# martinruenz/co-fusion

Hardware: AMD Instinct MI355X
Metric: frames/sec at 640x480 (N active models) + ICP-reduce achieved HBM GB/s vs peak (higher is better)
Workload: dtype f32

## Files before the change

co_fusion_amd/csrc/cabi_model.hip:

```cpp
#include <math.h>
#include <string.h>

#include <string>
#include <vector>

#include "cf_host.h"

using namespace cf;

#define HIPCHK(ctx, call)                                                                      \
    do {                                                                                       \
        hipError_t e_ = (call);                                                                \
        if (e_ != hipSuccess) {                                                                \
            (ctx)->set_error(std::string(#call) + ": " + hipGetErrorString(e_));               \
            return CF_EHIP;                                                                    \
        }                                                                                      \
    } while (0)
#define LAUNCHCHK(ctx) HIPCHK(ctx, hipGetLastError())

struct cf_model {
    cf_ctx* ctx = nullptr;
    uint32_t max_surfels = 0;
    uint32_t count_host = 0;
    bool count_pending = false;
    hipEvent_t count_event = nullptr;
    hipEvent_t count_wait = nullptr;
    bool ratio_valid = false;
    hipEvent_t ratio_event = nullptr;
    float* buf[2] = {nullptr, nullptr};
    int target = 0;
    float* staged = nullptr;
    unsigned* flags = nullptr;
    unsigned* block_sums = nullptr;
    unsigned* d_count = nullptr;
    unsigned* d_nfresh = nullptr;
    unsigned* d_tmp2 = nullptr;
    unsigned* h_counts = nullptr;
    float* records = nullptr;
    float* fresh = nullptr;
    unsigned* new_flags = nullptr;
    bool new_flags_clean = true;
    unsigned* owner = nullptr;
    float* fb_rec = nullptr;
    float* fb_raw = nullptr;
    float* fb_filt = nullptr;
    unsigned long long* keys = nullptr;
    unsigned* index = nullptr;
    float *vertConf = nullptr, *colorTime = nullptr, *normRad = nullptr;
    float* clean_rec = nullptr;
    uint8_t* splat_image = nullptr;
    float *splat_vertex = nullptr, *splat_normal = nullptr;
    uint16_t* splat_time = nullptr;
    float *fill_vertex = nullptr, *fill_normal = nullptr;
    uint8_t* fill_image = nullptr;
    float *tcx = nullptr, *tcy = nullptr;
    float* t_inv_dev = nullptr;
    const cf_odom* preindex_od = nullptr;
    int preindex_time = -1;
    float preindex_cutoff = 0.f; int preindex_delta = 0; uint32_t preindex_nb = 0;
    void drop_preindex() { preindex_od = nullptr; preindex_time = -1; }
    float* rays = nullptr;
    float inv_fx = 0, inv_fy = 0;
};

template <typename T>
static int dmalloc(cf_ctx* ctx, T** p, size_t count)
{
    HIPCHK(ctx, hipMalloc(reinterpret_cast<void**>(p), count * sizeof(T)));
    HIPCHK(ctx, hipMemsetAsync(*p, 0, count * sizeof(T), ctx->cur()));
    return CF_OK;
}

using cf::inv44f;

static inline cf_cam ctx_cam(const cf_ctx* ctx) { return cf_cam{ctx->cfg.fx, ctx->cfg.fy, ctx->cfg.cx, ctx->cfg.cy}; }

extern "C" {

int cf_bilateral(cf_ctx* ctx, const float* depth, int cols, int rows, float maxD, float* out)
{
    if (!ctx || !depth || !out) return CF_EINVAL;
    launch_bilateral(ctx->cur(), depth, cols, rows, maxD, out);
    LAUNCHCHK(ctx);
    return CF_OK;
}

int cf_model_create(cf_ctx* ctx, int max_surfels, cf_model** out)
{
    if (!ctx || !out || max_surfels <= 0) return CF_EINVAL;
    cf_model* m = new cf_model();
    m->ctx = ctx; m->max_surfels = (uint32_t)max_surfels;
    *out = m;
    const int W = ctx->cfg.width, H = ctx->cfg.height;
    const size_t N = (size_t)W * H, M = (size_t)max_surfels, Q = N / 4 + 64;
    if (int r = dmalloc(ctx, &m->buf[0], M * 12)) return r;
    if (int r = dmalloc(ctx, &m->buf[1], M * 12)) return r;
    if (int r = dmalloc(ctx, &m->staged, (M + Q) * 12)) return r;
    if (int r = dmalloc(ctx, &m->flags, M + Q)) return r;
    if (int r = dmalloc(ctx, &m->block_sums, (M + Q) / 2048 + N / 2048 + 16)) return r;
    if (int r = dmalloc(ctx, &m->d_count, 1)) return r;
    if (int r = dmalloc(ctx, &m->d_nfresh, 1)) return r;
    if (int r = dmalloc(ctx, &m->d_tmp2, 4)) return r;
    if (int r = dmalloc(ctx, &m->records, N * 12)) return r;
    if (int r = dmalloc(ctx, &m->fresh, Q * 12)) return r;
    if (int r = dmalloc(ctx, &m->new_flags, N)) return r;
    if (int r = dmalloc(ctx, &m->owner, M)) return r;
    HIPCHK(ctx, hipMemsetAsync(m->owner, 0xFF, M * sizeof(unsigned), ctx->cur()));
    if (int r = dmalloc(ctx, &m->fb_rec, N * 12)) return r;
    if (int r = dmalloc(ctx, &m->fb_raw, N * 12)) return r;
    if (int r = dmalloc(ctx, &m->fb_filt, N * 12)) return r;
    if (int r = dmalloc(ctx, &m->keys, N)) return r;
    HIPCHK(ctx, hipMemsetAsync(m->keys, 0xFF, N * sizeof(unsigned long long), ctx->cur()));
    if (int r = dmalloc(ctx, &m->index, N)) return r;
    if (int r = dmalloc(ctx, &m->vertConf, N * 4)) return r;
    if (int r = dmalloc(ctx, &m->colorTime, N * 4)) return r;
    if (int r = dmalloc(ctx, &m->normRad, N * 4)) return r;
    if (int r = dmalloc(ctx, &m->clean_rec, N * 8)) return r;
    if (int r = dmalloc(ctx, &m->splat_image, N * 4)) return r;
    if (int r = dmalloc(ctx, &m->splat_vertex, N * 4)) return r;
    if (int r = dmalloc(ctx, &m->splat_normal, N * 4)) return r;
    if (int r = dmalloc(ctx, &m->splat_time, N)) return r;
    if (int r = dmalloc(ctx, &m->fill_vertex, N * 4)) return r;
    if (int r = dmalloc(ctx, &m->fill_normal, N * 4)) return r;
    if (int r = dmalloc(ctx, &m->fill_image, N * 4)) return r;
    if (int r = dmalloc(ctx, &m->tcx, (size_t)W)) return r;
    if (int r = dmalloc(ctx, &m->tcy, (size_t)H)) return r;
    if (int r = dmalloc(ctx, &m->rays, N * 4)) return r;
    if (int r = dmalloc(ctx, &m->t_inv_dev, 16)) return r;
    launch_splat_rays(ctx->cur(), ctx_cam(ctx), W, H, m->rays);
    HIPCHK(ctx, hipHostMalloc(reinterpret_cast<void**>(&m->h_counts), sizeof(unsigned) * 4, hipHostMallocCoherent));
    HIPCHK(ctx, hipEventCreateWithFlags(&m->count_event, hipEventDisableTiming));
    HIPCHK(ctx, hipEventCreateWithFlags(&m->ratio_event, hipEventDisableTiming));
    std::vector<float> tx(W), ty(H);
    for (int i = 0; i < W; i++) tx[i] = (float)((double)((float)i / (float)W) + 1.0 / (2.0 * (double)(float)W));
    for (int j = 0; j < H; j++) ty[j] = (float)((double)((float)j / (float)H) + 1.0 / (2.0 * (double)(float)H));
    HIPCHK(ctx, hipMemcpyAsync(m->tcx, tx.data(), sizeof(float) * W, hipMemcpyHostToDevice, ctx->cur()));
    HIPCHK(ctx, hipMemcpyAsync(m->tcy, ty.data(), sizeof(float) * H, hipMemcpyHostToDevice, ctx->cur()));
    m->inv_fx = (float)(1.0 / (double)ctx->cfg.fx); m->inv_fy = (float)(1.0 / (double)ctx->cfg.fy);
    HIPCHK(ctx, hipStreamSynchronize(ctx->cur()));
    return CF_OK;
}

void cf_model_destroy(cf_model* m)
{
    if (!m) return;
    (void)hipStreamSynchronize(m->ctx->cur());
    void* ptrs[] = {m->buf[0], m->buf[1], m->staged, m->flags, m->block_sums, m->d_count, m->d_nfresh, m->d_tmp2, m->records,
                    m->fresh, m->new_flags, m->owner, m->fb_rec, m->fb_raw, m->fb_filt, m->keys, m->index, m->vertConf,
                    m->colorTime, m->normRad, m->splat_image, m->splat_vertex, m->splat_normal, m->splat_time, m->fill_vertex,
                    m->fill_normal, m->fill_image, m->tcx, m->tcy, m->rays, m->t_inv_dev, m->clean_rec};
    for (void* p : ptrs) (void)hipFree(p);
    (void)hipHostFree(m->h_counts);
    if (m->count_event) (void)hipEventDestroy(m->count_event);
    if (m->ratio_event) (void)hipEventDestroy(m->ratio_event);
    delete m;
}

static int adopt_count(cf_model* m)
{
    m->count_host = m->h_counts[0];
    m->count_pending = false;
    if (m->count_host > m->max_surfels) { m->ctx->set_error("surfel buffer overflow"); return CF_ENOMEM; }
    return CF_OK;
}
static int sync_count(cf_model* m)
{
    cf_ctx* ctx = m->ctx;
    HIPCHK(ctx, hipMemcpyAsync(m->h_counts, m->d_count, sizeof(unsigned), hipMemcpyDeviceToHost, ctx->cur()));
    HIPCHK(ctx, hipStreamSynchronize(ctx->cur()));
    return adopt_count(m);
}
static int post_count(cf_model* m, uint32_t upper_bound)
{
    cf_ctx* ctx = m->ctx;
    HIPCHK(ctx, hipEventRecord(m->count_event, ctx->cur()));
    m->count_wait = m->count_event;
    m->count_host = upper_bound;
    m->count_pending = true;
    return CF_OK;
}
static int count_bound(cf_model* m, uint32_t* out)
{
    if (m->count_pending) {
        if (!m->count_wait) { if (int r = sync_count(m)) return r; *out = m->count_host; return CF_OK; }
        if (hipEventQuery(m->count_wait) == hipSuccess) { if (int r = adopt_count(m)) return r; }
        else (void)hipGetLastError();
    }
    *out = m->count_host;
    return CF_OK;
}
static int exact_count(cf_model* m, uint32_t* out)
{
    if (m->count_pending) {
        if (!m->count_wait) { if (int r = sync_count(m)) return r; *out = m->count_host; return CF_OK; }
        HIPCHK(m->ctx, hipEventSynchronize(m->count_wait));
        if (int r = adopt_count(m)) return r;
    }
    *out = m->count_host;
    return CF_OK;
}

int cf_model_initialise(cf_model* m, const uint8_t* rgba, const float* depth_raw, const float* depth_filt, int time, float maxDepth)
{
    if (!m || !rgba || !depth_raw || !depth_filt) return CF_EINVAL;
    m->drop_preindex();
    cf_ctx* ctx = m->ctx; hipStream_t s = ctx->cur();
    const int W = ctx->cfg.width, H = ctx->cfg.height; const long long N = (long long)W * H;
    if ((uint32_t)N > m->max_surfels) return CF_ENOMEM;
    const cf_cam cam = ctx_cam(ctx);
    launch_feedback(s, rgba, depth_raw, W, H, cam, m->inv_fx, m->inv_fy, m->tcx, m->tcy, time, maxDepth, m->fb_rec, m->new_flags);
    HIPCHK(ctx, hipMemsetAsync(m->fb_raw, 0, sizeof(float) * 12 * N, s));
    launch_scan_scatter(s, m->fb_rec, m->new_flags, N, m->block_sums, m->d_count, 0, m->fb_raw);
    launch_feedback(s, rgba, depth_filt, W, H, cam, m->inv_fx, m->inv_fy, m->tcx, m->tcy, time, maxDepth, m->fb_rec, m->new_flags);
    HIPCHK(ctx, hipMemsetAsync(m->fb_filt, 0, sizeof(float) * 12 * N, s));
    launch_scan_scatter(s, m->fb_rec, m->new_flags, N, m->block_sums, m->d_tmp2, 0, m->fb_filt);
    m->new_flags_clean = false;
    launch_init(s, m->fb_raw, m->fb_filt, m->d_count, N, m->buf[m->target]);
    LAUNCHCHK(ctx);
    return sync_count(m);
}

int cf_model_count(cf_model* m, uint32_t* count) { if (!m || !count) return CF_EINVAL; return exact_count(m, count); }

int cf_model_predict_indices(cf_model* m, const float pose[16], int time, float maxDepth, int timeDelta)
{
    if (!m || !pose) return CF_EINVAL;
    m->drop_preindex();
    cf_ctx* ctx = m->ctx;
    float t_inv[16];
    inv44f(pose, t_inv);
    uint32_t nb = 0;
    if (int r = count_bound(m, &nb)) return r;
    launch_predict_indices(ctx->cur(), m->buf[m->target], m->d_count, nb, t_inv, ctx_cam(ctx), ctx->cfg.width, ctx->cfg.height,
                           maxDepth, time, timeDelta, m->keys, m->index, m->vertConf, m->colorTime, m->normRad);
    LAUNCHCHK(ctx);
    return CF_OK;
}

int cf_model_index_keys(cf_model* m, const float pose[16], int time, float maxDepth, int timeDelta, uint32_t surfel_begin, uint32_t surfel_end,
                        uint64_t* keys_dev)
{
    if (!m || !pose || !keys_dev || surfel_begin > surfel_end) return CF_EINVAL;
    m->drop_preindex();
    cf_ctx* ctx = m->ctx;
    const int W = ctx->cfg.width, H = ctx->cfg.height;
    float t_inv[16];
    inv44f(pose, t_inv);
    uint32_t nb = 0;
    if (int r = count_bound(m, &nb)) return r;
    HIPCHK(ctx, hipMemsetAsync(keys_dev, 0xFF, sizeof(uint64_t) * (size_t)W * H, ctx->cur()));
    launch_index_keys(ctx->cur(), m->buf[m->target], m->d_count, surfel_begin, surfel_end < nb ? surfel_end : nb, t_inv, ctx_cam(ctx), W, H, maxDepth,
                      time, timeDelta, reinterpret_cast<unsigned long long*>(keys_dev));
    LAUNCHCHK(ctx);
    return CF_OK;
}
int cf_model_index_resolve(cf_model* m, const float pose[16], uint64_t* keys_dev)
{
    if (!m || !pose || !keys_dev) return CF_EINVAL;
    m->drop_preindex();
    cf_ctx* ctx = m->ctx;
    float t_inv[16];
    inv44f(pose, t_inv);
    launch_index_resolve(ctx->cur(), m->buf[m->target], t_inv, ctx->cfg.width, ctx->cfg.height, reinterpret_cast<unsigned long long*>(keys_dev),
                         m->index, m->vertConf, m->colorTime, m->normRad);
    LAUNCHCHK(ctx);
    return CF_OK;
}

int cf_model_predict_indices_sharded(cf_model* m, const float pose[16], int time, float maxDepth, int timeDelta, int shard, int nshards)
{
    if (!m || !pose || nshards < 1 || shard < 0 || shard >= nshards) return CF_EINVAL;
    m->drop_preindex();
    cf_ctx* ctx = m->ctx;
    if (!ctx->collective) { ctx->set_error("cf_model_predict_indices_sharded: no collective registered (cf_set_collective)"); return CF_ESTATE; }
    uint32_t n = 0;
    if (int r = exact_count(m, &n)) return r;
    const uint32_t b = (uint32_t)(((uint64_t)n * (uint64_t)shard) / (uint64_t)nshards), e = (uint32_t)(((uint64_t)n * (uint64_t)(shard + 1)) / (uint64_t)nshards);
    if (int r = cf_model_index_keys(m, pose, time, maxDepth, timeDelta, b, e, reinterpret_cast<uint64_t*>(m->keys))) return r;
    if (ctx->collective(ctx->collective_user, 1, m->keys, (uint64_t)ctx->cfg.width * ctx->cfg.height, (void*)ctx->cur()) != 0) {
        ctx->set_error("cf_model_predict_indices_sharded: the collective failed");
        return CF_ESTATE;
    }
    return cf_model_index_resolve(m, pose, reinterpret_cast<uint64_t*>(m->keys));
}

int cf_model_combined_predict(cf_model* m, const float pose[16], float maxDepth, float confThreshold, int time, int maxTime, int timeDelta)
{
    if (!m || !pose) return CF_EINVAL;
    cf_ctx* ctx = m->ctx;
    float t_inv[16];
    inv44f(pose, t_inv);
    uint32_t nb = 0;
    if (int r = count_bound(m, &nb)) return r;
    launch_combined_predict(ctx->cur(), m->buf[m->target], m->d_count, nb, t_inv, ctx_cam(ctx), ctx->cfg.width, ctx->cfg.height,
                            maxDepth, confThreshold, time, maxTime, timeDelta, m->rays, m->keys, m->splat_image, m->splat_vertex, m->splat_normal,
                            m->splat_time);
    LAUNCHCHK(ctx);
    m->ratio_valid = false;
    return CF_OK;
}

int cf_model_prefetch_fill_ratio(cf_model* m)
{
    if (!m) return CF_EINVAL;
    cf_ctx* ctx = m->ctx;
    launch_fill_ratio(ctx->cur(), m->splat_image, ctx->cfg.width, ctx->cfg.height, m->d_tmp2 + 2, m->h_counts + 2);
    LAUNCHCHK(ctx);
    HIPCHK(ctx, hipEventRecord(m->ratio_event, ctx->cur()));
    m->ratio_valid = true;
    return CF_OK;
}

int cf_model_perform_fill_in(cf_model* m, const uint8_t* rgba, const float* depth_filt, int passthrough_geom, int passthrough_rgb)
{
    if (!m || !rgba || !depth_filt) return CF_EINVAL;
    cf_ctx* ctx = m->ctx;
    launch_fill_in(ctx->cur(), m->splat_vertex, m->splat_normal, m->splat_image, depth_filt, rgba, ctx->cfg.width, ctx->cfg.height, ctx_cam(ctx),
                   m->inv_fx, m->inv_fy, passthrough_geom, passthrough_rgb, m->fill_vertex, m->fill_normal, m->fill_image);
    LAUNCHCHK(ctx);
    return CF_OK;
}

int cf_model_requires_fill_in(cf_model* m, float ratio, int* out)
{
    if (!m || !out) return CF_EINVAL;
    cf_ctx* ctx = m->ctx;
    if (m->ratio_valid) {
        HIPCHK(ctx, hipEventSynchronize(m->ratio_event));
    } else {
        launch_fill_ratio(ctx->cur(), m->splat_image, ctx->cfg.width, ctx->cfg.height, m->d_tmp2 + 2, m->h_counts + 2);
        LAUNCHCHK(ctx);
        HIPCHK(ctx, hipStreamSynchronize(ctx->cur()));
    }
    *out = ((float)m->h_counts[2] / (float)m->h_counts[3] < ratio) ? 1 : 0;
    return CF_OK;
}

int cf_model_fill_ratio_device(cf_model* m, const uint32_t** counts_dev)
{
    if (!m || !counts_dev) return CF_EINVAL;
    *counts_dev = m->ratio_valid ? m->d_tmp2 + 2 : nullptr;
    return CF_OK;
}

int cf_model_fuse(cf_model* m, const float pose[16], int time, const uint8_t* rgba, const uint8_t* mask, const float* depth_raw,
                  const float* depth_filt, float maxDepth, float weighting, int maskID)
{
    if (!m || !pose || !rgba || !mask || !depth_raw || !depth_filt) return CF_EINVAL;
    m->drop_preindex();
    cf_ctx* ctx = m->ctx; hipStream_t s = ctx->cur();
    const int W = ctx->cfg.width, H = ctx->cfg.height; const long long N = (long long)W * H;
    SurfelFuseArgs a;
    a.index = m->index; a.vertConf = m->vertConf; a.normRad = m->normRad; a.rgba = rgba; a.depth_raw = depth_raw; a.depth_filt = depth_filt;
    a.mask = mask; a.tcx = m->tcx; a.tcy = m->tcy; memcpy(a.pose, pose, sizeof(a.pose)); a.cam = ctx_cam(ctx); a.inv_fx = m->inv_fx;
    a.inv_fy = m->inv_fy; a.cols = W; a.rows = H; a.time = time; a.weighting = weighting; a.maskID = maskID; a.maxDepth = maxDepth;
    a.records = m->records; a.new_flags = m->new_flags; a.owner = m->owner; a.flags_clean = m->new_flags_clean ? 1 : 0;
    launch_associate(s, a);
    {
        ScanPassArgs sp{m->records, m->new_flags, N, m->block_sums, m->d_nfresh, 0, m->fresh, nullptr};
        sp.zero_flags = 1;
        launch_scan_scatter_batch(s, &sp, 1);
        m->new_flags_clean = true;
    }
    uint32_t nb = 0;
    if (int r = count_bound(m, &nb)) return r;
    launch_update(s, m->buf[m->target], m->d_count, nb, m->owner, m->records, time, m->buf[1 - m->target]);
    m->target = 1 - m->target;
    LAUNCHCHK(ctx);
    return CF_OK;
}

int cf_model_clean(cf_model* m, const float pose[16], int time, float confThreshold, float outlierCoeff, int timeDelta, const float* depth_filt,
                   const uint8_t* mask, int maskID, uint32_t* count_out)
{
    if (!m || !pose || !depth_filt || !mask) return CF_EINVAL;
    m->drop_preindex();
    cf_ctx* ctx = m->ctx; hipStream_t s = ctx->cur();
    const int W = ctx->cfg.width, H = ctx->cfg.height;
    uint32_t nb = 0;
    if (int r = count_bound(m, &nb)) return r;
    const unsigned bound = nb + (unsigned)((W / 2) * (H / 2));
    if (bound > m->max_surfels + (unsigned)(W * H / 4 + 64)) return CF_ENOMEM;
    SurfelCleanArgs a;
    a.index = m->index; a.vertConf = m->vertConf; a.colorTime = m->colorTime; a.depth_filt = depth_filt; a.mask = mask; a.rec = nullptr;
    inv44f(pose, a.t_inv); a.cam = ctx_cam(ctx); a.cols = W; a.rows = H; a.time = time; a.confThreshold = confThreshold;
    a.outlierCoeff = outlierCoeff; a.timeDelta = timeDelta; a.maskID = maskID;
    launch_clean(s, m->buf[m->target], m->d_count, m->fresh, m->d_nfresh, bound, a, m->staged, m->flags);
    launch_scan_scatter(s, m->staged, m->flags, bound, m->block_sums, m->d_count, 0, m->buf[1 - m->target], m->h_counts);
    m->target = 1 - m->target;
    LAUNCHCHK(ctx);
    const uint32_t upper = bound < m->max_surfels ? bound : m->max_surfels;
    if (int r = post_count(m, upper)) return r;
    if (count_out) return exact_count(m, count_out);
    return CF_OK;
}

int cf_models_preindex(cf_ctx* ctx, const cf_model_preindex* items, int n, float depth_cutoff, int time_delta)
{
    if (!ctx || !items || n <= 0) return CF_EINVAL;
    hipStream_t s = ctx->cur();
    const int W = ctx->cfg.width, H = ctx->cfg.height;
    std::vector<IndexPassArgs> a((size_t)n);
    for (int k = 0; k < n; k++) {
        cf_model* m = items[k].model; const cf_odom* od = items[k].odom;
        if (!m || !od || m->ctx != ctx || od->ctx != ctx) return CF_EINVAL;
        uint32_t nb = 0;
        if (int r = count_bound(m, &nb)) return r;
        const float* pinv = reinterpret_cast<const float*>(reinterpret_cast<const char*>(od->d_state) + offsetof(cf::OdomDev, pose_inv));
        IndexPassArgs& p = a[k];
        p.surfels = m->buf[m->target]; p.count = m->d_count; p.id_begin = 0; p.id_end = nb; p.maxDepth = depth_cutoff; p.time = items[k].time;
        p.timeDelta = time_delta; p.keys = m->keys; p.index = m->index; p.vertConf = m->vertConf; p.colorTime = m->colorTime; p.normRad = m->normRad;
        p.t_inv_dev = pinv;
    }
    launch_index_keys_batch(s, a.data(), n, ctx_cam(ctx), W, H);
    launch_index_resolve_batch(s, a.data(), n, ctx_cam(ctx), W, H);
    LAUNCHCHK(ctx);
    for (int k = 0; k < n; k++) {
        cf_model* m = items[k].model;
        m->preindex_od = items[k].odom; m->preindex_time = items[k].time; m->preindex_cutoff = depth_cutoff; m->preindex_delta = time_delta; m->preindex_nb = a[k].id_end;
    }
    return CF_OK;
}
static bool preindexed_with(const cf_model* m, const float pose[16], int time, float depth_cutoff, int time_delta, uint32_t nb)
{
    if (!m->preindex_od || m->preindex_time != time) return false;
    if (m->preindex_cutoff != depth_cutoff || m->preindex_delta != time_delta || m->preindex_nb != nb) return false;
    const cf::OdomDev* h = m->preindex_od->h_state;
    for (int r = 0; r < 3; r++) {
        if (memcmp(&pose[r * 4], &h->Rcurr[r * 3], 12) != 0 || memcmp(&pose[r * 4 + 3], &h->tcurr[r], 4) != 0) return false;
    }
    return pose[12] == 0 && pose[13] == 0 && pose[14] == 0 && pose[15] == 1;
}

int cf_models_frame_passes(cf_ctx* ctx, const cf_model_pass* items, int n, float depth_cutoff, float outlier_coeff, int time_delta)
{
    if (!ctx || !items || n <= 0) return CF_EINVAL;
    hipStream_t s = ctx->cur();
    const int W = ctx->cfg.width, H = ctx->cfg.height; const long long N = (long long)W * H;
    const cf_cam cam = ctx_cam(ctx);
    std::vector<int> fusing;
    for (int k = 0; k < n; k++) {
        const cf_model_pass& it = items[k];
        if (!it.model || it.model->ctx != ctx || !it.pose || !it.rgba || !it.depth_filtered) return CF_EINVAL;
        if (it.do_fuse) { if (!it.mask || !it.depth_raw) return CF_EINVAL; fusing.push_back(k); }
    }
    for (int k : fusing) {
        cf_model* m = items[k].model;
        uint32_t nb = 0;
        if (int r = count_bound(m, &nb)) return r;
        if (nb + (unsigned)((W / 2) * (H / 2)) > m->max_surfels + (unsigned)(W * H / 4 + 64)) {
            ctx->set_error("cf_models_frame_passes: a model's surfel buffer cannot hold the clean stage's staging area (max_surfels too small)");
            return CF_ENOMEM;
        }
    }
    for (int k = 0; k < n; k++) { uint32_t nb = 0; if (int r = count_bound(items[k].model, &nb)) return r; }
    int surf_ev = -1;
    if (ctx->prof.enabled > 0 && (ctx->surf_calls_seen++ % (unsigned)ctx->prof.enabled) == 0 && ctx->surf_used + 2 <= cf_ctx::kSurfEvents) {
        for (int e = ctx->surf_used; e < ctx->surf_used + 2; e++)
            if (!ctx->surf_events[e]) HIPCHK(ctx, hipEventCreate(&ctx->surf_events[e]));
        surf_ev = ctx->surf_used; ctx->surf_used += 2;
        HIPCHK(ctx, hipEventRecord(ctx->surf_events[surf_ev], s));
        for (int k = 0; k < n; k++) ctx->surf_bytes += (uint64_t)items[k].model->count_host * 48u * (items[k].do_fuse ? 8u : 2u);
        ctx->surf_calls++;
    }
    static const bool clean_rec_on = getenv("CF_NO_CLEAN_REC") == nullptr;
    auto index_args_of = [&](const std::vector<int>& which, bool feeds_clean, std::vector<IndexPassArgs>& a) -> int {
        a.assign(which.size(), IndexPassArgs{});
        for (size_t q = 0; q < which.size(); q++) {
            const cf_model_pass& it = items[which[q]]; cf_model* m = it.model;
            uint32_t nb = 0;
            if (int r = count_bound(m, &nb)) return r;
            IndexPassArgs& p = a[q];
            p.surfels = m->buf[m->target]; p.count = m->d_count; p.id_begin = 0; p.id_end = nb; inv44f(it.pose, p.t_inv); p.maxDepth = depth_cutoff;
            p.time = it.time; p.timeDelta = time_delta; p.keys = m->keys; p.index = m->index; p.vertConf = m->vertConf; p.colorTime = m->colorTime;
            p.normRad = m->normRad;
            if (feeds_clean && clean_rec_on) { p.clean_rec = m->clean_rec; p.clean_depth = it.depth_filtered; }
        }
        return CF_OK;
    };
    auto index_pass = [&](const std::vector<int>& which) -> int {
        std::vector<IndexPassArgs> a;
        if (int r = index_args_of(which, false, a)) return r;
        launch_index_keys_batch(s, a.data(), (int)a.size(), cam, W, H);
        launch_index_resolve_batch(s, a.data(), (int)a.size(), cam, W, H);
        return CF_OK;
    };
    if (!fusing.empty()) {
        const int nf = (int)fusing.size();
        {
            std::vector<int> todo;
            for (int k : fusing) {
                uint32_t nb = 0;
                if (int r = count_bound(items[k].model, &nb)) return r;
                if (!preindexed_with(items[k].model, items[k].pose, items[k].time, depth_cutoff, time_delta, nb)) todo.push_back(k);
            }
            if (!todo.empty()) { if (int r = index_pass(todo)) return r; }
        }
        std::vector<SurfelFuseArgs> fa(nf);
        std::vector<ScanPassArgs> sa(nf);
        std::vector<UpdatePassArgs> ua(nf);
        for (int q = 0; q < nf; q++) {
            const cf_model_pass& it = items[fusing[q]]; cf_model* m = it.model;
            SurfelFuseArgs& a = fa[q];
            a.index = m->index; a.vertConf = m->vertConf; a.normRad = m->normRad; a.rgba = it.rgba; a.depth_raw = it.depth_raw; a.depth_filt = it.depth_filtered;
            a.mask = it.mask; a.tcx = m->tcx; a.tcy = m->tcy; memcpy(a.pose, it.pose, sizeof(a.pose)); a.cam = cam; a.inv_fx = m->inv_fx;
            a.inv_fy = m->inv_fy; a.cols = W; a.rows = H; a.time = it.time; a.weighting = it.weighting; a.maskID = it.mask_id; a.maxDepth = it.fuse_max_depth;
            a.records = m->records; a.new_flags = m->new_flags; a.owner = m->owner; a.flags_clean = m->new_flags_clean ? 1 : 0;
            sa[q] = ScanPassArgs{m->records, m->new_flags, N, m->block_sums, m->d_nfresh, 0, m->fresh, nullptr};
            sa[q].zero_flags = 1;
            m->new_flags_clean = true;
            uint32_t nb = 0;
            if (int r = count_bound(m, &nb)) return r;
            ua[q] = UpdatePassArgs{m->buf[m->target], m->d_count, nb, m->owner, m->records, it.time, m->buf[1 - m->target]};
        }
        launch_associate_batch(s, fa.data(), nf);
        for (int q = 0; q < nf; q++) items[fusing[q]].model->target = 1 - items[fusing[q]].model->target;
        {
            std::vector<IndexPassArgs> ia;
            if (int r = index_args_of(fusing, true, ia)) return r;
            static const bool side_by_side = getenv("CF_NO_SIDE_BY_SIDE") == nullptr;
            if (!(side_by_side && launch_update_compaction_index_keys(s, ua.data(), sa.data(), ia.data(), nf, cam, W, H))) {
                launch_scan_scatter_batch(s, sa.data(), nf);
                launch_update_batch(s, ua.data(), nf);
                launch_index_keys_batch(s, ia.data(), nf, cam, W, H);
            }
            launch_index_resolve_batch(s, ia.data(), nf, cam, W, H);
        }
        std::vector<CleanPassArgs> ca(nf);
        std::vector<uint32_t> upper(nf);
        for (int q = 0; q < nf; q++) {
            const cf_model_pass& it = items[fusing[q]]; cf_model* m = it.model;
            uint32_t nb = 0;
            if (int r = count_bound(m, &nb)) return r;
            const unsigned bound = nb + (unsigned)((W / 2) * (H / 2));
            if (bound > m->max_surfels + (unsigned)(W * H / 4 + 64)) return CF_ENOMEM;
            CleanPassArgs& c = ca[q];
            c.h.index = m->index; c.h.vertConf = m->vertConf; c.h.colorTime = m->colorTime; c.h.depth_filt = it.depth_filtered; c.h.mask = it.mask;
            c.h.rec = clean_rec_on ? m->clean_rec : nullptr;
            inv44f(it.pose, c.h.t_inv); c.h.cam = cam; c.h.cols = W; c.h.rows = H; c.h.time = it.time; c.h.confThreshold = it.conf_threshold;
            c.h.outlierCoeff = outlier_coeff; c.h.timeDelta = time_delta; c.h.maskID = it.mask_id;
            c.surfels = m->buf[m->target]; c.count = m->d_count; c.fresh = m->fresh; c.n_fresh = m->d_nfresh; c.total_bound = bound; c.staged = m->staged;
            c.flags = m->flags;
            sa[q] = ScanPassArgs{m->staged, m->flags, (long long)bound, m->block_sums, m->d_count, 0, m->buf[1 - m->target], m->h_counts};
            upper[q] = bound < m->max_surfels ? bound : m->max_surfels;
        }
        launch_clean_batch(s, ca.data(), nf);
        launch_scan_scatter_batch(s, sa.data(), nf);
        if (!ctx->batch_event) HIPCHK(ctx, hipEventCreateWithFlags(&ctx->batch_event, hipEventDisableTiming));
        for (int q = 0; q < nf; q++) {
            cf_model* m = items[fusing[q]].model;
            m->target = 1 - m->target;
            m->count_host = upper[q]; m->count_pending = true; m->count_wait = nullptr;
        }
    }
    std::vector<SplatPassArgs> pa(n);
    for (int k = 0; k < n; k++) {
        const cf_model_pass& it = items[k]; cf_model* m = it.model;
        uint32_t nb = m->count_host;
        if (!(m->count_pending && !m->count_wait)) { if (int r = count_bound(m, &nb)) return r; }
        SplatPassArgs& p = pa[k];
        p.surfels = m->buf[m->target]; p.count = m->d_count; p.count_bound = nb; inv44f(it.pose, p.t_inv); p.maxDepth = depth_cutoff;
        p.confThreshold = it.conf_threshold; p.time = it.time; p.maxTime = it.time; p.timeDelta = time_delta; p.rays = m->rays; p.keys = m->keys;
        p.image = m->splat_image; p.vertexConf = m->splat_vertex; p.normalRad = m->splat_normal; p.time16 = m->splat_time;
        m->ratio_valid = false;
    }
    launch_combined_predict_batch(s, pa.data(), n, cam, W, H);
    LAUNCHCHK(ctx);
    if (surf_ev >= 0) HIPCHK(ctx, hipEventRecord(ctx->surf_events[surf_ev + 1], s));
    if (!fusing.empty()) {
        HIPCHK(ctx, hipEventRecord(ctx->batch_event, s));
        for (int k : fusing) items[k].model->count_wait = ctx->batch_event;
    }
    for (int k = 0; k < n; k++) items[k].model->drop_preindex();
    return CF_OK;
}

int cf_model_download_map(cf_model* m, float* host_surfels, uint32_t capacity, uint32_t* count)
{
    if (!m || !count) return CF_EINVAL;
    cf_ctx* ctx = m->ctx;
    if (int r = exact_count(m, count)) return r;
    if (host_surfels) {
        const uint32_t n = m->count_host < capacity ? m->count_host : capacity;
        HIPCHK(ctx, hipMemcpyAsync(host_surfels, m->buf[m->target], (size_t)n * 48, hipMemcpyDeviceToHost, ctx->cur()));
        HIPCHK(ctx, hipStreamSynchronize(ctx->cur()));
    }
    return CF_OK;
}

int cf_model_upload_map(cf_model* m, const float* host_surfels, uint32_t count)
{
    if (!m || (!host_surfels && count) || count > m->max_surfels) return CF_EINVAL;
    m->drop_preindex();
    cf_ctx* ctx = m->ctx;
    if (count) HIPCHK(ctx, hipMemcpyAsync(m->buf[m->target], host_surfels, (size_t)count * 48, hipMemcpyHostToDevice, ctx->cur()));
    launch_set_count(ctx->cur(), m->d_count, count);
    HIPCHK(ctx, hipStreamSynchronize(ctx->cur()));
    m->count_host = count; m->count_pending = false;
    return CF_OK;
}

int cf_model_buffer(cf_model* m, int which, void** dptr, uint64_t* bytes)
{
    if (!m || !dptr) return CF_EINVAL;
    const size_t N = (size_t)m->ctx->cfg.width * m->ctx->cfg.height;
    void* p = nullptr; size_t b = 0;
    switch (which) {
        case 0: p = m->index; b = N * 4; break;
        case 1: p = m->vertConf; b = N * 16; break;
        case 2: p = m->colorTime; b = N * 16; break;
        case 3: p = m->normRad; b = N * 16; break;
        case 4: p = m->splat_image; b = N * 4; break;
        case 5: p = m->splat_vertex; b = N * 16; break;
        case 6: p = m->splat_normal; b = N * 16; break;
        case 7: p = m->splat_time; b = N * 2; break;
        case 8: p = m->fill_vertex; b = N * 16; break;
        case 9: p = m->fill_normal; b = N * 16; break;
        case 10: p = m->fill_image; b = N * 4; break;
        case 11: { uint32_t c = 0; if (int r = exact_count(m, &c)) return r; p = m->buf[m->target]; b = (size_t)c * 48; break; }
        default: return CF_EINVAL;
    }
    *dptr = p; if (bytes) *bytes = b;
    return CF_OK;
}

float cf_fusion_weight(const float pose[16], const float lastPose[16], float weightMultiplier)
{
    float pinv[16], diff[16];
    inv44f(pose, pinv);
    for (int i = 0; i < 4; i++)
        for (int j = 0; j < 4; j++) {
            float s = 0;
            for (int k = 0; k < 4; k++) s += pinv[i * 4 + k] * lastPose[k * 4 + j];
            diff[i * 4 + j] = s;
        }
    const float tn = sqrtf(diff[3] * diff[3] + diff[7] * diff[7] + diff[11] * diff[11]);
    const float* R = diff;
    double rx = R[2 * 4 + 1] - R[1 * 4 + 2], ry = R[0 * 4 + 2] - R[2 * 4 + 0], rz = R[1 * 4 + 0] - R[0 * 4 + 1];
    const double s = sqrt((rx * rx + ry * ry + rz * rz) * 0.25);
    double c = (double)((R[0] + R[5] + R[10]) - 1.0f) * 0.5;
    c = c > 1. ? 1. : c < -1. ? -1. : c;
    double theta = acos(c);
    if (s < 1e-5) {
        double t;
        if (c > 0) rx = ry = rz = 0;
        else {
            t = (R[0] + 1) * 0.5; rx = sqrt(t > 0.0 ? t : 0.0);
            t = (R[5] + 1) * 0.5; ry = sqrt(t > 0.0 ? t : 0.0) * (R[0 * 4 + 1] < 0 ? -1.0 : 1.0);
            t = (R[10] + 1) * 0.5; rz = sqrt(t > 0.0 ? t : 0.0) * (R[0 * 4 + 2] < 0 ? -1.0 : 1.0);
            if (fabs(rx) < fabs(ry) && fabs(rx) < fabs(rz) && (R[1 * 4 + 2] > 0) != (ry * rz > 0)) rz = -rz;
            theta /= sqrt(rx * rx + ry * ry + rz * rz);
            rx *= theta; ry *= theta; rz *= theta;
        }
    } else {
        double vth = 1 / (2 * s);
        vth *= theta;
        rx *= vth; ry *= vth; rz *= vth;
    }
    const float rv[3] = {(float)rx, (float)ry, (float)rz};
    const float rn = sqrtf(rv[0] * rv[0] + rv[1] * rv[1] + rv[2] * rv[2]);
    float weighting = tn > rn ? tn : rn;
    const float largest = 0.01f, minWeight = 0.5f;
    if (weighting > largest) weighting = largest;
    const float w = 1.0f - (weighting / largest);
    weighting = (w > minWeight ? w : minWeight) * weightMultiplier;
    return weighting;
}

}
```

co_fusion_amd/csrc/cf_kernels.h:

```cpp
#pragma once

#include <hip/hip_runtime.h>
#include <hip/hip_ext.h>
#include <stdint.h>

#include "../../include/cofusion_hip.h"

namespace cf {

constexpr int kGroups = 64;

struct alignas(64) GnHot {
    int icp, level_done; float cull_z[2];
    float Rcurr[9], tcurr[3];
    float Rprev_inv[9], tprev[3];
    int cull_box[4];
    int rgb, rgbOnly, level_done2, pad;
    float krkInv[9], kt[3];
};
static_assert(sizeof(GnHot) == 192, "three 64-byte lines");

struct OdomDev;
struct OdomDev {
    const float* vmap_curr[3];
    const float* nmap_curr[3];
    const float* vmap_g_prev[3];
    const float* nmap_g_prev[3];
    const float* lastDepth[3];
    const float* nextDepth[3];
    const uint8_t* lastImage[3];
    const uint8_t* nextImage[3];
    const uint8_t* lastNextImage[3];
    const int16_t* dIdx[3];
    const int16_t* dIdy[3];
    const float* cloud[3];
    cf_dataterm* corres[3];
    const uint8_t* cand[3];
    unsigned long long* icp_acc;
    unsigned long long* rgb_acc;
    float* err_surface;
    cf_cam intr;
    int width, height;
    float distThres, angleThres, sobelScale, maxDepthDeltaRGB;
    float minGrad[3];
    float icpWeight;
    int icp, rgb, rgbOnly;
    unsigned* aabb_acc;
    int cull;
    float box_R[9], box_t[3];
    unsigned* res_range;
    OdomDev* host_twin;
    float Rprev[9], tprev[3], Rprev_inv[9], Rcurr[9], tcurr[3];
    double resultRt[16];
    float krkInv[9], kt[3];
    float lastRGBError;
    int level_done;
    int solves;
    float residual[2];
    float box_lo[3], box_hi[3];
    int res_seen[3];
    float cull_z[2];
    float pose_inv[16];
    cf_track_stats stats;
    GnHot hot;
};
__host__ __device__ inline void refresh_hot(OdomDev* od)
{
    GnHot& h = od->hot;
    h.icp = od->icp; h.level_done = od->level_done; h.cull_z[0] = od->cull_z[0]; h.cull_z[1] = od->cull_z[1];
    for (int k = 0; k < 9; k++) { h.Rcurr[k] = od->Rcurr[k]; h.Rprev_inv[k] = od->Rprev_inv[k]; h.krkInv[k] = od->krkInv[k]; }
    for (int k = 0; k < 3; k++) { h.tcurr[k] = od->tcurr[k]; h.tprev[k] = od->tprev[k]; h.kt[k] = od->kt[k]; }
    for (int k = 0; k < 4; k++) h.cull_box[k] = od->stats.cull_box[k];
    h.rgb = od->rgb; h.rgbOnly = od->rgbOnly; h.level_done2 = od->level_done; h.pad = 0;
}

void launch_vmap(hipStream_t s, const float* depth, int cols, int rows, cf_cam intr, float cutoff, float* vmap);
void launch_nmap(hipStream_t s, const float* vmap, int cols, int rows, float* nmap);
void launch_copy_maps(hipStream_t s, const float* v4, const float* n4, int cols, int rows, float* vmap, float* nmap);
void launch_resize_map(hipStream_t s, const float* in, int in_cols, int in_rows, float* out, bool normalize);
void launch_transform_maps(hipStream_t s, float* vmap, float* nmap, int cols, int rows, const float R[9], const float t[3]);
void launch_vertices_to_depth(hipStream_t s, const float* v4, int cols, int rows, float cutoff, float* depth);
void launch_pyrdown_f32(hipStream_t s, const float* src, int scols, int srows, float* dst);
void launch_pyrdown_u8(hipStream_t s, const uint8_t* src, int scols, int srows, uint8_t* dst);
void launch_intensity(hipStream_t s, const uint8_t* rgba, int cols, int rows, uint8_t* dst);
void launch_rgb_expand(hipStream_t s, const uint8_t* rgb, int n, uint8_t* rgba);
void launch_sobel(hipStream_t s, const uint8_t* src, int cols, int rows, int16_t* dx, int16_t* dy);
void launch_cloud(hipStream_t s, const float* depth, int cols, int rows, cf_cam il, float* cloud3);

struct Level3 { int cols[3], rows[3], blk_end[3]; };
struct FrameMapsArgs {
    Level3 L;
    const float* depth[3]; float* vmap[3]; float* nmap[3];
    float fx_inv[3], fy_inv[3], cx[3], cy[3];
    float cutoff;
    float2* zrange[3];
};
struct RgbPrepArgs {
    Level3 L;
    const uint8_t* nextImage[3]; const float* nextDepth[3]; const float* lastDepth[3];
    int16_t* dIdx[3]; int16_t* dIdy[3]; uint8_t* cand[3]; float* cloud[3];
    float minScale[3], fx_inv[3], fy_inv[3], cx[3], cy[3];
    unsigned* res_range;
};
struct ModelMapsArgs {
    const float* pred_v4; const float* pred_n4;
    const float* alt_v4; const float* alt_n4;
    const unsigned* sel; float sel_ratio;
    float* snapshot;
    float* vmap[3]; float* nmap[3];
    int cols, rows;
    float R[9], t[3];
    unsigned char* occ;
    unsigned* aabb;
};
constexpr int kPrepBatch = 8;
struct ModelMapsBatch { ModelMapsArgs m[kPrepBatch]; };
struct RgbPrepBatch { RgbPrepArgs m[kPrepBatch]; };
struct RgbdChain {
    const float* v4; const uint8_t* rgba; float* depth[3]; uint8_t* image[3];
    const float* alt_v4; const uint8_t* alt_rgba; const unsigned* sel; float sel_ratio;
};
struct RgbdBatch {
    RgbdChain c[2 * kPrepBatch];
    uint8_t* fan_image[3][kPrepBatch];
    signed char fan_owner[kPrepBatch];
};
void launch_model_maps(hipStream_t s, const ModelMapsBatch& b, int n);
void launch_frame_maps(hipStream_t s, FrameMapsArgs a, int W, int H);
void launch_rgbd_pyramids(hipStream_t s, const RgbdBatch& b, int n_chains, int W, int H, float cutoff);
void launch_model_maps_and_pyramids(hipStream_t s, const ModelMapsBatch& mb, int n, const RgbdBatch& rb, int n_chains, int W, int H, float cutoff);
void launch_rgb_prep(hipStream_t s, RgbPrepBatch b, int n, int W, int H);

struct IDiv { unsigned M, s; };
inline IDiv make_idiv(int d)
{
    if (d < 2) return IDiv{0x80000000u, 0u};
    unsigned l = 0;
    while ((1u << l) < (unsigned)d) l++;
    return IDiv{(unsigned)((((unsigned long long)1 << (31 + l)) + (unsigned)d - 1) / (unsigned)d), l - 1};
}
constexpr int kGramBits[8] = {20, 20, 20, 17, 17, 17, 22, 0};
struct LaunchShape { int icp[3]; int res[3]; int icp_err; };
struct IcpLaunch { int threads; int ppt; int gram;
                   LaunchShape* const* shape = nullptr; };

constexpr int kMaxBatch = 16;
struct IcpModelArgs {
    const float* vc; const float* nc;
    const float* vp; const float* np;
    const OdomDev* st;
    unsigned long long* acc;
    float* err;
    const unsigned char* occ;
    int row_begin, row_end;
    int cull;
    const float2* zr;
    int box_blocks;
};
constexpr int kNoBoxHint = 0x7fffffff;
struct CullRuns { int x0, y0, nrx, total; };
__host__ __device__ inline CullRuns cull_runs(const int box[4], int L, int cols, int rows)
{
    int bx0 = (box[0] >> L) - 1, by0 = (box[1] >> L) - 1, bx1 = (box[2] >> L) + 1, by1 = (box[3] >> L) + 1;
    bx0 = bx0 < 0 ? 0 : bx0; by0 = by0 < 0 ? 0 : by0; bx1 = bx1 > cols - 1 ? cols - 1 : bx1; by1 = by1 > rows - 1 ? rows - 1 : by1;
    if (bx0 > bx1 || by0 > by1) return CullRuns{0, 0, 0, 0};
    if ((cols & 63) == 0) { const int nrx = (bx1 >> 6) - (bx0 >> 6) + 1; return CullRuns{bx0 >> 6, by0, nrx, nrx * (by1 - by0 + 1)}; }
    const int q0 = (by0 * cols) >> 6, q1 = ((by1 + 1) * cols - 1) >> 6;
    return CullRuns{0, q0, 0, q1 - q0 + 1};
}
inline int box_blocks_for(const int box_hint[4], int L, int cols, int rows, int threads)
{
    if (box_hint[0] == kNoBoxHint) return 0;
    const CullRuns cr = cull_runs(box_hint, L, cols, rows);
    const int wpb = threads / 64;
    const int runs = cr.total + cr.total / 4 + 2 * (cr.nrx > 0 ? cr.nrx : (cols + 63) / 64);
    int want = (((runs + 2 * wpb - 1) / (2 * wpb) + 7) / 8) * 8;
    return want < 8 ? 8 : want;
}
inline int residual_blocks_for(int seen) { return seen < 0 ? 0 : seen + seen / 4 + 2; }
struct GnArgs {
    OdomDev* od[kMaxBatch];
    unsigned long long* icp_acc[kMaxBatch];
    unsigned long long* rgb_acc[kMaxBatch];
    OdomDev* od_host[kMaxBatch];
    int slot_px;
    int icp_gram;
};
struct RgbModelArgs {
    OdomDev* st;
    const uint8_t* cand; const float* nextDepth; const float* lastDepth;
    const uint8_t* lastImage; const uint8_t* nextImage;
    cf_dataterm* corres; const float* cloud; const int16_t* dIdx; const int16_t* dIdy;
    unsigned long long* icp_acc; unsigned long long* rgb_acc;
    int no_counts;
    uint2* recs;
    unsigned* slot_counts;
    const unsigned* res_range;
    int res_blocks;
};
struct RgbArgs {
    RgbModelArgs m[kMaxBatch];
    int cols, rows;
    cf_cam il;
    float sobelScale, maxDepthDelta;
    int compact;
    int slot_px;
    IDiv cdiv;
};
inline RgbModelArgs rgb_model_args(const OdomDev* h , OdomDev* d_state, int level)
{
    return RgbModelArgs{d_state, h->cand[level], h->nextDepth[level], h->lastDepth[level], h->lastImage[level], h->nextImage[level],
                        h->corres[level], h->cloud[level], h->dIdx[level], h->dIdy[level], h->icp_acc, h->rgb_acc, 0,
                        reinterpret_cast<uint2*>(h->corres[level]),
                        reinterpret_cast<unsigned*>(reinterpret_cast<uint2*>(h->corres[level]) + (size_t)(h->width >> level) * (h->height >> level)),
                        h->res_range ? h->res_range + 2 * level : nullptr, 0};
}
constexpr int kMaxSlots = 2 * kMaxBatch;
struct IcpArgs {
    IcpModelArgs m[kMaxBatch];
    int cols, rows;
    cf_cam intr;
    float distThres, angleThres;
    float angleSqLt, distSqLe;
    int occ_w, occ_shift;
    int flags;
    int row_begin, row_end;
    IDiv cdiv;
    int slot_end[kMaxSlots];
    unsigned char slot_desc[kMaxSlots];
    int slots_used;
};
constexpr unsigned char kResidualSlot = 0x80;
void launch_icp_level(hipStream_t s, IcpLaunch cfg, const IcpArgs& args, int n, int level, hipEvent_t ev0 = nullptr, hipEvent_t ev1 = nullptr);
void launch_rgb_residual(hipStream_t s, const RgbArgs& ra, int n);
void launch_rgb_step(hipStream_t s, const RgbArgs& ra, int n);
constexpr uint64_t kRgbResidualBytes = 27;
constexpr uint64_t kRgbResidualBytesCompact = 11;
void launch_acc_total(hipStream_t s, const unsigned long long* acc, unsigned long long* out);
void launch_rgb_cand(hipStream_t s, const int16_t* dIdx, const int16_t* dIdy, const float* next_depth,
                     const uint8_t* next_image, float min_scale, int cols, int rows, uint8_t* cand);
void launch_so3_step(hipStream_t s, const uint8_t* last_image, const uint8_t* next_image, const float basis[9],
                     const float kinv[9], const float krlr[9], int cols, int rows, unsigned long long* out16);

struct ProfSink {
    hipEvent_t* events; int capacity; int used; uint64_t bytes; uint64_t launches; int enabled;
};

constexpr int kSo3Blocks = 16;
constexpr int kStepSubs = 16;
struct So3Sync { unsigned long long acc[10][16]; unsigned arrive, depart;
                 unsigned step_top, pad;
                 unsigned step_sub[kStepSubs][32]; };
struct GnHook { int (*fn)(void* user, int op, void* dev_buf, uint64_t words, void* stream); void* user; int split[kMaxBatch]; };
struct TrackerStates { OdomDev* dev[kMaxBatch]; const OdomDev* host[kMaxBatch]; };
bool launch_gn_track(hipStream_t s, IcpLaunch cfg, const TrackerStates& states, So3Sync* so3_syncs ,
                     const GnHook* hook, const IcpArgs icp_args[3], const RgbArgs rgb_args[3], int n, int width, int height, bool so3,
                     bool pyramid, bool fast_odom, bool rgb, bool icp, int mode, ProfSink* prof,
                     OdomDev* const* h_states = nullptr ,
                     const RgbPrepBatch* prep = nullptr );
void rgb_prep_levels(RgbPrepBatch& b, int n, int W, int H);
float replay_icp_level0(hipStream_t s, IcpLaunch cfg, const IcpArgs& a0, const RgbArgs& r0, int n, int slots, int ablate, int reps, hipEvent_t e0, hipEvent_t e1);
#ifdef CF_ABLATE
void trace_so3_dump(hipStream_t s);
void trace_solve_begin();
void trace_solve_end(hipStream_t s, const char* path);
void trace_step_solve(hipStream_t s, IcpLaunch cfg, const IcpArgs& a0, const RgbArgs& r0, So3Sync* syncs, int n, const char* path);
void trace_icp_level0(hipStream_t s, IcpLaunch cfg, const IcpArgs& a0, const RgbArgs& r0, int n, int slots, const char* path);
#endif
bool probe_xcd_round_robin(hipStream_t s);
float sqrt_gate_lt(float T);
float sqrt_gate_le(float T);

constexpr int kSurfBatch = 16;
struct IndexPassArgs {
    const float* surfels; const unsigned* count; unsigned id_begin, id_end; float t_inv[16]; float maxDepth; int time, timeDelta;
    unsigned long long* keys; unsigned* index; float* vertConf; float* colorTime; float* normRad;
    const float* t_inv_dev;
    float* clean_rec;
    const float* clean_depth;
};
__host__ __device__ inline void inv44f(const float a[16], float o[16])
{
    const float c00 = a[5] * a[10] - a[6] * a[9];
    const float c01 = a[6] * a[8] - a[4] * a[10];
    const float c02 = a[4] * a[9] - a[5] * a[8];
    const float det = a[0] * c00 + a[1] * c01 + a[2] * c02;
    const float id = 1.0f / det;
    float Li[9];
    Li[0] = c00 * id; Li[1] = (a[2] * a[9] - a[1] * a[10]) * id; Li[2] = (a[1] * a[6] - a[2] * a[5]) * id;
    Li[3] = c01 * id; Li[4] = (a[0] * a[10] - a[2] * a[8]) * id; Li[5] = (a[2] * a[4] - a[0] * a[6]) * id;
    Li[6] = c02 * id; Li[7] = (a[1] * a[8] - a[0] * a[9]) * id; Li[8] = (a[0] * a[5] - a[1] * a[4]) * id;
    for (int i = 0; i < 3; i++) {
        o[i * 4 + 0] = Li[i * 3 + 0]; o[i * 4 + 1] = Li[i * 3 + 1]; o[i * 4 + 2] = Li[i * 3 + 2];
        o[i * 4 + 3] = -(Li[i * 3 + 0] * a[3] + Li[i * 3 + 1] * a[7] + Li[i * 3 + 2] * a[11]);
    }
    o[12] = 0; o[13] = 0; o[14] = 0; o[15] = 1;
}
struct SplatPassArgs {
    const float* surfels; const unsigned* count; unsigned count_bound; float t_inv[16]; float maxDepth, confThreshold; int time, maxTime, timeDelta;
    const float* rays; unsigned long long* keys; uint8_t* image; float* vertexConf; float* normalRad; uint16_t* time16;
};
struct UpdatePassArgs { const float* in; const unsigned* count; unsigned count_bound; unsigned* owner; const float* records; int time; float* out; };
struct SurfelFuseArgs {
    const unsigned* index; const float* vertConf; const float* normRad;
    const uint8_t* rgba; const float* depth_raw; const float* depth_filt; const uint8_t* mask;
    const float* tcx; const float* tcy;
    float pose[16]; cf_cam cam; float inv_fx, inv_fy;
    int cols, rows, time; float weighting; int maskID; float maxDepth;
    float* records; unsigned* new_flags; unsigned* owner;
    int flags_clean = 0;
};
struct SurfelCleanArgs {
    const unsigned* index; const float* vertConf; const float* colorTime;
    const float* depth_filt; const uint8_t* mask;
    const float* rec;
    float t_inv[16]; cf_cam cam; int cols, rows, time; float confThreshold, outlierCoeff; int timeDelta, maskID;
};
struct CleanPassArgs {
    SurfelCleanArgs h; const float* surfels; const unsigned* count; const float* fresh; const unsigned* n_fresh; unsigned total_bound;
    float* staged; unsigned* flags;
};
struct ScanPassArgs {
    const float* rec; const unsigned* flags; long long n; unsigned* block_sums; unsigned* total; unsigned add_to_total; float* out; unsigned* total_host;
    int zero_flags = 0;
};
void launch_index_keys_batch(hipStream_t s, const IndexPassArgs* items, int n, cf_cam cam, int cols, int rows);
bool launch_update_compaction_index_keys(hipStream_t s, const UpdatePassArgs* up, const ScanPassArgs* sc, const IndexPassArgs* ix, int n, cf_cam cam, int cols,
                                         int rows);
void launch_index_resolve_batch(hipStream_t s, const IndexPassArgs* items, int n, cf_cam cam, int cols, int rows);
void launch_combined_predict_batch(hipStream_t s, const SplatPassArgs* items, int n, cf_cam cam, int cols, int rows);
void launch_associate_batch(hipStream_t s, const SurfelFuseArgs* items, int n);
void launch_update_batch(hipStream_t s, const UpdatePassArgs* items, int n);
void launch_clean_batch(hipStream_t s, const CleanPassArgs* items, int n);
void launch_scan_scatter_batch(hipStream_t s, const ScanPassArgs* items, int n);
void launch_bilateral(hipStream_t s, const float* depth, int cols, int rows, float maxD, float* out);
void launch_scan_scatter(hipStream_t s, const float* rec, const unsigned* flags, long long n, unsigned* block_sums, unsigned* total,
                         unsigned add_to_total, float* out, unsigned* total_host = nullptr );
void launch_feedback(hipStream_t s, const uint8_t* rgba, const float* depth, int cols, int rows, cf_cam cam, float inv_fx, float inv_fy,
                     const float* tcx, const float* tcy, int time, float maxDepth, float* rec, unsigned* flags);
void launch_init(hipStream_t s, const float* raw, const float* filt, const unsigned* raw_count, long long max_n, float* out);
void launch_index_keys(hipStream_t s, const float* surfels, const unsigned* count, unsigned id_begin, unsigned id_end, const float t_inv[16],
                       cf_cam cam, int cols, int rows, float maxDepth, int time, int timeDelta, unsigned long long* keys);
void launch_index_resolve(hipStream_t s, const float* surfels, const float t_inv[16], int cols, int rows, unsigned long long* keys,
                          unsigned* index, float* vertConf, float* colorTime, float* normRad);
void launch_predict_indices(hipStream_t s, const float* surfels, const unsigned* count, unsigned count_bound, const float t_inv[16], cf_cam cam,
                            int cols, int rows, float maxDepth, int time, int timeDelta, unsigned long long* keys, unsigned* index,
                            float* vertConf, float* colorTime, float* normRad);
void launch_splat_rays(hipStream_t s, cf_cam cam, int cols, int rows, float* rays );
void launch_combined_predict(hipStream_t s, const float* surfels, const unsigned* count, unsigned count_bound, const float t_inv[16], cf_cam cam,
                             int cols, int rows, float maxDepth, float confThreshold, int time, int maxTime, int timeDelta,
                             const float* rays, unsigned long long* keys, uint8_t* image, float* vertexConf, float* normalRad, uint16_t* time16);
void launch_fill_in(hipStream_t s, const float* pv, const float* pn, const uint8_t* pimg, const float* depth, const uint8_t* rgba, int cols,
                    int rows, cf_cam cam, float inv_fx, float inv_fy, int pass_geom, int pass_rgb, float* ov, float* on, uint8_t* oi);
void launch_fill_ratio(hipStream_t s, const uint8_t* pimg, int cols, int rows, unsigned* out2, unsigned* out2_host = nullptr );
void launch_associate(hipStream_t s, const SurfelFuseArgs& h);
void launch_update(hipStream_t s, const float* in, const unsigned* count, unsigned count_bound, unsigned* owner, const float* records, int time,
                   float* out);
void launch_clean(hipStream_t s, const float* surfels, const unsigned* count, const float* fresh, const unsigned* n_fresh, unsigned total_bound,
                  const SurfelCleanArgs& h, float* staged, unsigned* flags);
void launch_set_count(hipStream_t s, unsigned* out, unsigned v);

}
```

co_fusion_amd/csrc/cf_surfel_device.h:

```cpp
#pragma once

#include "cf_device.h"

namespace cf {

struct Surfel { float4 pos_conf, col_time, norm_rad; };

__device__ __forceinline__ int iclamp(int v, int lo, int hi) { return v < lo ? lo : (v > hi ? hi : v); }
__device__ __forceinline__ int nearest_texel(float u, int size) { return iclamp((int)floorf(u * (float)size), 0, size - 1); }

__device__ __forceinline__ float det_expf(float x)
{
    if (!(x > -87.0f)) return (x != x) ? x : 0.0f;
    if (x > 88.0f) return __int_as_float(0x7f800000);
    const float n = rintf(x * 1.44269504088896341f);
    float r = x - n * 0.693145751953125f;
    r = r - n * 1.42860682030941723212e-6f;
    float p = 1.0f / 720.0f;
    p = p * r + 1.0f / 120.0f;
    p = p * r + 1.0f / 24.0f;
    p = p * r + 1.0f / 6.0f;
    p = p * r + 0.5f;
    p = p * r + 1.0f;
    p = p * r + 1.0f;
    return ldexpf(p, (int)n);
}
__device__ __forceinline__ float det_acos_r(float z)
{
    const float pS0 = 1.6666586697e-01f, pS1 = -4.2743422091e-02f, pS2 = -8.6563630030e-03f, qS1 = -7.0662963390e-01f;
    const float p = z * (pS0 + z * (pS1 + z * pS2));
    const float q = 1.0f + z * qS1;
    return p / q;
}
__device__ __forceinline__ float det_acosf(float x)
{
    const float pio2 = 1.57079637050628662109375f, pi = 3.1415927410125732421875f;
    if (x != x || x > 1.0f || x < -1.0f) return qnan();
    if (fabsf(x) < 0.5f) return pio2 - (x + x * det_acos_r(x * x));
    if (x < 0.0f) {
        const float z = (1.0f + x) * 0.5f, s = sqrtf(z);
        return pi - 2.0f * (s + s * det_acos_r(z));
    }
    const float z = (1.0f - x) * 0.5f, s = sqrtf(z);
    return 2.0f * (s + s * det_acos_r(z));
}

__device__ __forceinline__ float get_radius(float depth, float norm_z, float inv_fx, float inv_fy)
{
    const float meanFocal = ((1.0f / fabsf(inv_fx)) + (1.0f / fabsf(inv_fy))) / 2.0f;
    const float sqrt2 = 1.41421356237f;
    const float radius = (depth / meanFocal) * sqrt2;
    float radius_n = radius;
    radius_n = radius_n / fabsf(norm_z);
    radius_n = fminf(2.0f * radius, radius_n);
    return radius_n;
}
__device__ __forceinline__ float confidence(float x, float y, float cx, float cy, float weighting)
{
    const float dx = x - cx, dy = y - cy;
    const float radialDist = sqrtf(dx * dx + dy * dy) / 400.0f;
    return det_expf((-(radialDist * radialDist) / 0.72f)) * weighting;
}
__device__ __forceinline__ float glsl_round(float v) { return (v < 0) ? -floorf(-v + 0.5f) : floorf(v + 0.5f); }
__device__ __forceinline__ float encode_color(float r, float g, float b)
{
    int rgb = (int)glsl_round(r * 255.0f);
    rgb = (rgb << 8) + (int)glsl_round(g * 255.0f);
    rgb = (rgb << 8) + (int)glsl_round(b * 255.0f);
    return (float)rgb;
}
__device__ __forceinline__ f3 decode_color(float c)
{
    const int ci = (int)c;
    return f3{(float)((ci >> 16) & 0xFF) / 255.0f, (float)((ci >> 8) & 0xFF) / 255.0f, (float)(ci & 0xFF) / 255.0f};
}

struct Mat4 { float m[16]; };
__device__ __forceinline__ f3 xform_point(const Mat4& T, f3 p)
{
    return f3{T.m[0] * p.x + T.m[1] * p.y + T.m[2] * p.z + T.m[3], T.m[4] * p.x + T.m[5] * p.y + T.m[6] * p.z + T.m[7],
              T.m[8] * p.x + T.m[9] * p.y + T.m[10] * p.z + T.m[11]};
}
__device__ __forceinline__ f3 xform_dir(const Mat4& T, f3 p)
{
    return f3{T.m[0] * p.x + T.m[1] * p.y + T.m[2] * p.z, T.m[4] * p.x + T.m[5] * p.y + T.m[6] * p.z,
              T.m[8] * p.x + T.m[9] * p.y + T.m[10] * p.z};
}

__device__ __forceinline__ float4 tex4_linear(const float4* __restrict__ img, int cols, int rows, float u, float v)
{
    const float fu = u * (float)cols - 0.5f, fv = v * (float)rows - 0.5f;
    const float x0f = floorf(fu), y0f = floorf(fv);
    const float wx = fu - x0f, wy = fv - y0f;
    const int x0 = iclamp((int)x0f, 0, cols - 1), x1 = iclamp((int)x0f + 1, 0, cols - 1);
    const int y0 = iclamp((int)y0f, 0, rows - 1), y1 = iclamp((int)y0f + 1, 0, rows - 1);
    const float4 a = img[y0 * cols + x0], b = img[y0 * cols + x1], c = img[y1 * cols + x0], d = img[y1 * cols + x1];
    float4 r;
    {
        const float top = a.x * (1.0f - wx) + b.x * wx, bot = c.x * (1.0f - wx) + d.x * wx;
        r.x = top * (1.0f - wy) + bot * wy;
    }
    {
        const float top = a.y * (1.0f - wx) + b.y * wx, bot = c.y * (1.0f - wx) + d.y * wx;
        r.y = top * (1.0f - wy) + bot * wy;
    }
    {
        const float top = a.z * (1.0f - wx) + b.z * wx, bot = c.z * (1.0f - wx) + d.z * wx;
        r.z = top * (1.0f - wy) + bot * wy;
    }
    {
        const float top = a.w * (1.0f - wx) + b.w * wx, bot = c.w * (1.0f - wx) + d.w * wx;
        r.w = top * (1.0f - wy) + bot * wy;
    }
    return r;
}

__device__ __forceinline__ f3 get_vertex(const float* __restrict__ depth, int cols, int rows, int px, int py, float x, float y,
                                         float cx, float cy, float inv_fx, float inv_fy)
{
    const float z = depth[iclamp(py, 0, rows - 1) * cols + iclamp(px, 0, cols - 1)];
    return f3{(x - cx) * z * inv_fx, (y - cy) * z * inv_fy, z};
}
__device__ __forceinline__ f3 half_sum(f3 a, f3 b) { return f3{(a.x + b.x) / 2, (a.y + b.y) / 2, (a.z + b.z) / 2}; }
__device__ __forceinline__ f3 get_normal_central(f3 p, const float* __restrict__ depth, int cols, int rows, int px, int py, float x,
                                                 float y, float cx, float cy, float inv_fx, float inv_fy)
{
    const f3 xf = get_vertex(depth, cols, rows, px + 1, py, x + 1, y, cx, cy, inv_fx, inv_fy);
    const f3 xb = get_vertex(depth, cols, rows, px - 1, py, x - 1, y, cx, cy, inv_fx, inv_fy);
    const f3 yf = get_vertex(depth, cols, rows, px, py + 1, x, y + 1, cx, cy, inv_fx, inv_fy);
    const f3 yb = get_vertex(depth, cols, rows, px, py - 1, x, y - 1, cx, cy, inv_fx, inv_fy);
    const f3 del_x = half_sum(xb, p) - half_sum(xf, p);
    const f3 del_y = half_sum(yb, p) - half_sum(yf, p);
    return normalized(cross(del_x, del_y));
}

}
```

co_fusion_amd/csrc/surfel.hip:

```cpp
#include "cf_surfel_device.h"
#include "cf_kernels.h"

namespace cf {

static constexpr int kB = 256;
static inline int gridFor(long long n) { return (int)((n + kB - 1) / kB); }
static inline int gridXcd(long long n, int chunk = 1) { const int q = 8 * (chunk > 1 ? chunk : 1); return (gridFor(n) + q - 1) / q * q; }
#ifdef CF_ABLATE
static int xcd_env(const char* name, int dflt) { const char* e = getenv(name); return e ? atoi(e) : dflt; }
#else
static constexpr int xcd_env(const char*, int dflt) { return dflt; }
#endif
struct BatchHdr { int n; int blk_end[kSurfBatch]; };
template <class A> struct Batch { BatchHdr h; A m[kSurfBatch]; };
struct VBlock { int model, bid, nblk; };
__device__ __forceinline__ VBlock batch_decode_at(const BatchHdr& h, int b)
{
    int slot = 0;
#pragma unroll
    for (int k = 0; k < kSurfBatch - 1; k++) slot += (b >= h.blk_end[k]) ? 1 : 0;
    const int start = slot ? h.blk_end[slot - 1] : 0;
    return VBlock{slot, b - start, h.blk_end[slot] - start};
}
__device__ __forceinline__ VBlock batch_decode(const BatchHdr& h) { return batch_decode_at(h, (int)blockIdx.x); }
template <class A>
static int batch_layout(Batch<A>& B, const int* blocks, int n)
{
    int total = 0;
    B.h.n = n;
    for (int k = 0; k < kSurfBatch; k++) {
        if (k < n) total += (blocks[k] + 7) / 8 * 8;
        B.h.blk_end[k] = k < n ? total : 0x7fffffff;
    }
    return total;
}

__device__ __forceinline__ int xcd_block(int chunk, int b, int nblk)
{
    if (chunk == 0) return b;
    const int per = nblk >> 3, x = b & 7, r = b >> 3;
    if (chunk < 0) return x * per + r;
    const int lb = ((r / chunk) * 8 + x) * chunk + (r % chunk);
    return lb;
}

__device__ __forceinline__ unsigned sortable_bits(float z)
{
    const unsigned b = __float_as_uint(z);
    return (b & 0x80000000u) ? ~b : (b | 0x80000000u);
}
__device__ __forceinline__ unsigned long long zkey(float z, unsigned id) { return ((unsigned long long)sortable_bits(z) << 32) | id; }
constexpr unsigned long long kEmptyKey = ~0ull;

__global__ void __launch_bounds__(kB) bilateral_kernel(const float* __restrict__ depth, int cols, int rows, float maxD,
                                                       float* __restrict__ out)
{
    const int i = blockIdx.x * kB + threadIdx.x;
    if (i >= cols * rows) return;
    const int y = i / cols, x = i - y * cols;
    const float value = depth[i];
    if (value > maxD || value < 0.3f) { out[i] = 0; return; }
    float sum1 = 0, sum2 = 0;
#pragma unroll
    for (int dy = -6; dy <= 6; ++dy) {
        const int cy = y + dy;
        if (cy < 0 || cy >= rows) continue;
        const float* __restrict__ rowp = depth + cy * cols + x;
#pragma unroll
        for (int dx = -6; dx <= 6; ++dx) {
            const int cx = x + dx;
            if (cx < 0 || cx >= cols) continue;
            const float tmp = rowp[dx];
            const float space2 = (float)(dx * dx + dy * dy);
            const float color2 = (value - tmp) * (value - tmp);
            const float weight = det_expf(-(space2 * 0.024691358f + color2 * 555.556f));
            sum1 += tmp * weight;
            sum2 += weight;
        }
    }
    out[i] = sum1 / sum2;
}

static constexpr int kScanItems = 2048;
struct ScanArgs {
    const float4* rec; const unsigned* flags; long long n; unsigned* block_sums; unsigned* total; unsigned add_to_total; float4* out;
    unsigned* total_host; int zero_flags;
};
__device__ __forceinline__ void scan_load_flags(const unsigned* __restrict__ flags, long long i0, long long n, unsigned (&f)[8])
{
    if (i0 + 8 <= n) {
        const uint4 a = *reinterpret_cast<const uint4*>(flags + i0), c = *reinterpret_cast<const uint4*>(flags + i0 + 4);
        f[0] = a.x; f[1] = a.y; f[2] = a.z; f[3] = a.w; f[4] = c.x; f[5] = c.y; f[6] = c.z; f[7] = c.w;
    } else {
        unsigned t[8];
#pragma unroll
        for (int e = 0; e < 8; e++) t[e] = flags[i0 + e < n ? i0 + e : n - 1];
#pragma unroll
        for (int e = 0; e < 8; e++) f[e] = (i0 + e < n) ? t[e] : 0u;
    }
}
__device__ __forceinline__ void scan_block_sums_body(const Batch<ScanArgs>& B, int blk)
{
    const VBlock vb = batch_decode_at(B.h, blk);
    const ScanArgs& a = B.m[vb.model];
    const unsigned* __restrict__ flags = a.flags; const long long n = a.n; unsigned* __restrict__ block_sums = a.block_sums;
    if ((long long)vb.bid * kScanItems >= n) return;
    unsigned f[8];
    scan_load_flags(flags, (long long)vb.bid * kScanItems + (long long)threadIdx.x * 8, n, f);
    unsigned s = 0;
#pragma unroll
    for (int e = 0; e < 8; e++) s += f[e];
    for (int o = 32; o > 0; o >>= 1) s += __shfl_xor((int)s, o, 64);
    __shared__ unsigned w[4];
    if ((threadIdx.x & 63) == 0) w[threadIdx.x >> 6] = s;
    __syncthreads();
    if (threadIdx.x == 0) block_sums[vb.bid] = w[0] + w[1] + w[2] + w[3];
}
__global__ void __launch_bounds__(256) scan_block_sums_kernel(const Batch<ScanArgs> B) { scan_block_sums_body(B, (int)blockIdx.x); }
__global__ void set_count_kernel(unsigned* out, unsigned v);
__global__ void set_count2_kernel(unsigned* out, unsigned* out_host, unsigned v);
__device__ __forceinline__ void scan_scatter_body(const Batch<ScanArgs>& B, int blk)
{
    const VBlock vb = batch_decode_at(B.h, blk);
    const ScanArgs& a = B.m[vb.model];
    const float4* __restrict__ rec = a.rec; const unsigned* __restrict__ flags = a.flags; const long long n = a.n;
    const unsigned* __restrict__ block_sums = a.block_sums; unsigned* __restrict__ total = a.total; const unsigned add_to_total = a.add_to_total;
    float4* __restrict__ out = a.out; unsigned* __restrict__ total_host = a.total_host;
    const int nb = (int)((n + kScanItems - 1) / kScanItems);
    if (vb.bid >= nb) return;
    __shared__ unsigned wsum[4], s_base;
    __shared__ unsigned short s_src[kScanItems];
    const int tid = threadIdx.x, lane = tid & 63, wave = tid >> 6;
    const long long i0 = (long long)vb.bid * kScanItems + (long long)tid * 8;
    unsigned f[8];
    scan_load_flags(flags, i0, n, f);
    if (a.zero_flags) {
        unsigned* fz = const_cast<unsigned*>(flags);
        if (i0 + 8 <= n) { *reinterpret_cast<uint4*>(fz + i0) = make_uint4(0, 0, 0, 0); *reinterpret_cast<uint4*>(fz + i0 + 4) = make_uint4(0, 0, 0, 0); }
        else
            for (int e = 0; e < 8; e++) if (i0 + e < n) fz[i0 + e] = 0;
    }
    unsigned b = 0;
    for (int k = tid; k < vb.bid; k += 256) b += block_sums[k];
    for (int o = 32; o > 0; o >>= 1) b += __shfl_xor((int)b, o, 64);
    if (lane == 0) wsum[wave] = b;
    __syncthreads();
    if (tid == 0) s_base = wsum[0] + wsum[1] + wsum[2] + wsum[3];
    unsigned mine = 0;
#pragma unroll
    for (int e = 0; e < 8; e++) mine += f[e];
    unsigned incl = mine;
    for (int o = 1; o < 64; o <<= 1) { const unsigned t = __shfl_up((int)incl, o, 64); if (lane >= o) incl += t; }
    __syncthreads();
    if (lane == 63) wsum[wave] = incl;
    __syncthreads();
    unsigned rel = incl - mine;
    for (int w = 0; w < wave; w++) rel += wsum[w];
#pragma unroll
    for (int e = 0; e < 8; e++)
        if (f[e]) s_src[rel++] = (unsigned short)(tid * 8 + e);
    const unsigned count = wsum[0] + wsum[1] + wsum[2] + wsum[3];
    const unsigned base = s_base;
    __syncthreads();
    const float4* __restrict__ in0 = rec + (size_t)vb.bid * kScanItems * 3;
    float4* __restrict__ out0 = out + (size_t)base * 3;
    const unsigned words = count * 3;
#ifndef CF_SCAN_FLY
#define CF_SCAN_FLY 4
#endif
    constexpr int kFly = CF_SCAN_FLY;
    for (unsigned m0 = tid; m0 < words; m0 += kFly * 256) {
        float4 v[kFly];
#pragma unroll
        for (int u = 0; u < kFly; u++) {
            const unsigned m = m0 + u * 256;
            const unsigned mc = m < words ? m : words - 1;
            const unsigned j = mc / 3u;
            v[u] = in0[(size_t)s_src[j] * 3 + (mc - 3u * j)];
        }
#pragma unroll
        for (int u = 0; u < kFly; u++) { const unsigned m = m0 + u * 256; if (m < words) out0[m] = v[u]; }
    }
    if (vb.bid == nb - 1 && tid == 255) {
        *total = base + count + add_to_total;
        if (total_host) *total_host = base + count + add_to_total;
    }
}
__global__ void __launch_bounds__(256) scan_scatter_kernel(const Batch<ScanArgs> B) { scan_scatter_body(B, (int)blockIdx.x); }

void launch_scan_scatter_batch(hipStream_t s, const ScanPassArgs* items, int n_items)
{
    for (int base = 0; base < n_items; base += kSurfBatch) {
        const int nb = n_items - base < kSurfBatch ? n_items - base : kSurfBatch;
        Batch<ScanArgs> B;
        int blocks[kSurfBatch], any = 0;
        for (int k = 0; k < nb; k++) {
            const ScanPassArgs& h = items[base + k];
            B.m[k] = ScanArgs{reinterpret_cast<const float4*>(h.rec), h.flags, h.n, h.block_sums, h.total, h.add_to_total, reinterpret_cast<float4*>(h.out), h.total_host, h.zero_flags};
            blocks[k] = (int)((B.m[k].n + kScanItems - 1) / kScanItems);
            any += blocks[k];
            if (blocks[k] == 0) set_count2_kernel<<<1, 1, 0, s>>>(B.m[k].total, B.m[k].total_host, B.m[k].add_to_total);
        }
        if (!any) continue;
        const int grid = batch_layout(B, blocks, nb);
        scan_block_sums_kernel<<<grid, 256, 0, s>>>(B);
        scan_scatter_kernel<<<grid, 256, 0, s>>>(B);
    }
}
void launch_scan_scatter(hipStream_t s, const float* rec, const unsigned* flags, long long n, unsigned* block_sums, unsigned* total,
                         unsigned add_to_total, float* out, unsigned* total_host)
{
    const ScanPassArgs a{rec, flags, n, block_sums, total, add_to_total, out, total_host};
    launch_scan_scatter_batch(s, &a, 1);
}

__global__ void __launch_bounds__(kB) feedback_kernel(const uchar4* __restrict__ rgba, const float* __restrict__ depth, int cols, int rows,
                                                      float cx, float cy, float inv_fx, float inv_fy, const float* __restrict__ tcx,
                                                      const float* __restrict__ tcy, int time, float maxDepth,
                                                      float4* __restrict__ rec , unsigned* __restrict__ flags)
{
    const int q = blockIdx.x * kB + threadIdx.x;
    if (q >= cols * rows) return;
    const int j = q / cols, i = q - j * cols;
    const int rank = i * rows + j;
    const float x = tcx[i] * (float)cols, y = tcy[j] * (float)rows;
    const f3 p = get_vertex(depth, cols, rows, i, j, x, y, cx, cy, inv_fx, inv_fy);
    if (p.z <= 0 || p.z > maxDepth) { flags[rank] = 0; return; }
    const f3 n = get_normal_central(p, depth, cols, rows, i, j, x, y, cx, cy, inv_fx, inv_fy);
    const uchar4 c = rgba[q];
    flags[rank] = 1;
    rec[rank * 3 + 0] = make_float4(p.x, p.y, p.z, confidence(x, y, cx, cy, 1.0f));
    rec[rank * 3 + 1] = make_float4(encode_color((float)c.x / 255.0f, (float)c.y / 255.0f, (float)c.z / 255.0f), 0.f, (float)c.z / 255.0f, (float)time);
    rec[rank * 3 + 2] = make_float4(n.x, n.y, n.z, get_radius(p.z, n.z, inv_fx, inv_fy));
}


__global__ void __launch_bounds__(kB) init_kernel(const float4* __restrict__ raw, const float4* __restrict__ filt,
                                                  const unsigned* __restrict__ raw_count, float4* __restrict__ out)
{
    const unsigned k = blockIdx.x * kB + threadIdx.x;
    if (k >= *raw_count) return;
    const float4 c = raw[k * 3 + 1];
    out[k * 3] = raw[k * 3];
    out[k * 3 + 1] = make_float4(c.x, 0.f, 1.f, c.w);
    out[k * 3 + 2] = filt[k * 3 + 2];
}

__device__ __forceinline__ bool index_project(const float4 pc, const float4 ct, const Mat4& t_inv, cf_cam cam, int cols, int rows,
                                              float maxDepth, int time, int timeDelta, f3& ph, int& q)
{
    ph = xform_point(t_inv, f3{pc.x, pc.y, pc.z});
    if (ph.z > maxDepth || ph.z < 0 || (float)time - ct.w > (float)timeDelta) return false;
    const float u = ((cam.fx * ph.x) / ph.z) + cam.cx, v = ((cam.fy * ph.y) / ph.z) + cam.cy;
    if (!(u >= 0.0f && v >= 0.0f && u < (float)cols && v < (float)rows)) return false;
    if (!(ph.z < maxDepth)) return false;
    q = (int)floorf(v) * cols + (int)floorf(u);
    return true;
}

struct IndexArgs {
    const float4* surfels; const unsigned* count; Mat4 t_inv; float maxDepth; int time, timeDelta; unsigned id_begin, id_end;
    unsigned long long* keys; unsigned* index; float4* vertConf; float4* colorTime; float4* normRad;
    const float* t_inv_dev;
    float4* clean_rec; const float* clean_depth;
};
__device__ __forceinline__ Mat4 index_matrix(const IndexArgs& a)
{
    if (!a.t_inv_dev) return a.t_inv;
    Mat4 m;
#pragma unroll
    for (int k = 0; k < 16; k++) m.m[k] = a.t_inv_dev[k];
    return m;
}
struct FrameGeom { cf_cam cam; int cols, rows; };

__device__ __forceinline__ void index_splat_body(const Batch<IndexArgs>& B, const FrameGeom& g, int blk)
{
    const VBlock vb = batch_decode_at(B.h, blk);
    const IndexArgs& a = B.m[vb.model];
    const float4* __restrict__ surfels = a.surfels;
    const unsigned id = a.id_begin + vb.bid * kB + threadIdx.x;
    if (id >= *a.count || id >= a.id_end) return;
    f3 ph; int q;
    const Mat4 T = index_matrix(a);
    if (!index_project(surfels[id * 3], surfels[id * 3 + 1], T, g.cam, g.cols, g.rows, a.maxDepth, a.time, a.timeDelta, ph, q)) return;
    atomicMin(&a.keys[q], zkey(ph.z, id));
}
__global__ void __launch_bounds__(kB) index_splat_kernel(const Batch<IndexArgs> B, const FrameGeom g) { index_splat_body(B, g, (int)blockIdx.x); }

__global__ void __launch_bounds__(kB) index_resolve_kernel(const Batch<IndexArgs> B, const FrameGeom g)
{
    const VBlock vb = batch_decode(B.h);
    const IndexArgs& a = B.m[vb.model];
    const float4* __restrict__ surfels = a.surfels; unsigned long long* __restrict__ keys = a.keys; unsigned* __restrict__ index = a.index;
    float4* __restrict__ vertConf = a.vertConf; float4* __restrict__ colorTime = a.colorTime; float4* __restrict__ normRad = a.normRad;
    const int q = vb.bid * kB + threadIdx.x;
    if (q >= g.cols * g.rows) return;
    const unsigned long long k = keys[q];
    keys[q] = kEmptyKey;
    float4* __restrict__ const rec = a.clean_rec;
    const float dflt = rec ? a.clean_depth[q] : 0.f;
    if (k == kEmptyKey) {
        index[q] = 0;
        vertConf[q] = colorTime[q] = normRad[q] = make_float4(0, 0, 0, 0);
        if (rec) { rec[2 * q] = make_float4(0, 0, 0, 0); rec[2 * q + 1] = make_float4(0, 0, __uint_as_float(0u), dflt); }
        return;
    }
    const unsigned id = (unsigned)k;
    const float4 pc = surfels[id * 3], ct = surfels[id * 3 + 1], nr = surfels[id * 3 + 2];
    const Mat4 T = index_matrix(a);
    const f3 ph = xform_point(T, f3{pc.x, pc.y, pc.z});
    const f3 n = normalized(xform_dir(T, f3{nr.x, nr.y, nr.z}));
    index[q] = id;
    vertConf[q] = make_float4(ph.x, ph.y, ph.z, pc.w);
    colorTime[q] = ct;
    normRad[q] = make_float4(n.x, n.y, n.z, nr.w);
    if (rec) { rec[2 * q] = make_float4(ph.x, ph.y, ph.z, pc.w); rec[2 * q + 1] = make_float4(ct.z, ct.w, __uint_as_float(id), dflt); }
}

struct SplatSetup { f3 ph, n; float rad, pn; int x_lo, x_hi, y_lo, y_hi; };

__device__ __forceinline__ bool splat_setup(const float4 pc, const float4 ct, const float4 nr, const Mat4& t_inv, cf_cam cam, int cols,
                                            int rows, float maxDepth, float confThreshold, int time, int maxTime, int timeDelta,
                                            SplatSetup& s)
{
    s.ph = xform_point(t_inv, f3{pc.x, pc.y, pc.z});
    if (s.ph.z > maxDepth || s.ph.z < 0 || pc.w < confThreshold || (float)time - ct.w > (float)timeDelta || ct.w > (float)maxTime) return false;
    s.n = normalized(xform_dir(t_inv, f3{nr.x, nr.y, nr.z}));
    s.rad = nr.w;
    const f3 x1n = normalized(f3{s.n.y - s.n.z, -s.n.x, s.n.x});
    const f3 x1 = {x1n.x * s.rad * 1.41421356f, x1n.y * s.rad * 1.41421356f, x1n.z * s.rad * 1.41421356f};
    const f3 y1 = cross(s.n, x1);
    const f3 c[4] = {s.ph + x1, s.ph + y1, s.ph - y1, s.ph - x1};
    float px_[4], py_[4];
#pragma unroll
    for (int k = 0; k < 4; k++) { px_[k] = ((cam.fx * c[k].x) / c[k].z) + cam.cx; py_[k] = ((cam.fy * c[k].y) / c[k].z) + cam.cy; }
    const float xmin = fminf(px_[0], fminf(px_[1], fminf(px_[2], px_[3]))), xmax = fmaxf(px_[0], fmaxf(px_[1], fmaxf(px_[2], px_[3])));
    const float ymin = fminf(py_[0], fminf(py_[1], fminf(py_[2], py_[3]))), ymax = fmaxf(py_[0], fmaxf(py_[1], fmaxf(py_[2], py_[3])));
    const float size = fmaxf(0.0f, fmaxf(fabsf(xmax - xmin), fabsf(ymax - ymin)));
    if (!(size > 0.0f) || !(size <= 4096.0f)) return false;
    const float u = ((cam.fx * s.ph.x) / s.ph.z) + cam.cx, v = ((cam.fy * s.ph.y) / s.ph.z) + cam.cy;
    if (!(u >= 0.0f && v >= 0.0f && u <= (float)cols && v <= (float)rows)) return false;
    const float half = size * 0.5f;
    s.x_lo = max((int)ceilf(u - half - 0.5f), 0); s.x_hi = min((int)ceilf(u + half - 0.5f) - 1, cols - 1);
    s.y_lo = max((int)ceilf(v - half - 0.5f), 0); s.y_hi = min((int)ceilf(v + half - 0.5f) - 1, rows - 1);
    s.pn = dot(s.ph, s.n);
    return true;
}

__device__ __forceinline__ bool splat_fragment(const SplatSetup& s, const float4* __restrict__ rays, int cols, int px, int py, float maxDepth,
                                               float& z)
{
    const float4 lr = rays[py * cols + px];
    const f3 l = {lr.x, lr.y, lr.z};
    const float k = s.pn / dot(l, s.n);
    const f3 cp = {k * l.x, k * l.y, k * l.z};
    const f3 diff = cp - s.ph;
    if (!(dot(diff, diff) <= s.rad * s.rad)) return false;
    if (!(cp.z < maxDepth)) return false;
    z = cp.z;
    return true;
}

__global__ void __launch_bounds__(kB) splat_rays_kernel(cf_cam cam, int cols, int rows, float4* __restrict__ rays)
{
    const int q = blockIdx.x * kB + threadIdx.x;
    if (q >= cols * rows) return;
    const int py = q / cols, px = q - py * cols;
    const float fx_ = (float)px + 0.5f, fy_ = (float)py + 0.5f;
    const f3 l = normalized(f3{(fx_ - cam.cx) / cam.fx, (fy_ - cam.cy) / cam.fy, 1.0f});
    rays[q] = make_float4(l.x, l.y, l.z, 0.f);
}

struct SplatArgs {
    const float4* surfels; const unsigned* count; Mat4 t_inv; float maxDepth, confThreshold; int time, maxTime, timeDelta;
    const float4* rays; unsigned long long* keys; uchar4* image; float4* vertexConf; float4* normalRad; unsigned short* time16;
};

__global__ void __launch_bounds__(kB) splat_raster_kernel(const Batch<SplatArgs> B, const FrameGeom g)
{
    const VBlock vb = batch_decode(B.h);
    const SplatArgs& a = B.m[vb.model];
    const float4* __restrict__ surfels = a.surfels; const float4* __restrict__ rays = a.rays; unsigned long long* __restrict__ keys = a.keys;
    const int cols = g.cols, rows = g.rows;
    const unsigned gt = vb.bid * kB + threadIdx.x;
    const unsigned id = gt >> 2;
    const int sub = (int)(gt & 3u);
    if (id >= *a.count) return;
    SplatSetup s;
    if (!splat_setup(surfels[id * 3], surfels[id * 3 + 1], surfels[id * 3 + 2], a.t_inv, g.cam, cols, rows, a.maxDepth, a.confThreshold, a.time,
                     a.maxTime, a.timeDelta, s))
        return;
    const int w = s.x_hi - s.x_lo + 1, h = s.y_hi - s.y_lo + 1;
    if (w <= 0 || h <= 0) return;
    int fx = sub, fy = 0;
    while (fx >= w) { fx -= w; fy++; }
    while (fy < h) {
        const int px = s.x_lo + fx, py = s.y_lo + fy;
        float z;
        if (splat_fragment(s, rays, cols, px, py, a.maxDepth, z)) {
            atomicMin(&keys[py * cols + px], zkey(z, id));
        }
        fx += 4;
        while (fx >= w) { fx -= w; fy++; }
    }
}

__global__ void __launch_bounds__(kB) splat_resolve_kernel(const Batch<SplatArgs> B, const FrameGeom g)
{
    const VBlock vb = batch_decode(B.h);
    const SplatArgs& a = B.m[vb.model];
    const float4* __restrict__ surfels = a.surfels; const float4* __restrict__ rays = a.rays; unsigned long long* __restrict__ keys = a.keys;
    uchar4* __restrict__ image = a.image; float4* __restrict__ vertexConf = a.vertexConf; float4* __restrict__ normalRad = a.normalRad;
    unsigned short* __restrict__ time16 = a.time16;
    const int cols = g.cols, rows = g.rows;
    const cf_cam cam = g.cam;
    const int q = vb.bid * kB + threadIdx.x;
    if (q >= cols * rows) return;
    const unsigned long long k = keys[q];
    keys[q] = kEmptyKey;
    if (k == kEmptyKey) {
        image[q] = make_uchar4(0, 0, 0, 0);
        vertexConf[q] = normalRad[q] = make_float4(0, 0, 0, 0);
        time16[q] = 0;
        return;
    }
    const unsigned id = (unsigned)k;
    const int py = q / cols, px = q - py * cols;
    const float4 pc = surfels[id * 3], ct = surfels[id * 3 + 1], nr = surfels[id * 3 + 2];
    SplatSetup s;
    splat_setup(pc, ct, nr, a.t_inv, cam, cols, rows, a.maxDepth, a.confThreshold, a.time, a.maxTime, a.timeDelta, s);
    float z;
    splat_fragment(s, rays, cols, px, py, a.maxDepth, z);
    const f3 col = decode_color(ct.x);
    image[q] = make_uchar4((unsigned char)glsl_round(col.x * 255.0f), (unsigned char)glsl_round(col.y * 255.0f),
                           (unsigned char)glsl_round(col.z * 255.0f), 255);
    const float fx_ = (float)px + 0.5f, fy_ = (float)py + 0.5f;
    vertexConf[q] = make_float4((fx_ - cam.cx) * z * (1.f / cam.fx), (fy_ - cam.cy) * z * (1.f / cam.fy), z, pc.w);
    normalRad[q] = make_float4(s.n.x, s.n.y, s.n.z, s.rad);
    time16[q] = (unsigned short)(unsigned)ct.z;
}

__global__ void __launch_bounds__(kB) fill_in_kernel(const float4* __restrict__ pv, const float4* __restrict__ pn, const uchar4* __restrict__ pimg,
                                                     const float* __restrict__ depth, const uchar4* __restrict__ rgba, int cols, int rows,
                                                     float cx, float cy, float inv_fx, float inv_fy, int pass_geom, int pass_rgb,
                                                     float4* __restrict__ ov, float4* __restrict__ on, uchar4* __restrict__ oi)
{
    const int q = blockIdx.x * kB + threadIdx.x;
    if (q >= cols * rows) return;
    const int y = q / cols, x = q - y * cols;
    const float z = depth[q];
    const f3 p = {((float)x - cx) * z * inv_fx, ((float)y - cy) * z * inv_fy, z};
    const float4 v = pv[q];
    ov[q] = (v.z == 0 || pass_geom) ? make_float4(p.x, p.y, p.z, 1.f) : v;
    const float4 n = pn[q];
    if (n.z == 0 || pass_geom) {
        const float zx = depth[y * cols + min(x + 1, cols - 1)], zy = depth[min(y + 1, rows - 1) * cols + x];
        const f3 vx = {((float)(x + 1) - cx) * zx * inv_fx, ((float)y - cy) * zx * inv_fy, zx};
        const f3 vy = {((float)x - cx) * zy * inv_fx, ((float)(y + 1) - cy) * zy * inv_fy, zy};
        const f3 nn = normalized(cross(vx - p, vy - p));
        on[q] = make_float4(nn.x, nn.y, nn.z, 1.f);
    } else
        on[q] = n;
    const uchar4 e = pimg[q];
    oi[q] = (((int)e.x + (int)e.y + (int)e.z) == 0 || pass_rgb) ? rgba[q] : e;
}

__global__ void __launch_bounds__(1024) fill_ratio_kernel(const uchar4* __restrict__ pimg, int cols, int rows, unsigned* __restrict__ out2,
                                                          unsigned* __restrict__ out2_host)
{
    const int dw = cols / 20, dh = rows / 20;
    unsigned s = 0;
    for (int k = threadIdx.x; k < dw * dh; k += 1024) {
        const int j = k / dw, i = k - j * dw;
        const int sx = nearest_texel(((float)i + 0.5f) / (float)dw, cols), sy = nearest_texel(((float)j + 0.5f) / (float)dh, rows);
        const uchar4 p = pimg[sy * cols + sx];
        s += (p.x > 0 && p.y > 0 && p.z > 0) ? 1u : 0u;
    }
    for (int o = 32; o > 0; o >>= 1) s += __shfl_xor((int)s, o, 64);
    __shared__ unsigned w[16];
    if ((threadIdx.x & 63) == 0) w[threadIdx.x >> 6] = s;
    __syncthreads();
    if (threadIdx.x == 0) {
        unsigned t = 0;
        for (int k = 0; k < 16; k++) t += w[k];
        out2[0] = t; out2[1] = (unsigned)(dw * dh);
        if (out2_host) { out2_host[0] = t; out2_host[1] = (unsigned)(dw * dh); }
    }
}

__device__ __forceinline__ float angle_between(f3 a, f3 b) { return det_acosf(dot(a, b) / (norm(a) * norm(b))); }

struct FuseArgs {
    const unsigned* index; const float4* vertConf; const float4* normRad;
    const uchar4* rgba; const float* depth_raw; const float* depth_filt; const unsigned char* mask;
    const float* tcx; const float* tcy;
    Mat4 pose; cf_cam cam; float inv_fx, inv_fy;
    int cols, rows, time; float weighting; int maskID; float maxDepth;
    float4* records;
    unsigned* new_flags;
    unsigned* owner;
};

__device__ __forceinline__ float bilerp(float a, float b, float c, float d, float wx, float wy)
{
    const float top = a * (1.0f - wx) + b * wx, bot = c * (1.0f - wx) + d * wx;
    return top * (1.0f - wy) + bot * wy;
}

static constexpr int kAssocItems = kB / 4;
static constexpr int kPatchStride = 7 * 16 + 1;

__global__ void __launch_bounds__(kB) associate_kernel(const Batch<FuseArgs> B, int xcd)
{
    __shared__ float s_patch[kAssocItems * kPatchStride];
    const VBlock vb = batch_decode(B.h);
    const FuseArgs& a = B.m[vb.model];
    const int cols = a.cols, rows = a.rows;
    const int par = a.time % 2;
    const int n_i = (cols - par + 1) / 2, n_j = (rows - par + 1) / 2;
    const int gt = xcd_block(xcd, vb.bid, vb.nblk) * kB + threadIdx.x;
    const int t = gt >> 2, sub = gt & 3;
    float* const P = s_patch + (threadIdx.x >> 2) * kPatchStride;
    bool alive = t < n_i * n_j;
    int i = 0, j = 0, q = 0, rank = 0;
    float tcx = 0, tcy = 0, x = 0, y = 0;
    f3 vPosLocal{0, 0, 0};
    if (alive) {
        j = 2 * (t / n_i) + par; i = 2 * (t % n_i) + par;
        q = j * cols + i; rank = i * rows + j;
        tcx = a.tcx[i]; tcy = a.tcy[j];
        x = tcx * (float)cols; y = tcy * (float)rows;
        alive = (((int)x % 2 == a.time % 2) && ((int)y % 2 == a.time % 2)) && ((int)a.mask[q] == a.maskID);
    }
    const float* dr = a.depth_raw;
    if (alive)
        alive = !(dr[j * cols + iclamp(i - 1, 0, cols - 1)] == 0 || dr[iclamp(j - 1, 0, rows - 1) * cols + i] == 0 ||
                  dr[j * cols + iclamp(i + 1, 0, cols - 1)] == 0 || dr[iclamp(j + 1, 0, rows - 1) * cols + i] == 0);
    const float cx = a.cam.cx, cy = a.cam.cy;
    if (alive) {
        vPosLocal = get_vertex(dr, cols, rows, i, j, x, y, cx, cy, a.inv_fx, a.inv_fy);
        alive = (vPosLocal.z > 0 && vPosLocal.z <= a.maxDepth);
    }
    const float scale = 1.0f;
    const float indexXStep = (1.0f / ((float)cols * scale)) * 0.5f, indexYStep = (1.0f / ((float)rows * scale)) * 0.5f;
    const float windowMultiplier = 2;
    const float iBeg = tcx - (scale * indexXStep * windowMultiplier), jBeg = tcy - (scale * indexYStep * windowMultiplier);
    const int X0 = (int)floorf(iBeg * (float)cols - 0.5f), Y0 = (int)floorf(jBeg * (float)rows - 0.5f);
    if (alive) {
#pragma unroll
        for (int c = 0; c < 4; c++) {
            const int k = sub * 4 + c;
            const int g = iclamp(Y0 + sub, 0, rows - 1) * cols + iclamp(X0 + c, 0, cols - 1);
            const float4 vcf = a.vertConf[g];
            const float4 nrd = a.normRad[g];
            const unsigned idx = a.index[g];
            P[0 * 16 + k] = vcf.x; P[1 * 16 + k] = vcf.y; P[2 * 16 + k] = vcf.z;
            P[3 * 16 + k] = nrd.x; P[4 * 16 + k] = nrd.y; P[5 * 16 + k] = nrd.z;
            P[6 * 16 + k] = __uint_as_float(idx);
        }
    }
    __syncthreads();
    if (!alive) return;

    const f3 vPos = xform_point(a.pose, vPosLocal);
    const f3 vPos_f = get_vertex(a.depth_filt, cols, rows, i, j, x, y, cx, cy, a.inv_fx, a.inv_fy);
    const f3 vNormLocal = get_normal_central(vPos_f, a.depth_filt, cols, rows, i, j, x, y, cx, cy, a.inv_fx, a.inv_fy);
    const float xl = (x - cx) * a.inv_fx, yl = (y - cy) * a.inv_fy;
    const float lambda = sqrtf(xl * xl + yl * yl + 1);
    const f3 ray = {xl, yl, 1};
    float bestDist = 1000;
    unsigned best = 0; int operation = 0, bestSeq = 0;
    float ii = iBeg;
    for (int s4 = 0; s4 < sub; s4++) ii += indexXStep;
    for (int outer = sub; ii < tcx + (scale * indexXStep * windowMultiplier);
         outer += 4, ii += indexXStep, ii += indexXStep, ii += indexXStep, ii += indexXStep) {
        int inner = 0;
        for (float jj = jBeg; jj < tcy + (scale * indexYStep * windowMultiplier); jj += indexYStep, inner++) {
            const int nlx = (int)floorf(ii * (float)cols) - X0, nly = (int)floorf(jj * (float)rows) - Y0;
            const unsigned current = ((unsigned)nlx < 4u && (unsigned)nly < 4u)
                                         ? __float_as_uint(P[6 * 16 + nly * 4 + nlx])
                                         : a.index[nearest_texel(jj, rows) * cols + nearest_texel(ii, cols)];
            if (current > 0U) {
                const float fu = ii * (float)cols - 0.5f, fv = jj * (float)rows - 0.5f;
                const float x0f = floorf(fu), y0f = floorf(fv);
                const int lx = (int)x0f - X0, ly = (int)y0f - Y0;
                const bool staged = (unsigned)lx < 3u && (unsigned)ly < 3u;
                const float wx = fu - x0f, wy = fv - y0f;
                const float* qd = P + (ly * 4 + lx);
                float4 vertConf;
                if (staged) {
                    vertConf.x = bilerp(qd[0 * 16], qd[0 * 16 + 1], qd[0 * 16 + 4], qd[0 * 16 + 5], wx, wy);
                    vertConf.y = bilerp(qd[1 * 16], qd[1 * 16 + 1], qd[1 * 16 + 4], qd[1 * 16 + 5], wx, wy);
                    vertConf.z = bilerp(qd[2 * 16], qd[2 * 16 + 1], qd[2 * 16 + 4], qd[2 * 16 + 5], wx, wy);
                } else
                    vertConf = tex4_linear(a.vertConf, cols, rows, ii, jj);
                const float zdiff = (vertConf.z - vPosLocal.z);
                if (fabsf(zdiff * lambda) < 0.05f) {
                    const float dist = norm(cross(ray, f3{vertConf.x, vertConf.y, vertConf.z}));
                    float4 normRad;
                    if (staged) {
                        normRad.x = bilerp(qd[3 * 16], qd[3 * 16 + 1], qd[3 * 16 + 4], qd[3 * 16 + 5], wx, wy);
                        normRad.y = bilerp(qd[4 * 16], qd[4 * 16 + 1], qd[4 * 16 + 4], qd[4 * 16 + 5], wx, wy);
                        normRad.z = bilerp(qd[5 * 16], qd[5 * 16 + 1], qd[5 * 16 + 4], qd[5 * 16 + 5], wx, wy);
                    } else
                        normRad = tex4_linear(a.normRad, cols, rows, ii, jj);
                    if (dist < bestDist && (fabsf(normRad.z) < 0.75f || fabsf(angle_between(f3{normRad.x, normRad.y, normRad.z}, vNormLocal)) < 0.5f)) {
                        operation = 1; bestDist = dist; best = current; bestSeq = outer * 64 + inner;
                    }
                }
            }
        }
    }
#pragma unroll
    for (int o = 1; o <= 2; o <<= 1) {
        const int oOp = __shfl_xor(operation, o, 4), oSeq = __shfl_xor(bestSeq, o, 4);
        const float oDist = __shfl_xor(bestDist, o, 4);
        const unsigned oBest = (unsigned)__shfl_xor((int)best, o, 4);
        const bool take = oOp && (!operation || oDist < bestDist || (oDist == bestDist && oSeq < bestSeq));
        if (take) { operation = 1; bestDist = oDist; best = oBest; bestSeq = oSeq; }
    }
    if (sub != 0) return;
    const uchar4 c = a.rgba[q];
    const f3 nG = xform_dir(a.pose, vNormLocal);
    const float radius = get_radius(vPos_f.z, vNormLocal.z, a.inv_fx, a.inv_fy);
    const float conf = confidence(x, y, cx, cy, a.weighting);
    const float col = (float)(((int)c.x << 16) + ((int)c.y << 8) + (int)c.z);
    a.records[rank * 3 + 0] = make_float4(vPos.x, vPos.y, vPos.z, conf);
    a.records[rank * 3 + 1] = make_float4(col, 0.f, (float)a.time, operation == 1 ? -1.f : -2.f);
    a.records[rank * 3 + 2] = make_float4(nG.x, nG.y, nG.z, radius);
    if (operation == 1) atomicMin(&a.owner[best], (unsigned)rank);
    else a.new_flags[rank] = 1;
}

struct UpdateArgs { const float4* in; const unsigned* count; unsigned* owner; const float4* records; int time; float4* out; };
__device__ __forceinline__ void update_body(const Batch<UpdateArgs>& B, int blk)
{
    const VBlock vb = batch_decode_at(B.h, blk);
    const UpdateArgs& ua = B.m[vb.model];
    const float4* __restrict__ in = ua.in; unsigned* __restrict__ owner = ua.owner; const float4* __restrict__ records = ua.records;
    float4* __restrict__ out = ua.out; const int time = ua.time;
    const unsigned id = vb.bid * kB + threadIdx.x;
    if (id >= *ua.count) return;
    const float4 pc = in[id * 3], ct = in[id * 3 + 1], nr = in[id * 3 + 2];
    const unsigned ow = owner[id];
    if (ow == 0xFFFFFFFFu) { out[id * 3] = pc; out[id * 3 + 1] = ct; out[id * 3 + 2] = nr; return; }
    owner[id] = 0xFFFFFFFFu;
    const float4 rp = records[ow * 3], rc = records[ow * 3 + 1], rn = records[ow * 3 + 2];
    const float c_k = pc.w, a = rp.w;
    if (rn.w < (1.0f + 0.5f) * nr.w) {
        float4 op, oc, on;
        op.x = ((c_k * pc.x) + (a * rp.x)) / (c_k + a);
        op.y = ((c_k * pc.y) + (a * rp.y)) / (c_k + a);
        op.z = ((c_k * pc.z) + (a * rp.z)) / (c_k + a);
        op.w = c_k + a;
        const f3 oldc = decode_color(ct.x), newc = decode_color(rc.x);
        oc.x = encode_color(((c_k * oldc.x) + (a * newc.x)) / (c_k + a), ((c_k * oldc.y) + (a * newc.y)) / (c_k + a),
                            ((c_k * oldc.z) + (a * newc.z)) / (c_k + a));
        oc.y = ct.y; oc.z = ct.z; oc.w = (float)time;
        const float n0 = ((c_k * nr.x) + (a * rn.x)) / (c_k + a), n1 = ((c_k * nr.y) + (a * rn.y)) / (c_k + a);
        const float n2 = ((c_k * nr.z) + (a * rn.z)) / (c_k + a), n3 = ((c_k * nr.w) + (a * rn.w)) / (c_k + a);
        const f3 nn = normalized(f3{n0, n1, n2});
        on = make_float4(nn.x, nn.y, nn.z, n3);
        out[id * 3] = op; out[id * 3 + 1] = oc; out[id * 3 + 2] = on;
    } else {
        out[id * 3] = make_float4(pc.x, pc.y, pc.z, c_k + a);
        out[id * 3 + 1] = make_float4(ct.x, ct.y, ct.z, (float)time);
        out[id * 3 + 2] = nr;
    }
}
__global__ void __launch_bounds__(kB) update_kernel(const Batch<UpdateArgs> B) { update_body(B, (int)blockIdx.x); }

static_assert(sizeof(Batch<IndexArgs>) + sizeof(FrameGeom) + sizeof(Batch<ScanArgs>) + 16 <= 4096 && sizeof(Batch<UpdateArgs>) + sizeof(Batch<ScanArgs>) + 16 <= 4096,
              "the side-by-side launches carry two batches' arguments in one 4 KB kernel-argument segment");
__global__ void __launch_bounds__(kB) update_blocksums_kernel(const Batch<UpdateArgs> U, const Batch<ScanArgs> S, int u_blocks)
{
    const int b = (int)blockIdx.x;
    if (b < u_blocks) update_body(U, b);
    else scan_block_sums_body(S, b - u_blocks);
}
__global__ void __launch_bounds__(kB) indexsplat_scatter_kernel(const Batch<IndexArgs> I, const FrameGeom g, const Batch<ScanArgs> S, int i_blocks)
{
    const int b = (int)blockIdx.x;
    if (b < i_blocks) index_splat_body(I, g, b);
    else scan_scatter_body(S, b - i_blocks);
}

struct CleanArgs {
    const unsigned* index; const float4* vertConf; const float4* colorTime;
    const float* depth_filt; const unsigned char* mask;
    Mat4 t_inv; cf_cam cam; int cols, rows, time; float confThreshold, outlierCoeff; int timeDelta, maskID;
    const float4* rec;
    const float4* surfels; const unsigned* count; const float4* fresh; const unsigned* n_fresh; unsigned total_bound; float4* staged; unsigned* flags;
    int xcd;
#ifdef CF_ABLATE
    int abl;
#endif
};

#ifndef CF_CLEAN_B
#define CF_CLEAN_B 64
#endif
static constexpr int kCleanB = CF_CLEAN_B;
static constexpr int kCleanItems = kCleanB / 4;
static constexpr int kCleanStride = 8 * 16 + 1;

__global__ void __launch_bounds__(kCleanB) clean_kernel(const Batch<CleanArgs> B)
{
    __shared__ float s_patch[kCleanItems * kCleanStride];
    const VBlock vb = batch_decode(B.h);
    const CleanArgs& a = B.m[vb.model];
    const float4* __restrict__ surfels = a.surfels; const unsigned* __restrict__ count = a.count; const float4* __restrict__ fresh = a.fresh;
    const unsigned* __restrict__ n_fresh = a.n_fresh; const unsigned total_bound = a.total_bound; float4* __restrict__ staged = a.staged;
    unsigned* __restrict__ flags = a.flags;
    float* const P = s_patch + (threadIdx.x >> 2) * kCleanStride;
    const float4* __restrict__ const rec = a.rec;
    const unsigned gt = (unsigned)xcd_block(a.xcd, vb.bid, vb.nblk) * kCleanB + threadIdx.x;
    const unsigned k = gt >> 2;
    const int sub = (int)(gt & 3u);
    const unsigned n_old = *count, n_all = n_old + *n_fresh;
    const bool exists = k < n_all;
    if (!exists && sub == 0 && k < total_bound) flags[k] = 0;
    const int cols = a.cols, rows = a.rows;
    const float scale = 1.0f;
    float4 pc = make_float4(0, 0, 0, 0), ct = pc, nr = pc;
    f3 localPos{0, 0, 0}, localNorm{0, 0, 0};
    float x = 0, y = 0, x_n = 0, y_n = 0;
    const float stepX = 1.0f / (float)cols, stepY = 1.0f / (float)rows;
    const float indexXStep = stepX * 0.5f / scale, indexYStep = stepY * 0.5f / scale;
    const float windowMultiplier = 2;
    bool window = false;
    if (exists) {
        const float4* src = (k < n_old) ? surfels + (size_t)k * 3 : fresh + (size_t)(k - n_old) * 3;
        pc = src[0]; ct = src[1]; nr = src[2];
        localPos = xform_point(a.t_inv, f3{pc.x, pc.y, pc.z});
        x = ((a.cam.fx * localPos.x) / localPos.z) + a.cam.cx; y = ((a.cam.fy * localPos.y) / localPos.z) + a.cam.cy;
        localNorm = normalized(xform_dir(a.t_inv, f3{nr.x, nr.y, nr.z}));
        x_n = x / (float)cols; y_n = y / (float)rows;
        window = (float)a.time - ct.w < (float)a.timeDelta && localPos.z > 0 && x > 0 && y > 0 && x < (float)cols && y < (float)rows;
    }
    const float iBeg = x_n - (scale * indexXStep * windowMultiplier), jBeg = y_n - (scale * indexYStep * windowMultiplier);
    const int X0 = (int)floorf(iBeg * (float)cols - 0.5f), Y0 = (int)floorf(jBeg * (float)rows - 0.5f);
#ifdef CF_ABLATE
    const int abl = a.abl;
#else
    constexpr int abl = 0;
#endif
    if (window && rec && !(abl & 1)) {
        const int half = sub & 1;
#pragma unroll
        for (int q = 0; q < 8; q++) {
            const int row = q >> 1, tex = (sub >> 1) + 2 * (q & 1), t = row * 4 + tex;
            const int g = iclamp(Y0 + row, 0, rows - 1) * cols + iclamp(X0 + tex, 0, cols - 1);
            const float4 v = rec[2 * g + half];
            float* const o = P + half * 64 + t;
            o[0] = v.x; o[16] = v.y; o[32] = v.z; o[48] = v.w;
        }
    } else
    if (window && !(abl & 1)) {
#pragma unroll
        for (int c = 0; c < 4; c++) {
            const int t = sub * 4 + c;
            const int g = iclamp(Y0 + sub, 0, rows - 1) * cols + iclamp(X0 + c, 0, cols - 1);
            const float4 vcf = a.vertConf[g];
            const float4 ctm = a.colorTime[g];
            const unsigned idx = a.index[g];
            P[0 * 16 + t] = vcf.x; P[1 * 16 + t] = vcf.y; P[2 * 16 + t] = vcf.z; P[3 * 16 + t] = vcf.w;
            P[4 * 16 + t] = ctm.z; P[5 * 16 + t] = ctm.w;
            P[6 * 16 + t] = __uint_as_float(idx);
        }
    }
    __syncthreads();
    if (!exists) return;
    int test = 1;
    int cnt = 0, zCount = 0, violationCount = 0;
    float avgViolation = 0;
    if (window && !(abl & 2)) {
        float i = iBeg;
        for (int s4 = 0; s4 < sub; s4++) i += indexXStep;
        for (; i < x_n + (scale * indexXStep * windowMultiplier); i += indexXStep, i += indexXStep, i += indexXStep, i += indexXStep) {
            for (float j = jBeg; j < y_n + (scale * indexYStep * windowMultiplier); j += indexYStep) {
                const int nlx = (int)floorf(i * (float)cols) - X0, nly = (int)floorf(j * (float)rows) - Y0;
                const unsigned current = ((unsigned)nlx < 4u && (unsigned)nly < 4u)
                                             ? __float_as_uint(P[6 * 16 + nly * 4 + nlx])
                                             : a.index[nearest_texel(j, rows) * cols + nearest_texel(i, cols)];
                if (current > 0U) {
                    float4 vertConf, colorTime;
                    const float fu = i * (float)cols - 0.5f, fv = j * (float)rows - 0.5f;
                    const float x0f = floorf(fu), y0f = floorf(fv);
                    const int lx = (int)x0f - X0, ly = (int)y0f - Y0;
                    if ((unsigned)lx < 3u && (unsigned)ly < 3u) {
                        const float wx = fu - x0f, wy = fv - y0f;
                        const float* q = P + (ly * 4 + lx);
                        vertConf.x = bilerp(q[0 * 16], q[0 * 16 + 1], q[0 * 16 + 4], q[0 * 16 + 5], wx, wy);
                        vertConf.y = bilerp(q[1 * 16], q[1 * 16 + 1], q[1 * 16 + 4], q[1 * 16 + 5], wx, wy);
                        vertConf.z = bilerp(q[2 * 16], q[2 * 16 + 1], q[2 * 16 + 4], q[2 * 16 + 5], wx, wy);
                        vertConf.w = bilerp(q[3 * 16], q[3 * 16 + 1], q[3 * 16 + 4], q[3 * 16 + 5], wx, wy);
                        colorTime.z = bilerp(q[4 * 16], q[4 * 16 + 1], q[4 * 16 + 4], q[4 * 16 + 5], wx, wy);
                        colorTime.w = bilerp(q[5 * 16], q[5 * 16 + 1], q[5 * 16 + 4], q[5 * 16 + 5], wx, wy);
                    } else {
                        vertConf = tex4_linear(a.vertConf, cols, rows, i, j);
                        colorTime = tex4_linear(a.colorTime, cols, rows, i, j);
                    }
                    const float dx = vertConf.x - localPos.x, dy = vertConf.y - localPos.y;
                    if (colorTime.z < ct.z && vertConf.w > a.confThreshold && vertConf.z > localPos.z && vertConf.z - localPos.z < 0.01f &&
                        sqrtf(dx * dx + dy * dy) < nr.w * 1.4f)
                        cnt++;
                    if (colorTime.w == (float)a.time && vertConf.w > a.confThreshold && vertConf.z > localPos.z &&
                        vertConf.z - localPos.z > 0.01f && fabsf(localNorm.z) > 0.85f)
                        zCount++;
                }
            }
        }
    }
    if (window && !(abl & 4)) {
        for (float i = x_n - stepX; i <= x_n + stepX; i += stepX)
            for (float j = y_n - stepY; j <= y_n + stepY; j += stepY) {
                const int tx = nearest_texel(i, cols), ty = nearest_texel(j, rows);
                const int lx = tx - X0, ly = ty - Y0;
                const float dv = (rec && (unsigned)lx < 4u && (unsigned)ly < 4u) ? P[7 * 16 + ly * 4 + lx] : a.depth_filt[ty * cols + tx];
                const float d = dv - localPos.z;
                if (d > 0.03f) { violationCount++; avgViolation += d; }
            }
    }
    cnt += __shfl_xor(cnt, 1, 4); cnt += __shfl_xor(cnt, 2, 4);
    zCount += __shfl_xor(zCount, 1, 4); zCount += __shfl_xor(zCount, 2, 4);
    if (sub != 0) return;
    if (cnt > 8 || zCount > 4) test = 0;
    if (ct.w == -2) ct.w = (float)a.time;
    if ((ct.w == -1 || (((float)a.time - ct.w) > 20 && pc.w < a.confThreshold))) test = 0;
    if (ct.w > 0 && (float)a.time - ct.w > (float)a.timeDelta) test = 1;
    if (violationCount > 0) {
        avgViolation /= (float)violationCount;
        pc.w *= 1.0f / (1 + a.outlierCoeff * avgViolation);
        const int mx = nearest_texel(x_n, cols), my = nearest_texel(y_n, rows);
        const int maskValue = a.mask[my * cols + mx];
        const float wDepth = a.depth_filt[my * cols + mx];
        if (maskValue != a.maskID && (wDepth > localPos.z - 0.05f && wDepth < localPos.z + 0.05f))
            pc.w *= (0.5f + 0.5f * (1 - a.outlierCoeff / 10.0f));
    }
    flags[k] = (unsigned)test;
    staged[(size_t)k * 3] = pc; staged[(size_t)k * 3 + 1] = ct; staged[(size_t)k * 3 + 2] = nr;
}

struct FillArgs { uint4* p; long long n16; };
__global__ void __launch_bounds__(kB) fill_zero_kernel(const Batch<FillArgs> B)
{
    const VBlock vb = batch_decode(B.h);
    const FillArgs& a = B.m[vb.model];
    const long long i = (long long)vb.bid * kB + threadIdx.x;
    if (i < a.n16) a.p[i] = make_uint4(0, 0, 0, 0);
}
__global__ void set_count_kernel(unsigned* out, unsigned v) { *out = v; }
__global__ void set_count2_kernel(unsigned* out, unsigned* out_host, unsigned v) { *out = v; if (out_host) *out_host = v; }

void launch_bilateral(hipStream_t s, const float* depth, int cols, int rows, float maxD, float* out)
{
    bilateral_kernel<<<gridFor((long long)cols * rows), kB, 0, s>>>(depth, cols, rows, maxD, out);
}

static Mat4 mat4_from(const float m[16]) { Mat4 r; for (int i = 0; i < 16; i++) r.m[i] = m[i]; return r; }

void launch_feedback(hipStream_t s, const uint8_t* rgba, const float* depth, int cols, int rows, cf_cam cam, float inv_fx, float inv_fy,
                     const float* tcx, const float* tcy, int time, float maxDepth, float* rec, unsigned* flags)
{
    feedback_kernel<<<gridFor((long long)cols * rows), kB, 0, s>>>(reinterpret_cast<const uchar4*>(rgba), depth, cols, rows, cam.cx, cam.cy, inv_fx,
                                                                   inv_fy, tcx, tcy, time, maxDepth, reinterpret_cast<float4*>(rec), flags);
}
void launch_init(hipStream_t s, const float* raw, const float* filt, const unsigned* raw_count, long long max_n, float* out)
{
    init_kernel<<<gridFor(max_n), kB, 0, s>>>(reinterpret_cast<const float4*>(raw), reinterpret_cast<const float4*>(filt), raw_count,
                                              reinterpret_cast<float4*>(out));
}
static_assert(sizeof(Batch<FuseArgs>) + 16 <= 4096 && sizeof(Batch<CleanArgs>) + 16 <= 4096 && sizeof(Batch<IndexArgs>) + sizeof(FrameGeom) <= 4096 &&
              sizeof(Batch<SplatArgs>) + sizeof(FrameGeom) <= 4096 && sizeof(Batch<ScanArgs>) <= 4096, "lower kSurfBatch");
static IndexArgs index_args(const IndexPassArgs& h)
{
    return IndexArgs{reinterpret_cast<const float4*>(h.surfels), h.count, mat4_from(h.t_inv), h.maxDepth, h.time, h.timeDelta, h.id_begin, h.id_end,
                     h.keys, h.index, reinterpret_cast<float4*>(h.vertConf), reinterpret_cast<float4*>(h.colorTime), reinterpret_cast<float4*>(h.normRad),
                     h.t_inv_dev, reinterpret_cast<float4*>(h.clean_rec), h.clean_depth};
}
void launch_index_keys_batch(hipStream_t s, const IndexPassArgs* items, int n_items, cf_cam cam, int cols, int rows)
{
    const FrameGeom g{cam, cols, rows};
    for (int base = 0; base < n_items; base += kSurfBatch) {
        const int nb = n_items - base < kSurfBatch ? n_items - base : kSurfBatch;
        Batch<IndexArgs> B;
        int blocks[kSurfBatch], any = 0;
        for (int k = 0; k < nb; k++) {
            B.m[k] = index_args(items[base + k]);
            blocks[k] = B.m[k].id_end > B.m[k].id_begin ? gridFor(B.m[k].id_end - B.m[k].id_begin) : 0;
            any += blocks[k];
        }
        if (any) index_splat_kernel<<<batch_layout(B, blocks, nb), kB, 0, s>>>(B, g);
    }
}
void launch_index_resolve_batch(hipStream_t s, const IndexPassArgs* items, int n_items, cf_cam cam, int cols, int rows)
{
    const FrameGeom g{cam, cols, rows};
    for (int base = 0; base < n_items; base += kSurfBatch) {
        const int nb = n_items - base < kSurfBatch ? n_items - base : kSurfBatch;
        Batch<IndexArgs> B;
        int blocks[kSurfBatch];
        for (int k = 0; k < nb; k++) { B.m[k] = index_args(items[base + k]); blocks[k] = gridFor((long long)cols * rows); }
        index_resolve_kernel<<<batch_layout(B, blocks, nb), kB, 0, s>>>(B, g);
    }
}
void launch_index_keys(hipStream_t s, const float* surfels, const unsigned* count, unsigned id_begin, unsigned id_end, const float t_inv[16],
                       cf_cam cam, int cols, int rows, float maxDepth, int time, int timeDelta, unsigned long long* keys)
{
    IndexPassArgs a{};
    a.surfels = surfels; a.count = count; a.id_begin = id_begin; a.id_end = id_end; for (int q = 0; q < 16; q++) a.t_inv[q] = t_inv[q];
    a.maxDepth = maxDepth; a.time = time; a.timeDelta = timeDelta; a.keys = keys;
    launch_index_keys_batch(s, &a, 1, cam, cols, rows);
}
void launch_index_resolve(hipStream_t s, const float* surfels, const float t_inv[16], int cols, int rows, unsigned long long* keys,
                          unsigned* index, float* vertConf, float* colorTime, float* normRad)
{
    IndexPassArgs a{};
    a.surfels = surfels; for (int q = 0; q < 16; q++) a.t_inv[q] = t_inv[q]; a.keys = keys; a.index = index; a.vertConf = vertConf; a.colorTime = colorTime;
    a.normRad = normRad;
    launch_index_resolve_batch(s, &a, 1, cf_cam{}, cols, rows);
}
void launch_predict_indices(hipStream_t s, const float* surfels, const unsigned* count, unsigned count_bound, const float t_inv[16], cf_cam cam,
                            int cols, int rows, float maxDepth, int time, int timeDelta, unsigned long long* keys, unsigned* index,
                            float* vertConf, float* colorTime, float* normRad)
{
    launch_index_keys(s, surfels, count, 0, count_bound, t_inv, cam, cols, rows, maxDepth, time, timeDelta, keys);
    launch_index_resolve(s, surfels, t_inv, cols, rows, keys, index, vertConf, colorTime, normRad);
}
void launch_combined_predict_batch(hipStream_t s, const SplatPassArgs* items, int n_items, cf_cam cam, int cols, int rows)
{
    const FrameGeom g{cam, cols, rows};
    for (int base = 0; base < n_items; base += kSurfBatch) {
        const int nb = n_items - base < kSurfBatch ? n_items - base : kSurfBatch;
        Batch<SplatArgs> B;
        int blocks[kSurfBatch], any = 0;
        for (int k = 0; k < nb; k++) {
            const SplatPassArgs& h = items[base + k];
            B.m[k] = SplatArgs{reinterpret_cast<const float4*>(h.surfels), h.count, mat4_from(h.t_inv), h.maxDepth, h.confThreshold, h.time, h.maxTime,
                               h.timeDelta, reinterpret_cast<const float4*>(h.rays), h.keys, reinterpret_cast<uchar4*>(h.image),
                               reinterpret_cast<float4*>(h.vertexConf), reinterpret_cast<float4*>(h.normalRad), h.time16};
            blocks[k] = h.count_bound > 0 ? gridFor(4ll * h.count_bound) : 0;
            any += blocks[k];
        }
        if (any) splat_raster_kernel<<<batch_layout(B, blocks, nb), kB, 0, s>>>(B, g);
        for (int k = 0; k < nb; k++) blocks[k] = gridFor((long long)cols * rows);
        splat_resolve_kernel<<<batch_layout(B, blocks, nb), kB, 0, s>>>(B, g);
    }
}
void launch_combined_predict(hipStream_t s, const float* surfels, const unsigned* count, unsigned count_bound, const float t_inv[16], cf_cam cam,
                             int cols, int rows, float maxDepth, float confThreshold, int time, int maxTime, int timeDelta,
                             const float* rays, unsigned long long* keys, uint8_t* image, float* vertexConf, float* normalRad,
                             uint16_t* time16)
{
    SplatPassArgs a{};
    a.surfels = surfels; a.count = count; a.count_bound = count_bound; for (int q = 0; q < 16; q++) a.t_inv[q] = t_inv[q]; a.maxDepth = maxDepth;
    a.confThreshold = confThreshold; a.time = time; a.maxTime = maxTime; a.timeDelta = timeDelta; a.rays = rays; a.keys = keys; a.image = image;
    a.vertexConf = vertexConf; a.normalRad = normalRad; a.time16 = time16;
    launch_combined_predict_batch(s, &a, 1, cam, cols, rows);
}
void launch_splat_rays(hipStream_t s, cf_cam cam, int cols, int rows, float* rays)
{
    splat_rays_kernel<<<gridFor((long long)cols * rows), kB, 0, s>>>(cam, cols, rows, reinterpret_cast<float4*>(rays));
}
void launch_fill_in(hipStream_t s, const float* pv, const float* pn, const uint8_t* pimg, const float* depth, const uint8_t* rgba, int cols,
                    int rows, cf_cam cam, float inv_fx, float inv_fy, int pass_geom, int pass_rgb, float* ov, float* on, uint8_t* oi)
{
    fill_in_kernel<<<gridFor((long long)cols * rows), kB, 0, s>>>(
        reinterpret_cast<const float4*>(pv), reinterpret_cast<const float4*>(pn), reinterpret_cast<const uchar4*>(pimg), depth,
        reinterpret_cast<const uchar4*>(rgba), cols, rows, cam.cx, cam.cy, inv_fx, inv_fy, pass_geom, pass_rgb, reinterpret_cast<float4*>(ov),
        reinterpret_cast<float4*>(on), reinterpret_cast<uchar4*>(oi));
}
void launch_fill_ratio(hipStream_t s, const uint8_t* pimg, int cols, int rows, unsigned* out2, unsigned* out2_host)
{
    fill_ratio_kernel<<<1, 1024, 0, s>>>(reinterpret_cast<const uchar4*>(pimg), cols, rows, out2, out2_host);
}
void launch_associate_batch(hipStream_t s, const SurfelFuseArgs* items, int n_items)
{
    const int chunk = xcd_env("CF_XCD_ASSOC", 0);
    for (int base = 0; base < n_items; base += kSurfBatch) {
        const int nb = n_items - base < kSurfBatch ? n_items - base : kSurfBatch;
        Batch<FuseArgs> B;
        Batch<FillArgs> Z;
        int blocks[kSurfBatch], zblocks[kSurfBatch], zany = 0;
        for (int k = 0; k < nb; k++) {
            const SurfelFuseArgs& h = items[base + k];
            FuseArgs& a = B.m[k];
            a.index = h.index; a.vertConf = reinterpret_cast<const float4*>(h.vertConf); a.normRad = reinterpret_cast<const float4*>(h.normRad);
            a.rgba = reinterpret_cast<const uchar4*>(h.rgba); a.depth_raw = h.depth_raw; a.depth_filt = h.depth_filt; a.mask = h.mask;
            a.tcx = h.tcx; a.tcy = h.tcy; a.pose = mat4_from(h.pose); a.cam = h.cam; a.inv_fx = h.inv_fx; a.inv_fy = h.inv_fy;
            a.cols = h.cols; a.rows = h.rows; a.time = h.time; a.weighting = h.weighting; a.maskID = h.maskID; a.maxDepth = h.maxDepth;
            a.records = reinterpret_cast<float4*>(h.records); a.new_flags = h.new_flags; a.owner = h.owner;
            const int par = h.time % 2;
            const long long n = (long long)((h.cols - par + 1) / 2) * ((h.rows - par + 1) / 2);
            blocks[k] = gridXcd(4 * n, chunk);
            const long long n16 = ((long long)h.cols * h.rows + 3) / 4;
            Z.m[k] = FillArgs{reinterpret_cast<uint4*>(h.new_flags), n16};
            zblocks[k] = h.flags_clean ? 0 : gridFor(n16);
            zany += zblocks[k];
        }
        if (zany) fill_zero_kernel<<<batch_layout(Z, zblocks, nb), kB, 0, s>>>(Z);
        associate_kernel<<<batch_layout(B, blocks, nb), kB, 0, s>>>(B, chunk);
    }
}
void launch_associate(hipStream_t s, const SurfelFuseArgs& h) { launch_associate_batch(s, &h, 1); }
void launch_update_batch(hipStream_t s, const UpdatePassArgs* items, int n_items)
{
    for (int base = 0; base < n_items; base += kSurfBatch) {
        const int nb = n_items - base < kSurfBatch ? n_items - base : kSurfBatch;
        Batch<UpdateArgs> B;
        int blocks[kSurfBatch], any = 0;
        for (int k = 0; k < nb; k++) {
            const UpdatePassArgs& h = items[base + k];
            B.m[k] = UpdateArgs{reinterpret_cast<const float4*>(h.in), h.count, h.owner, reinterpret_cast<const float4*>(h.records), h.time,
                                reinterpret_cast<float4*>(h.out)};
            blocks[k] = h.count_bound > 0 ? gridFor(h.count_bound) : 0;
            any += blocks[k];
        }
        if (any) update_kernel<<<batch_layout(B, blocks, nb), kB, 0, s>>>(B);
    }
}
void launch_update(hipStream_t s, const float* in, const unsigned* count, unsigned count_bound, unsigned* owner, const float* records, int time,
                   float* out)
{
    const UpdatePassArgs a{in, count, count_bound, owner, records, time, out};
    launch_update_batch(s, &a, 1);
}
bool launch_update_compaction_index_keys(hipStream_t s, const UpdatePassArgs* up, const ScanPassArgs* sc, const IndexPassArgs* ix, int n, cf_cam cam, int cols,
                                         int rows)
{
    if (n <= 0 || n > kSurfBatch) return false;
    Batch<UpdateArgs> U; Batch<ScanArgs> S; Batch<IndexArgs> I;
    int ub[kSurfBatch], sb[kSurfBatch], ib[kSurfBatch];
    for (int k = 0; k < n; k++) {
        U.m[k] = UpdateArgs{reinterpret_cast<const float4*>(up[k].in), up[k].count, up[k].owner, reinterpret_cast<const float4*>(up[k].records), up[k].time,
                            reinterpret_cast<float4*>(up[k].out)};
        ub[k] = up[k].count_bound > 0 ? gridFor(up[k].count_bound) : 0;
        const ScanPassArgs& h = sc[k];
        S.m[k] = ScanArgs{reinterpret_cast<const float4*>(h.rec), h.flags, h.n, h.block_sums, h.total, h.add_to_total, reinterpret_cast<float4*>(h.out), h.total_host, h.zero_flags};
        sb[k] = (int)((h.n + kScanItems - 1) / kScanItems);
        if (sb[k] == 0) return false;
        I.m[k] = index_args(ix[k]);
        ib[k] = I.m[k].id_end > I.m[k].id_begin ? gridFor(I.m[k].id_end - I.m[k].id_begin) : 0;
    }
    const int ug = batch_layout(U, ub, n), sg = batch_layout(S, sb, n), ig = batch_layout(I, ib, n);
    const FrameGeom g{cam, cols, rows};
    update_blocksums_kernel<<<ug + sg, kB, 0, s>>>(U, S, ug);
    indexsplat_scatter_kernel<<<ig + sg, kB, 0, s>>>(I, g, S, ig);
    return true;
}
void launch_clean_batch(hipStream_t s, const CleanPassArgs* items, int n_items)
{
    const int chunk = xcd_env("CF_XCD_CLEAN", 64);
    for (int base = 0; base < n_items; base += kSurfBatch) {
        const int nb = n_items - base < kSurfBatch ? n_items - base : kSurfBatch;
        Batch<CleanArgs> B;
        int blocks[kSurfBatch], any = 0;
        for (int k = 0; k < nb; k++) {
            const CleanPassArgs& p = items[base + k];
            const SurfelCleanArgs& h = p.h;
            CleanArgs& a = B.m[k];
            a.index = h.index; a.vertConf = reinterpret_cast<const float4*>(h.vertConf); a.colorTime = reinterpret_cast<const float4*>(h.colorTime);
            a.rec = reinterpret_cast<const float4*>(h.rec);
            a.depth_filt = h.depth_filt; a.mask = h.mask; a.t_inv = mat4_from(h.t_inv); a.cam = h.cam; a.cols = h.cols; a.rows = h.rows; a.time = h.time;
            a.confThreshold = h.confThreshold; a.outlierCoeff = h.outlierCoeff; a.timeDelta = h.timeDelta; a.maskID = h.maskID;
            a.surfels = reinterpret_cast<const float4*>(p.surfels); a.count = p.count; a.fresh = reinterpret_cast<const float4*>(p.fresh);
            a.n_fresh = p.n_fresh; a.total_bound = p.total_bound; a.staged = reinterpret_cast<float4*>(p.staged); a.flags = p.flags;
            const int cchunk = chunk * (kB / kCleanB);
            const long long cgrid = (4ll * p.total_bound + kCleanB - 1) / kCleanB;
            a.xcd = cgrid >= 4ll * 8 * cchunk ? cchunk : 0;
#ifdef CF_ABLATE
            static const int clean_abl = getenv("CF_CLEAN_ABLATE") ? atoi(getenv("CF_CLEAN_ABLATE")) : 0;
            a.abl = clean_abl;
#endif
            { const int q = 8 * (a.xcd > 1 ? a.xcd : 1); blocks[k] = p.total_bound > 0 ? (int)((cgrid + q - 1) / q * q) : 0; }
            any += blocks[k];
        }
        if (any) clean_kernel<<<batch_layout(B, blocks, nb), kCleanB, 0, s>>>(B);
    }
}
void launch_clean(hipStream_t s, const float* surfels, const unsigned* count, const float* fresh, const unsigned* n_fresh, unsigned total_bound,
                  const SurfelCleanArgs& h, float* staged, unsigned* flags)
{
    const CleanPassArgs a{h, surfels, count, fresh, n_fresh, total_bound, staged, flags};
    launch_clean_batch(s, &a, 1);
}
void launch_set_count(hipStream_t s, unsigned* out, unsigned v) { set_count_kernel<<<1, 1, 0, s>>>(out, v); }

}
```

co_fusion_amd/lib.py:

```python
from __future__ import annotations

import ctypes as C
import os
import subprocess

_HERE = os.path.dirname(os.path.abspath(__file__))
_LIB_DIR = os.environ.get("CF_LIB_DIR") or os.path.join(_HERE, "lib")
LIB_PATH = os.environ.get("CF_HIP_LIB") or os.path.join(_LIB_DIR, "libcofusion_hip.so")

SYMBOLS = [
    "cf_create", "cf_destroy", "cf_last_error", "cf_set_stream", "cf_use_own_stream", "cf_get_stream", "cf_synchronize", "cf_fork", "cf_main", "cf_join", "cf_join_lane", "cf_thread_lane", "cf_mark", "cf_event_wait_host", "cf_fork_after", "cf_malloc",
    "cf_free", "cf_memcpy_h2d", "cf_memcpy_d2h", "cf_malloc_host", "cf_free_host", "cf_memcpy_h2d_async", "cf_memcpy_d2h_async", "cf_memcpy_d2d_async", "cf_rgb_to_rgba", "cf_create_vmap", "cf_create_nmap", "cf_copy_maps", "cf_resize_map",
    "cf_transform_maps", "cf_vertices_to_depth", "cf_pyrdown_gauss_f32", "cf_pyrdown_gauss_u8",
    "cf_rgba_to_intensity", "cf_sobel", "cf_project_cloud", "cf_icp_step", "cf_icp_step_band", "cf_rgb_residual", "cf_rgb_step",
    "cf_so3_step", "cf_odom_create", "cf_odom_destroy", "cf_odom_init_icp_model", "cf_odom_init_rgb_model",
    "cf_odom_init_rgb", "cf_odom_init_models_batch", "cf_odom_init_models_batch_frames", "cf_odom_init_models_batch_select", "cf_model_fill_ratio_device", "cf_odom_init_first_rgb", "cf_odom_init_icp", "cf_odom_get_incremental_transformation",
    "cf_odom_track_batch_async", "cf_odom_fetch_result", "cf_odom_get_covariance", "cf_odom_bind_frame_maps", "cf_odom_share_frame_maps", "cf_odom_set_culling", "cf_odom_set_band", "cf_set_collective", "cf_model_predict_indices_sharded", "cf_odom_buffer",
    "cf_bilateral", "cf_model_create", "cf_model_destroy", "cf_model_initialise", "cf_model_count",
    "cf_model_predict_indices", "cf_model_index_keys", "cf_model_index_resolve", "cf_model_combined_predict", "cf_model_prefetch_fill_ratio", "cf_model_perform_fill_in", "cf_model_requires_fill_in",
    "cf_model_fuse", "cf_model_clean", "cf_models_frame_passes", "cf_models_preindex", "cf_model_download_map", "cf_model_upload_map", "cf_model_buffer",
    "cf_fusion_weight", "cf_seg_create", "cf_seg_destroy", "cf_seg_slic", "cf_seg_accumulate", "cf_seg_crf", "cf_seg_upsample", "cf_seg_sums", "cf_seg_infer", "cf_seg_run_batch", "cf_seg_fetch", "cf_seg_publish_poses", "cf_seg_fetch_poses",
    "cf_seg_labels",
    "cf_depth_pyramid", "cf_set_icp_launch", "cf_set_icp_arith", "cf_get_icp_arith", "cf_set_gn_mode", "cf_profile_enable", "cf_profile_read", "cf_odom_bench_icp", "cf_odom_level0_visited", "cf_odom_last_launch_shape",
    "cf_rccl_unique_id", "cf_rccl_init", "cf_rccl_allreduce", "cf_rccl_broadcast", "cf_rccl_info", "cf_rccl_destroy",
    "cf_render_create", "cf_render_destroy", "cf_render", "cf_render_palette",
]


def build(verbose: bool = False) -> str:
    cmd = ["make", "-C", os.path.join(_HERE, "csrc"), "-j8"]
    if not verbose:
        cmd.insert(1, "-s")
    subprocess.check_call(cmd)
    cmd = ["make", "-C", os.path.join(_HERE, "host")]
    if not verbose:
        cmd.insert(1, "-s")
    subprocess.check_call(cmd)
    return LIB_PATH


HOST_LIB_PATH = os.path.join(_LIB_DIR, "libcofusion.so")
HOST_SYMBOLS = [
    "cofusion_default_config", "cofusion_create", "cofusion_destroy", "cofusion_last_error", "cofusion_set_stream",
    "cofusion_process_frame", "cofusion_process_frame_device", "cofusion_num_models", "cofusion_tick", "cofusion_model_info",
    "cofusion_model_download", "cofusion_model_icp_stats", "cofusion_model_cull_box", "cofusion_model_level0_visited", "cofusion_model_tracking_inputs", "cofusion_mask_device", "cofusion_context", "cofusion_set_crf",
    "cofusion_save_ply", "cofusion_export_poses", "cofusion_set_export_segmentation", "cofusion_klg_open", "cofusion_klg_next", "cofusion_klg_set_reference_compatible", "cofusion_klg_close",
    "cofusion_klg_create", "cofusion_klg_write", "cofusion_klg_finish", "cofusion_debug_phase_ms", "cofusion_set_allreduce", "cofusion_set_allreduce_device", "cofusion_group_create", "cofusion_group_destroy", "cofusion_group_size", "cofusion_group_sequence", "cofusion_group_set_stream", "cofusion_group_process_frames", "cofusion_group_process_frames_device", "cofusion_rccl_unique_id", "cofusion_init_rccl", "cofusion_broadcast", "cofusion_model_owned", "cofusion_is_lost",
    "cofusion_render", "cofusion_render_device", "cofusion_set_export_views",
]
_host = None


def load_host() -> C.CDLL:
    global _host
    if _host is None:
        load()
        if not os.path.exists(HOST_LIB_PATH):
            raise RuntimeError(f"{HOST_LIB_PATH} is missing: run __graft_entry__.build()")
        _host = C.CDLL(HOST_LIB_PATH)
        _host.cofusion_last_error.restype = C.c_char_p
        _host.cofusion_mask_device.restype = C.c_void_p
        _host.cofusion_context.restype = C.c_void_p
        _host.cofusion_group_sequence.restype = C.c_void_p
    return _host


_lib = None


def load() -> C.CDLL:
    global _lib
    if _lib is None:
        if not os.path.exists(LIB_PATH):
            raise RuntimeError(
                f"{LIB_PATH} is missing: build it with `python -c 'import __graft_entry__ as g; g.build()'` "
                "(there is no CPU fallback for the product path)")
        import torch
        _lib = C.CDLL(LIB_PATH)
        _lib.cf_last_error.restype = C.c_char_p
        _lib.cf_get_stream.restype = C.c_void_p
    return _lib
```

co_fusion_amd/model.py:

```python
from __future__ import annotations

import ctypes as C

import numpy as np
import torch

from .api import Context, Odometry, _f, _p

SURFEL = 12
TIME_DELTA = 2 ** 31 // 2 - 1

_BUF = {0: (np.uint32, 1), 1: (np.float32, 4), 2: (np.float32, 4), 3: (np.float32, 4), 4: (np.uint8, 4), 5: (np.float32, 4),
        6: (np.float32, 4), 7: (np.uint16, 1), 8: (np.float32, 4), 9: (np.float32, 4), 10: (np.uint8, 4)}


def bilateral(ctx: Context, depth, max_d):
    rows, cols = depth.shape
    out = ctx.empty((rows, cols))
    ctx._check(ctx.lib.cf_bilateral(ctx.h, _p(depth), cols, rows, C.c_float(max_d), _p(out)))
    return out


def fusion_weight(ctx: Context, pose, last_pose, mult):
    ctx.lib.cf_fusion_weight.restype = C.c_float
    return float(ctx.lib.cf_fusion_weight(_f(np.asarray(pose, np.float32).reshape(16)), _f(np.asarray(last_pose, np.float32).reshape(16)),
                                          C.c_float(mult)))


class Model:
    def __init__(self, ctx: Context, max_surfels=1 << 20):
        self.ctx = ctx
        self.h = C.c_void_p()
        ctx._check(ctx.lib.cf_model_create(ctx.h, int(max_surfels), C.byref(self.h)))

    def close(self):
        if getattr(self, "h", None) and self.ctx.h:
            self.ctx.lib.cf_model_destroy(self.h)
        self.h = None

    def __del__(self):
        try:
            self.close()
        except Exception:
            pass

    def _pose(self, pose):
        return _f(np.asarray(pose, np.float32).reshape(16))

    def initialise(self, rgba, depth_raw, depth_filt, time, max_depth):
        self.ctx._check(self.ctx.lib.cf_model_initialise(self.h, _p(rgba), _p(depth_raw), _p(depth_filt), time, C.c_float(max_depth)))

    def count(self):
        c = C.c_uint32()
        self.ctx._check(self.ctx.lib.cf_model_count(self.h, C.byref(c)))
        return c.value

    def predict_indices(self, pose, time, max_depth, time_delta=TIME_DELTA):
        self.ctx._check(self.ctx.lib.cf_model_predict_indices(self.h, self._pose(pose), time, C.c_float(max_depth), time_delta))

    def index_keys(self, pose, time, max_depth, surfel_begin, surfel_end, time_delta=TIME_DELTA):
        keys = torch.empty((self.ctx.height, self.ctx.width), dtype=torch.int64, device=self.ctx.device)
        self.ctx._check(self.ctx.lib.cf_model_index_keys(self.h, self._pose(pose), time, C.c_float(max_depth), time_delta,
                                                         int(surfel_begin), int(surfel_end), C.c_void_p(keys.data_ptr())))
        return keys

    def index_resolve(self, pose, keys):
        self.ctx._check(self.ctx.lib.cf_model_index_resolve(self.h, self._pose(pose), C.c_void_p(keys.data_ptr())))

    def combined_predict(self, pose, max_depth, conf_threshold, time, max_time, time_delta=TIME_DELTA):
        self.ctx._check(self.ctx.lib.cf_model_combined_predict(self.h, self._pose(pose), C.c_float(max_depth), C.c_float(conf_threshold),
                                                               time, max_time, time_delta))

    def perform_fill_in(self, rgba, depth_filt, pass_geom=False, pass_rgb=False):
        self.ctx._check(self.ctx.lib.cf_model_perform_fill_in(self.h, _p(rgba), _p(depth_filt), int(pass_geom), int(pass_rgb)))

    def requires_fill_in(self, ratio=0.75):
        out = C.c_int()
        self.ctx._check(self.ctx.lib.cf_model_requires_fill_in(self.h, C.c_float(ratio), C.byref(out)))
        return bool(out.value)

    def fuse(self, pose, time, rgba, mask, depth_raw, depth_filt, max_depth, weighting, mask_id):
        self.ctx._check(self.ctx.lib.cf_model_fuse(self.h, self._pose(pose), time, _p(rgba), _p(mask), _p(depth_raw), _p(depth_filt),
                                                   C.c_float(max_depth), C.c_float(weighting), mask_id))

    def clean(self, pose, time, conf_threshold, outlier_coeff, depth_filt, mask, mask_id, time_delta=TIME_DELTA):
        c = C.c_uint32()
        self.ctx._check(self.ctx.lib.cf_model_clean(self.h, self._pose(pose), time, C.c_float(conf_threshold), C.c_float(outlier_coeff),
                                                    time_delta, _p(depth_filt), _p(mask), mask_id, C.byref(c)))
        return c.value

    def download_map(self):
        n = self.count()
        out = np.zeros((max(n, 1), SURFEL), np.float32)
        c = C.c_uint32()
        self.ctx._check(self.ctx.lib.cf_model_download_map(self.h, out.ctypes.data_as(C.c_void_p), n, C.byref(c)))
        return out[:n]

    def upload_map(self, surfels):
        s = np.ascontiguousarray(surfels, np.float32).reshape(-1, SURFEL)
        self.ctx._check(self.ctx.lib.cf_model_upload_map(self.h, s.ctypes.data_as(C.c_void_p), s.shape[0]))

    def tensor(self, which):
        ptr = C.c_void_p(); nbytes = C.c_uint64()
        self.ctx._check(self.ctx.lib.cf_model_buffer(self.h, which, C.byref(ptr), C.byref(nbytes)))
        return ptr.value, nbytes.value

    def buffer(self, which):
        ptr, nbytes = self.tensor(which)
        host = np.empty(nbytes, np.uint8)
        self.ctx._check(self.ctx.lib.cf_memcpy_d2h(self.ctx.h, host.ctypes.data_as(C.c_void_p), C.c_void_p(ptr), C.c_uint64(nbytes)))
        h, w = self.ctx.height, self.ctx.width
        if which == 11:
            return host.view(np.float32).reshape(-1, SURFEL)
        dt, ch = _BUF[which]
        a = host.view(dt)
        return a.reshape(h, w, ch) if ch > 1 else a.reshape(h, w)


class _DevView:

    def __init__(self, ptr):
        self._ptr = ptr
        self.is_cuda = True

    def is_contiguous(self):
        return True

    def data_ptr(self):
        return self._ptr
```

include/cofusion_hip.h:

```cpp
#ifndef COFUSION_HIP_H_
#define COFUSION_HIP_H_

#include <stdint.h>

#ifdef __cplusplus
extern "C" {
#endif

#define CF_OK 0
#define CF_EINVAL (-1)
#define CF_EHIP (-2)
#define CF_ENOMEM (-3)
#define CF_ESTATE (-4)

#define CF_NUM_PYRS 3
#define CF_SE3_WORDS 32
#define CF_SO3_WORDS 16
#define CF_FIX_ICP 32
#define CF_FIX_RGB_MAX 32
static inline int CF_FIX_RGB_BITS(float sigma)
{
    union { float f; uint32_t u; } v;
    int F;
    if (sigma == -1.0f || !(sigma >= 2.0f)) return 8;
    v.f = sigma;
    F = 8 + 2 * ((int)((v.u >> 23) & 255u) - 127);
    return F > CF_FIX_RGB_MAX ? CF_FIX_RGB_MAX : F;
}
#define CF_FIX_SO3 12

typedef struct cf_ctx cf_ctx;
typedef struct cf_odom cf_odom;
typedef struct cf_model cf_model;

typedef struct { float fx, fy, cx, cy; } cf_cam;

typedef struct {
    float x, y, z, conf;
    float colour24, unused, init_time, last_time;
    float nx, ny, nz, radius;
} cf_surfel;
#ifdef __cplusplus
static_assert(sizeof(cf_surfel) == 48, "surfel record is 3 x float4");
#else
_Static_assert(sizeof(cf_surfel) == 48, "surfel record is 3 x float4");
#endif

typedef struct {
    int16_t zero_x, zero_y;
    int16_t one_x, one_y;
    float diff;
    int32_t valid;
} cf_dataterm;

typedef struct {
    int width, height;
    float fx, fy, cx, cy;
    int device;
    int max_models;
    int max_surfels;
} cf_config;

int cf_create(const cf_config *cfg, cf_ctx **out);
void cf_destroy(cf_ctx *ctx);
const char *cf_last_error(const cf_ctx *ctx);
int cf_set_stream(cf_ctx *ctx, void *hip_stream);
int cf_use_own_stream(cf_ctx *ctx);
void *cf_get_stream(cf_ctx *ctx);
int cf_synchronize(cf_ctx *ctx);
int cf_fork(cf_ctx *ctx, int lane);
int cf_main(cf_ctx *ctx);
int cf_join(cf_ctx *ctx);
int cf_join_lane(cf_ctx *ctx, int lane);
int cf_thread_lane(cf_ctx *ctx, int lane);
int cf_mark(cf_ctx *ctx, int slot);
int cf_event_wait_host(cf_ctx *ctx, int slot);
int cf_fork_after(cf_ctx *ctx, int lane, int slot);
int cf_malloc(cf_ctx *ctx, uint64_t bytes, void **dptr);
int cf_free(cf_ctx *ctx, void *dptr);
int cf_memcpy_h2d(cf_ctx *ctx, void *dst, const void *src, uint64_t bytes);
int cf_memcpy_d2h(cf_ctx *ctx, void *dst, const void *src, uint64_t bytes);
int cf_malloc_host(cf_ctx *ctx, uint64_t bytes, void **hptr);
int cf_free_host(cf_ctx *ctx, void *hptr);
int cf_memcpy_h2d_async(cf_ctx *ctx, void *dst, const void *src_pinned, uint64_t bytes);
int cf_memcpy_d2h_async(cf_ctx *ctx, void *dst_pinned, const void *src, uint64_t bytes);
int cf_memcpy_d2d_async(cf_ctx *ctx, void *dst, const void *src, uint64_t bytes);
int cf_rgb_to_rgba(cf_ctx *ctx, const uint8_t *rgb_dev, int cols, int rows, uint8_t *rgba_dev);

int cf_create_vmap(cf_ctx *ctx, const float *depth, int cols, int rows, cf_cam intr, float depth_cutoff, float *vmap);
int cf_create_nmap(cf_ctx *ctx, const float *vmap, int cols, int rows, float *nmap);
int cf_copy_maps(cf_ctx *ctx, const float *vertex4, const float *normal4, int cols, int rows, float *vmap, float *nmap);
int cf_resize_map(cf_ctx *ctx, const float *in, int in_cols, int in_rows, float *out, int normalize);
int cf_transform_maps(cf_ctx *ctx, float *vmap, float *nmap, int cols, int rows, const float R[9], const float t[3]);
int cf_vertices_to_depth(cf_ctx *ctx, const float *vertex4, int cols, int rows, float cutoff, float *depth);
int cf_pyrdown_gauss_f32(cf_ctx *ctx, const float *src, int src_cols, int src_rows, float *dst);
int cf_pyrdown_gauss_u8(cf_ctx *ctx, const uint8_t *src, int src_cols, int src_rows, uint8_t *dst);
int cf_rgba_to_intensity(cf_ctx *ctx, const uint8_t *rgba, int cols, int rows, uint8_t *dst);
int cf_sobel(cf_ctx *ctx, const uint8_t *src, int cols, int rows, int16_t *dx, int16_t *dy);
int cf_project_cloud(cf_ctx *ctx, const float *depth, int cols, int rows, cf_cam intr_level, float *cloud3);

int cf_icp_step(cf_ctx *ctx, const float Rcurr[9], const float tcurr[3], const float *vmap_curr,
                const float *nmap_curr, const float Rprev_inv[9], const float tprev[3], cf_cam intr,
                const float *vmap_g_prev, const float *nmap_g_prev, float dist_thres, float angle_thres,
                int cols, int rows, float *A_host, float *b_host, float *residual_host, int64_t *sums_host,
                float *err_surface);
int cf_icp_step_band(cf_ctx *ctx, const float Rcurr[9], const float tcurr[3], const float *vmap_curr,
                     const float *nmap_curr, const float Rprev_inv[9], const float tprev[3], cf_cam intr,
                     const float *vmap_g_prev, const float *nmap_g_prev, float dist_thres, float angle_thres,
                     int cols, int rows, int row_begin, int row_end, float *A_host, float *b_host,
                     float *residual_host, int64_t *sums_host, float *err_surface);
int cf_rgb_residual(cf_ctx *ctx, float min_scale, const int16_t *dIdx, const int16_t *dIdy, const float *last_depth,
                    const float *next_depth, const uint8_t *last_image, const uint8_t *next_image,
                    cf_dataterm *corres, float max_depth_delta, const float kt[3], const float krkinv[9],
                    int cols, int rows, int *sigma_sum_host, int *count_host);
int cf_rgb_step(cf_ctx *ctx, const cf_dataterm *corres, float sigma, const float *cloud3, float fx, float fy,
                const int16_t *dIdx, const int16_t *dIdy, float sobel_scale, int cols, int rows, float *A_host,
                float *b_host, int64_t *sums_host);
int cf_so3_step(cf_ctx *ctx, const uint8_t *last_image, const uint8_t *next_image, const float image_basis[9],
                const float kinv[9], const float krlr[9], int cols, int rows, float *A_host, float *b_host,
                float *residual_host, int64_t *sums_host);

typedef struct {
    int rgb_only, pyramid, fast_odom, so3;
    float icp_weight;
} cf_track_opts;
typedef struct {
    float last_icp_error, last_icp_count, last_rgb_error, last_rgb_count, last_so3_error, last_so3_count;
    double lastA[36], lastb[6];
    int so3_iterations;
    int fault;
    int cull_box[4];
} cf_track_stats;

int cf_odom_create(cf_ctx *ctx, cf_odom **out);
void cf_odom_destroy(cf_odom *od);
int cf_odom_init_icp_model(cf_odom *od, const float *pred_vertex4, const float *pred_normal4, const float pose[16]);
int cf_odom_init_rgb_model(cf_odom *od, const uint8_t *pred_rgba);
int cf_odom_init_rgb(cf_odom *od, const uint8_t *rgba);
int cf_odom_init_first_rgb(cf_odom *od, const uint8_t *rgba);
int cf_odom_init_models_batch(cf_ctx *ctx, cf_odom *const *ods, int n, const float *const *pred_vertex4,
                              const float *const *pred_normal4, const uint8_t *const *pred_rgba, const float *const *poses ,
                              const uint8_t *frame_rgba);
int cf_odom_init_models_batch_frames(cf_ctx *ctx, cf_odom *const *ods, int n, const float *const *pred_vertex4,
                                     const float *const *pred_normal4, const uint8_t *const *pred_rgba, const float *const *poses ,
                                     const uint8_t *const *frame_rgba );
int cf_odom_init_models_batch_select(cf_ctx *ctx, cf_odom *const *ods, int n, const float *const *pred_vertex4,
                                     const float *const *pred_normal4, const uint8_t *const *pred_rgba,
                                     const float *const *alt_vertex4, const float *const *alt_normal4, const uint8_t *const *alt_rgba,
                                     const uint32_t *const *fill_counts, float ratio, const float *const *poses ,
                                     const uint8_t *const *frame_rgba );
int cf_odom_init_icp(cf_odom *od, const float *const depth_pyr[CF_NUM_PYRS], float depth_cutoff);
int cf_odom_get_incremental_transformation(cf_odom *od, float trans[3], float rot[9], const cf_track_opts *opts,
                                           float *icp_err_surface, cf_track_stats *stats);
int cf_odom_track_batch_async(cf_ctx *ctx, cf_odom *const *ods, int n, const float *const *poses_in ,
                              const cf_track_opts *opts, float *const *icp_err_surfaces );
int cf_odom_fetch_result(cf_odom *od, float trans[3], float rot[9], cf_track_stats *stats);
int cf_odom_get_covariance(const cf_track_stats *stats, double cov[36]);
int cf_odom_level0_visited(cf_odom *od, uint64_t *icp_pixels, uint64_t *residual_pixels);
int cf_odom_last_launch_shape(cf_odom *od, int icp_blocks[3], int residual_blocks[3], int *icp_blocks_err);
int cf_odom_set_culling(cf_odom *od, int on);
typedef int (*cf_collective_fn)(void *user, int op, void *dev_buf, uint64_t words, void *hip_stream);
int cf_set_collective(cf_ctx *ctx, cf_collective_fn fn, void *user);
int cf_odom_set_band(cf_odom *od, int row_begin, int row_end, int add_counts);
#define CF_RCCL_ID_BYTES 128
int cf_rccl_unique_id(void *id128);
int cf_rccl_init(cf_ctx *ctx, const void *id128, int rank, int world);
int cf_rccl_allreduce(cf_ctx *ctx, void *dev_buf, uint64_t words, int op, void *hip_stream);
int cf_rccl_broadcast(cf_ctx *ctx, void *dev_buf, uint64_t bytes, int root, void *hip_stream);
int cf_rccl_info(const cf_ctx *ctx, int *rank, int *world, int *rccl_version);
int cf_rccl_destroy(cf_ctx *ctx);
int cf_odom_bind_frame_maps(cf_odom *od, const float *const vmaps[CF_NUM_PYRS], const float *const nmaps[CF_NUM_PYRS]);
int cf_odom_share_frame_maps(cf_odom *od, cf_odom *owner);
int cf_odom_buffer(cf_odom *od, int which, int level, void **dptr, uint64_t *bytes);
int cf_depth_pyramid(cf_ctx *ctx, const float *depth_filtered, int cols, int rows, float *l1, float *l2);

int cf_bilateral(cf_ctx *ctx, const float *depth, int cols, int rows, float maxD, float *out);

int cf_model_create(cf_ctx *ctx, int max_surfels, cf_model **out);
void cf_model_destroy(cf_model *m);
int cf_model_initialise(cf_model *m, const uint8_t *rgba, const float *depth_raw, const float *depth_filtered, int time,
                        float maxDepth);
int cf_model_count(cf_model *m, uint32_t *count);
int cf_model_predict_indices(cf_model *m, const float pose[16], int time, float maxDepth, int timeDelta);
int cf_model_index_keys(cf_model *m, const float pose[16], int time, float maxDepth, int timeDelta, uint32_t surfel_begin,
                        uint32_t surfel_end, uint64_t *keys_dev);
int cf_model_index_resolve(cf_model *m, const float pose[16], uint64_t *keys_dev);
int cf_model_predict_indices_sharded(cf_model *m, const float pose[16], int time, float maxDepth, int timeDelta, int shard, int nshards);
int cf_model_combined_predict(cf_model *m, const float pose[16], float maxDepth, float confThreshold, int time, int maxTime,
                              int timeDelta);
int cf_model_prefetch_fill_ratio(cf_model *m);
int cf_model_perform_fill_in(cf_model *m, const uint8_t *rgba, const float *depth_filtered, int passthrough_geom,
                             int passthrough_rgb);
int cf_model_requires_fill_in(cf_model *m, float ratio, int *out);
int cf_model_fill_ratio_device(cf_model *m, const uint32_t **counts_dev);
int cf_model_fuse(cf_model *m, const float pose[16], int time, const uint8_t *rgba, const uint8_t *mask, const float *depth_raw,
                  const float *depth_filtered, float maxDepth, float weighting, int maskID);
int cf_model_clean(cf_model *m, const float pose[16], int time, float confThreshold, float outlierCoeff, int timeDelta,
                   const float *depth_filtered, const uint8_t *mask, int maskID, uint32_t *count_out);
typedef struct {
    cf_model *model;
    const float *pose;
    const uint8_t *rgba, *mask;
    const float *depth_raw, *depth_filtered;
    int do_fuse;
    int time;
    float fuse_max_depth;
    float weighting;
    int mask_id;
    float conf_threshold;
} cf_model_pass;
int cf_models_frame_passes(cf_ctx *ctx, const cf_model_pass *items, int n, float depth_cutoff, float outlier_coeff, int time_delta);
typedef struct {
    cf_model *model;
    const cf_odom *odom;
    int time;
} cf_model_preindex;
int cf_models_preindex(cf_ctx *ctx, const cf_model_preindex *items, int n, float depth_cutoff, int time_delta);
int cf_model_download_map(cf_model *m, float *host_surfels, uint32_t capacity, uint32_t *count);
int cf_model_upload_map(cf_model *m, const float *host_surfels, uint32_t count);
int cf_model_buffer(cf_model *m, int which, void **dptr, uint64_t *bytes);
float cf_fusion_weight(const float pose[16], const float lastPose[16], float weightMultiplier);

typedef struct cf_segmenter cf_segmenter;
int cf_seg_create(cf_ctx *ctx, cf_segmenter **out);
void cf_seg_destroy(cf_segmenter *s);
int cf_seg_slic(cf_segmenter *s, const uint8_t *rgba);
int cf_seg_accumulate(cf_segmenter *s, const float *depth, int n_models, const float *const *icp_err,
                      const float *const *vertconf4, uint32_t *spix_count_host, uint32_t *depth_count_host,
                      int64_t *depth_sum_host, int64_t *icp_sum_host, int64_t *conf_sum_host, int32_t *resample_labels_host);
int cf_seg_crf(cf_segmenter *s, const float *unary_host, int L, const float *feat_smooth_host, const float *feat_app_host,
               float w_smooth, float w_app, int iterations, float *Q_host);
int cf_seg_upsample(cf_segmenter *s, const uint8_t *low_map_host, uint8_t *full_dev);
typedef struct {
    float unaryWeightError, unaryKError, unaryThresholdNew;
    float weightAppearance, weightSmoothness;
    float scaleFeaturesRGB, scaleFeaturesDepth, scaleFeaturesPos;
    float minRelSizeNew, maxRelSizeNew;
    int crfIterations;
} cf_seg_params;
#define CF_SEG_MAX_ENTRIES 256
typedef struct {
    uint32_t id, superPixelCount;
    float avgConfidence, depthMean, depthStd;
    int32_t top, right, bottom, left;
} cf_seg_model;
typedef struct {
    int32_t has_new_label, n_models;
    float depth_range;
    cf_seg_model model[CF_SEG_MAX_ENTRIES];
} cf_seg_result;
int cf_seg_sums(cf_segmenter *s, const float *depth, int n_models, const float *const *icp_err, const float *const *vertconf4,
                int64_t **sums_dev, uint64_t *sums_words);
int cf_seg_infer(cf_segmenter *s, const cf_seg_params *params, const uint8_t *rgba, int n_models, const uint32_t *model_ids,
                 uint32_t next_model_id, int allow_new, uint8_t *full_dev);
int cf_seg_fetch(cf_segmenter *s, cf_seg_result *out, uint8_t *low_map_host);
typedef struct cf_seg_job {
    cf_segmenter *seg;
    const float *depth;
    int32_t n_models;
    const float *const *icp_err;
    const float *const *vertconf4;
    const uint8_t *rgba;
    const uint32_t *model_ids;
    uint32_t next_model_id;
    int32_t allow_new;
    uint8_t *full_dev;
} cf_seg_job;
int cf_seg_run_batch(cf_ctx *ctx, const cf_seg_params *params, const cf_seg_job *jobs, int n_jobs);
int cf_seg_publish_poses(cf_segmenter *s, int n_models, cf_odom *const *trackers);
int cf_seg_fetch_poses(cf_segmenter *s, int n_models, int64_t *words_host);
int cf_seg_labels(cf_segmenter *s, void **dptr, uint64_t *bytes);

int cf_set_gn_mode(cf_ctx *ctx, int mode);
int cf_set_icp_launch(cf_ctx *ctx, int threads, int pixels_per_thread);
#define CF_ICP_ARITH_PRODUCT 0
#define CF_ICP_ARITH_GRAM 1
#define CF_ICP_ARITH_REFERENCE 2
int cf_set_icp_arith(cf_ctx *ctx, int mode);
int cf_get_icp_arith(cf_ctx *ctx);

typedef struct cf_renderer cf_renderer;
#define CF_RENDER_MAX_ITEMS 256
#define CF_RENDER_MAX_COLOUR 8
#define CF_RENDER_UNSTABLE 1
#define CF_RENDER_WINDOW 2
#define CF_RENDER_PHONG 4
#define CF_RENDER_GREY 0
#define CF_RENDER_NORMALS 1
#define CF_RENDER_COLOUR 2
#define CF_RENDER_TIMES 3
#define CF_RENDER_LABEL 4
#define CF_RENDER_ITEM_MODE (-1)
#define CF_RENDER_RGBA 0
#define CF_RENDER_DEPTH 1
#define CF_RENDER_LABELS 2
typedef struct {
    float pose[16];
    float fx, fy, cx, cy;
    int width, height;
    float near_z, far_z;
    int flags;
    int tick, time_delta;
} cf_render_view;
typedef struct {
    const float *surfels;
    uint32_t count;
    float pose[16];
    float conf_threshold;
    int model_id;
    int colour_mode;
} cf_render_item;
typedef struct {
    void *dst;
    int kind;
    int mode;
} cf_render_output;
int cf_render_create(cf_ctx *ctx, int max_w, int max_h, cf_renderer **out);
void cf_render_destroy(cf_renderer *r);
int cf_render(cf_renderer *r, const cf_render_view *view, const cf_render_item *items, int n_items, const cf_render_output *outputs,
              int n_outputs);
int cf_render_palette(uint8_t *rgb768);

int cf_odom_bench_icp(cf_odom *od, int level, int iters, float *avg_us);

typedef struct {
    double icp_ms_total;
    uint64_t icp_launches;
    uint64_t icp_bytes;
    double surfel_ms_total;
    uint64_t surfel_calls;
    uint64_t surfel_bytes;
} cf_profile;
int cf_profile_enable(cf_ctx *ctx, int on);
int cf_profile_read(cf_ctx *ctx, cf_profile *out, int reset);

#ifdef __cplusplus
}
#endif
#endif
```

Measured before the change: 889.1.

## Track projected bounding box in index splat and skip plane writes outside it

The index splat kernel now reduces each wavefront's projected pixel extent and atomically grows a per-model bounding box stored after the clean record buffer, double-buffered across two slots. By default the frame chain no longer writes the separate index/vertConf/colorTime/normRad planes. Resolve and the fuse and clean kernels read the packed clean record instead, treating texels outside the box as empty. The aim is to cut resolve, clearing and plane traffic for models that cover only part of the frame. The cost is extra shuffles and atomics in the splat, state tracking that makes the standalone fuse, clean and buffer APIs error until predict_indices is called, and a fallback to the old path via environment variables.

Measured after the change: 643.4. 27.6% lower.

```diff
diff --git a/co_fusion_amd/csrc/cabi_model.hip b/co_fusion_amd/csrc/cabi_model.hip
--- a/co_fusion_amd/csrc/cabi_model.hip
+++ b/co_fusion_amd/csrc/cabi_model.hip
@@ -48,6 +48,9 @@
     unsigned* index = nullptr;
     float *vertConf = nullptr, *colorTime = nullptr, *normRad = nullptr;
     float* clean_rec = nullptr;
+    unsigned box_seq = 0;
+    int box_slot = -1;
+    bool planes_valid = true;
     uint8_t* splat_image = nullptr;
     float *splat_vertex = nullptr, *splat_normal = nullptr;
     uint16_t* splat_time = nullptr;
@@ -115,7 +118,12 @@
     if (int r = dmalloc(ctx, &m->vertConf, N * 4)) return r;
     if (int r = dmalloc(ctx, &m->colorTime, N * 4)) return r;
     if (int r = dmalloc(ctx, &m->normRad, N * 4)) return r;
-    if (int r = dmalloc(ctx, &m->clean_rec, N * 8)) return r;
+    if (int r = dmalloc(ctx, &m->clean_rec, texel_rec_floats(N))) return r;
+    {
+        const int empty[8] = {0x7fffffff, 0x7fffffff, -1, -1, 0x7fffffff, 0x7fffffff, -1, -1};
+        HIPCHK(ctx, hipMemcpyAsync(texel_boxes(m->clean_rec, N), empty, sizeof(empty), hipMemcpyHostToDevice, ctx->cur()));
+        HIPCHK(ctx, hipStreamSynchronize(ctx->cur()));
+    }
     if (int r = dmalloc(ctx, &m->splat_image, N * 4)) return r;
     if (int r = dmalloc(ctx, &m->splat_vertex, N * 4)) return r;
     if (int r = dmalloc(ctx, &m->splat_normal, N * 4)) return r;
@@ -234,6 +242,7 @@
     launch_predict_indices(ctx->cur(), m->buf[m->target], m->d_count, nb, t_inv, ctx_cam(ctx), ctx->cfg.width, ctx->cfg.height,
                            maxDepth, time, timeDelta, m->keys, m->index, m->vertConf, m->colorTime, m->normRad);
     LAUNCHCHK(ctx);
+    m->planes_valid = true; m->box_slot = -1;
     return CF_OK;
 }
 
@@ -264,6 +273,7 @@
     launch_index_resolve(ctx->cur(), m->buf[m->target], t_inv, ctx->cfg.width, ctx->cfg.height, reinterpret_cast<unsigned long long*>(keys_dev),
                          m->index, m->vertConf, m->colorTime, m->normRad);
     LAUNCHCHK(ctx);
+    m->planes_valid = true; m->box_slot = -1;
     return CF_OK;
 }
 
@@ -347,6 +357,7 @@
                   const float* depth_filt, float maxDepth, float weighting, int maskID)
 {
     if (!m || !pose || !rgba || !mask || !depth_raw || !depth_filt) return CF_EINVAL;
+    if (!m->planes_valid) { m->ctx->set_error("cf_model_fuse: needs cf_model_predict_indices first (the frame chain leaves no index-map planes)"); return CF_ESTATE; }
     m->drop_preindex();
     cf_ctx* ctx = m->ctx; hipStream_t s = ctx->cur();
     const int W = ctx->cfg.width, H = ctx->cfg.height; const long long N = (long long)W * H;
@@ -374,6 +385,7 @@
                    const uint8_t* mask, int maskID, uint32_t* count_out)
 {
     if (!m || !pose || !depth_filt || !mask) return CF_EINVAL;
+    if (!m->planes_valid) { m->ctx->set_error("cf_model_clean: needs cf_model_predict_indices first (the frame chain leaves no index-map planes)"); return CF_ESTATE; }
     m->drop_preindex();
     cf_ctx* ctx = m->ctx; hipStream_t s = ctx->cur();
     const int W = ctx->cfg.width, H = ctx->cfg.height;
@@ -395,6 +407,23 @@
     return CF_OK;
 }
 
+static bool index_planes_on() { static const bool on = getenv("CF_INDEX_PLANES") != nullptr || getenv("CF_NO_CLEAN_REC") != nullptr; return on; }
+static void frame_index_outputs(cf_model* m, IndexPassArgs& p, bool feeds_clean, const float* depth_filtered)
+{
+    static const bool clean_rec_on = getenv("CF_NO_CLEAN_REC") == nullptr;
+    p.index = m->index; p.vertConf = m->vertConf; p.colorTime = m->colorTime; p.normRad = m->normRad;
+    if (index_planes_on()) {
+        p.flags = kIxPlanes;
+        if (feeds_clean && clean_rec_on) { p.clean_rec = m->clean_rec; p.clean_depth = depth_filtered; }
+        m->planes_valid = true; m->box_slot = -1;
+        return;
+    }
+    const int slot = (int)(m->box_seq++ & 1u);
+    p.flags = kIxBox | (slot ? kIxSlot1 : 0) | (feeds_clean ? 0 : kIxAssocRec);
+    p.clean_rec = m->clean_rec; p.clean_depth = feeds_clean ? depth_filtered : nullptr;
+    m->planes_valid = false; m->box_slot = slot;
+}
+
 int cf_models_preindex(cf_ctx* ctx, const cf_model_preindex* items, int n, float depth_cutoff, int time_delta)
 {
     if (!ctx || !items || n <= 0) return CF_EINVAL;
@@ -409,7 +438,8 @@
         const float* pinv = reinterpret_cast<const float*>(reinterpret_cast<const char*>(od->d_state) + offsetof(cf::OdomDev, pose_inv));
         IndexPassArgs& p = a[k];
         p.surfels = m->buf[m->target]; p.count = m->d_count; p.id_begin = 0; p.id_end = nb; p.maxDepth = depth_cutoff; p.time = items[k].time;
-        p.timeDelta = time_delta; p.keys = m->keys; p.index = m->index; p.vertConf = m->vertConf; p.colorTime = m->colorTime; p.normRad = m->normRad;
+        p.timeDelta = time_delta; p.keys = m->keys;
+        frame_index_outputs(m, p, false, nullptr);
         p.t_inv_dev = pinv;
     }
     launch_index_keys_batch(s, a.data(), n, ctx_cam(ctx), W, H);
@@ -464,6 +494,7 @@
         ctx->surf_calls++;
     }
     static const bool clean_rec_on = getenv("CF_NO_CLEAN_REC") == nullptr;
+    const bool planes_on = index_planes_on();
     auto index_args_of = [&](const std::vector<int>& which, bool feeds_clean, std::vector<IndexPassArgs>& a) -> int {
         a.assign(which.size(), IndexPassArgs{});
         for (size_t q = 0; q < which.size(); q++) {
@@ -472,9 +503,8 @@
             if (int r = count_bound(m, &nb)) return r;
             IndexPassArgs& p = a[q];
             p.surfels = m->buf[m->target]; p.count = m->d_count; p.id_begin = 0; p.id_end = nb; inv44f(it.pose, p.t_inv); p.maxDepth = depth_cutoff;
-            p.time = it.time; p.timeDelta = time_delta; p.keys = m->keys; p.index = m->index; p.vertConf = m->vertConf; p.colorTime = m->colorTime;
-            p.normRad = m->normRad;
-            if (feeds_clean && clean_rec_on) { p.clean_rec = m->clean_rec; p.clean_depth = it.depth_filtered; }
+            p.time = it.time; p.timeDelta = time_delta; p.keys = m->keys;
+            frame_index_outputs(m, p, feeds_clean, it.depth_filtered);
         }
         return CF_OK;
     };
@@ -503,6 +533,7 @@
             const cf_model_pass& it = items[fusing[q]]; cf_model* m = it.model;
             SurfelFuseArgs& a = fa[q];
             a.index = m->index; a.vertConf = m->vertConf; a.normRad = m->normRad; a.rgba = it.rgba; a.depth_raw = it.depth_raw; a.depth_filt = it.depth_filtered;
+            a.rec = planes_on ? nullptr : m->clean_rec; a.box_slot = m->box_slot;
             a.mask = it.mask; a.tcx = m->tcx; a.tcy = m->tcy; memcpy(a.pose, it.pose, sizeof(a.pose)); a.cam = cam; a.inv_fx = m->inv_fx;
             a.inv_fy = m->inv_fy; a.cols = W; a.rows = H; a.time = it.time; a.weighting = it.weighting; a.maskID = it.mask_id; a.maxDepth = it.fuse_max_depth;
             a.records = m->records; a.new_flags = m->new_flags; a.owner = m->owner; a.flags_clean = m->new_flags_clean ? 1 : 0;
@@ -536,7 +567,7 @@
             if (bound > m->max_surfels + (unsigned)(W * H / 4 + 64)) return CF_ENOMEM;
             CleanPassArgs& c = ca[q];
             c.h.index = m->index; c.h.vertConf = m->vertConf; c.h.colorTime = m->colorTime; c.h.depth_filt = it.depth_filtered; c.h.mask = it.mask;
-            c.h.rec = clean_rec_on ? m->clean_rec : nullptr;
+            c.h.rec = clean_rec_on ? m->clean_rec : nullptr; c.h.box_slot = m->box_slot;
             inv44f(it.pose, c.h.t_inv); c.h.cam = cam; c.h.cols = W; c.h.rows = H; c.h.time = it.time; c.h.confThreshold = it.conf_threshold;
             c.h.outlierCoeff = outlier_coeff; c.h.timeDelta = time_delta; c.h.maskID = it.mask_id;
             c.surfels = m->buf[m->target]; c.count = m->d_count; c.fresh = m->fresh; c.n_fresh = m->d_nfresh; c.total_bound = bound; c.staged = m->staged;
@@ -605,6 +636,10 @@
     if (!m || !dptr) return CF_EINVAL;
     const size_t N = (size_t)m->ctx->cfg.width * m->ctx->cfg.height;
     void* p = nullptr; size_t b = 0;
+    if (which >= 0 && which <= 3 && !m->planes_valid) {
+        m->ctx->set_error("cf_model_buffer: the index-map planes are written by cf_model_predict_indices / cf_model_index_resolve only; the last index pass was the frame chain's");
+        return CF_ESTATE;
+    }
     switch (which) {
         case 0: p = m->index; b = N * 4; break;
         case 1: p = m->vertConf; b = N * 16; break;
@@ -621,6 +656,19 @@
         default: return CF_EINVAL;
     }
     *dptr = p; if (bytes) *bytes = b;
+    return CF_OK;
+}
+
+int cf_model_index_box(cf_model* m, int box[4], int* culled, uint32_t* passes)
+{
+    if (!m || !box || !culled) return CF_EINVAL;
+    if (passes) *passes = m->box_seq;
+    cf_ctx* ctx = m->ctx;
+    const int W = ctx->cfg.width, H = ctx->cfg.height;
+    *culled = m->box_slot >= 0 ? 1 : 0;
+    if (m->box_slot < 0) { box[0] = 0; box[1] = 0; box[2] = W - 1; box[3] = H - 1; return CF_OK; }
+    HIPCHK(ctx, hipMemcpyAsync(box, texel_boxes(m->clean_rec, (size_t)W * H) + 4 * m->box_slot, 4 * sizeof(int), hipMemcpyDeviceToHost, ctx->cur()));
+    HIPCHK(ctx, hipStreamSynchronize(ctx->cur()));
     return CF_OK;
 }
 
diff --git a/co_fusion_amd/csrc/cf_kernels.h b/co_fusion_amd/csrc/cf_kernels.h
--- a/co_fusion_amd/csrc/cf_kernels.h
+++ b/co_fusion_amd/csrc/cf_kernels.h
@@ -272,12 +272,17 @@
 float sqrt_gate_le(float T);
 
 constexpr int kSurfBatch = 16;
+enum : int { kIxPlanes = 1, kIxAssocRec = 2, kIxBox = 4, kIxSlot1 = 8 };
+struct TexelBox { int x0, y0, x1, y1; };
+constexpr size_t texel_rec_floats(size_t n_texels) { return n_texels * 8 + 8; }
+__host__ __device__ inline int* texel_boxes(const float* rec, size_t n_texels) { return reinterpret_cast<int*>(const_cast<float*>(rec) + n_texels * 8); }
 struct IndexPassArgs {
     const float* surfels; const unsigned* count; unsigned id_begin, id_end; float t_inv[16]; float maxDepth; int time, timeDelta;
     unsigned long long* keys; unsigned* index; float* vertConf; float* colorTime; float* normRad;
     const float* t_inv_dev;
     float* clean_rec;
     const float* clean_depth;
+    int flags;
 };
 __host__ __device__ inline void inv44f(const float a[16], float o[16])
 {
@@ -303,6 +308,8 @@
 struct UpdatePassArgs { const float* in; const unsigned* count; unsigned count_bound; unsigned* owner; const float* records; int time; float* out; };
 struct SurfelFuseArgs {
     const unsigned* index; const float* vertConf; const float* normRad;
+    const float* rec = nullptr;
+    int box_slot = -1;
     const uint8_t* rgba; const float* depth_raw; const float* depth_filt; const uint8_t* mask;
     const float* tcx; const float* tcy;
     float pose[16]; cf_cam cam; float inv_fx, inv_fy;
@@ -314,6 +321,7 @@
     const unsigned* index; const float* vertConf; const float* colorTime;
     const float* depth_filt; const uint8_t* mask;
     const float* rec;
+    int box_slot = -1;
     float t_inv[16]; cf_cam cam; int cols, rows, time; float confThreshold, outlierCoeff; int timeDelta, maskID;
 };
 struct CleanPassArgs {
diff --git a/co_fusion_amd/csrc/cf_surfel_device.h b/co_fusion_amd/csrc/cf_surfel_device.h
--- a/co_fusion_amd/csrc/cf_surfel_device.h
+++ b/co_fusion_amd/csrc/cf_surfel_device.h
@@ -87,14 +87,15 @@
               T.m[8] * p.x + T.m[9] * p.y + T.m[10] * p.z};
 }
 
-__device__ __forceinline__ float4 tex4_linear(const float4* __restrict__ img, int cols, int rows, float u, float v)
+template <class Texel>
+__device__ __forceinline__ float4 tex4_linear_with(Texel texel, int cols, int rows, float u, float v)
 {
     const float fu = u * (float)cols - 0.5f, fv = v * (float)rows - 0.5f;
     const float x0f = floorf(fu), y0f = floorf(fv);
     const float wx = fu - x0f, wy = fv - y0f;
     const int x0 = iclamp((int)x0f, 0, cols - 1), x1 = iclamp((int)x0f + 1, 0, cols - 1);
     const int y0 = iclamp((int)y0f, 0, rows - 1), y1 = iclamp((int)y0f + 1, 0, rows - 1);
-    const float4 a = img[y0 * cols + x0], b = img[y0 * cols + x1], c = img[y1 * cols + x0], d = img[y1 * cols + x1];
+    const float4 a = texel(x0, y0), b = texel(x1, y0), c = texel(x0, y1), d = texel(x1, y1);
     float4 r;
     {
         const float top = a.x * (1.0f - wx) + b.x * wx, bot = c.x * (1.0f - wx) + d.x * wx;
@@ -113,6 +114,10 @@
         r.w = top * (1.0f - wy) + bot * wy;
     }
     return r;
+}
+__device__ __forceinline__ float4 tex4_linear(const float4* __restrict__ img, int cols, int rows, float u, float v)
+{
+    return tex4_linear_with([img, cols](int x, int y) { return img[y * cols + x]; }, cols, rows, u, v);
 }
 
 __device__ __forceinline__ f3 get_vertex(const float* __restrict__ depth, int cols, int rows, int px, int py, float x, float y,
diff --git a/co_fusion_amd/csrc/surfel.hip b/co_fusion_amd/csrc/surfel.hip
--- a/co_fusion_amd/csrc/surfel.hip
+++ b/co_fusion_amd/csrc/surfel.hip
@@ -247,23 +247,32 @@
 }
 
 __device__ __forceinline__ bool index_project(const float4 pc, const float4 ct, const Mat4& t_inv, cf_cam cam, int cols, int rows,
-                                              float maxDepth, int time, int timeDelta, f3& ph, int& q)
+                                              float maxDepth, int time, int timeDelta, f3& ph, int& px, int& py)
 {
     ph = xform_point(t_inv, f3{pc.x, pc.y, pc.z});
     if (ph.z > maxDepth || ph.z < 0 || (float)time - ct.w > (float)timeDelta) return false;
     const float u = ((cam.fx * ph.x) / ph.z) + cam.cx, v = ((cam.fy * ph.y) / ph.z) + cam.cy;
     if (!(u >= 0.0f && v >= 0.0f && u < (float)cols && v < (float)rows)) return false;
     if (!(ph.z < maxDepth)) return false;
-    q = (int)floorf(v) * cols + (int)floorf(u);
+    px = (int)floorf(u); py = (int)floorf(v);
     return true;
 }
 
 struct IndexArgs {
     const float4* surfels; const unsigned* count; Mat4 t_inv; float maxDepth; int time, timeDelta; unsigned id_begin, id_end;
+    int flags;
     unsigned long long* keys; unsigned* index; float4* vertConf; float4* colorTime; float4* normRad;
     const float* t_inv_dev;
     float4* clean_rec; const float* clean_depth;
 };
+static_assert(sizeof(IndexArgs) == 168, "IndexArgs: sixteen of them, a FrameGeom and a Batch<ScanArgs> share one kernel-argument segment");
+__device__ __forceinline__ TexelBox load_texel_box(const float4* rec, int n, int slot, int cols, int rows)
+{
+    if (slot < 0) return TexelBox{0, 0, cols - 1, rows - 1};
+    const int4 b = *reinterpret_cast<const int4*>(texel_boxes(reinterpret_cast<const float*>(rec), (size_t)n) + 4 * slot);
+    return TexelBox{b.x, b.y, b.z, b.w};
+}
+__device__ __forceinline__ bool box_has(const TexelBox& b, int x, int y) { return x >= b.x0 && x <= b.x1 && y >= b.y0 && y <= b.y1; }
 __device__ __forceinline__ Mat4 index_matrix(const IndexArgs& a)
 {
     if (!a.t_inv_dev) return a.t_inv;
@@ -280,11 +289,27 @@
     const IndexArgs& a = B.m[vb.model];
     const float4* __restrict__ surfels = a.surfels;
     const unsigned id = a.id_begin + vb.bid * kB + threadIdx.x;
-    if (id >= *a.count || id >= a.id_end) return;
-    f3 ph; int q;
-    const Mat4 T = index_matrix(a);
-    if (!index_project(surfels[id * 3], surfels[id * 3 + 1], T, g.cam, g.cols, g.rows, a.maxDepth, a.time, a.timeDelta, ph, q)) return;
-    atomicMin(&a.keys[q], zkey(ph.z, id));
+    bool hit = id < *a.count && id < a.id_end;
+    f3 ph; int px = 0, py = 0;
+    if (hit) {
+        const Mat4 T = index_matrix(a);
+        hit = index_project(surfels[id * 3], surfels[id * 3 + 1], T, g.cam, g.cols, g.rows, a.maxDepth, a.time, a.timeDelta, ph, px, py);
+    }
+    if (hit) atomicMin(&a.keys[py * g.cols + px], zkey(ph.z, id));
+    if (!(a.flags & kIxBox)) return;
+    if (__ballot(hit) == 0) return;
+    int x0 = hit ? px : 0x7fffffff, y0 = hit ? py : 0x7fffffff, x1 = hit ? px : -1, y1 = hit ? py : -1;
+#pragma unroll
+    for (int o = 32; o > 0; o >>= 1) {
+        x0 = min(x0, __shfl_xor(x0, o, 64)); y0 = min(y0, __shfl_xor(y0, o, 64));
+        x1 = max(x1, __shfl_xor(x1, o, 64)); y1 = max(y1, __shfl_xor(y1, o, 64));
+    }
+    if ((threadIdx.x & 63) != 0) return;
+    int* const box = texel_boxes(reinterpret_cast<const float*>(a.clean_rec), (size_t)g.cols * g.rows) + ((a.flags & kIxSlot1) ? 4 : 0);
+    if (x0 < __hip_atomic_load(&box[0], __ATOMIC_RELAXED, __HIP_MEMORY_SCOPE_AGENT)) atomicMin(&box[0], x0);
+    if (y0 < __hip_atomic_load(&box[1], __ATOMIC_RELAXED, __HIP_MEMORY_SCOPE_AGENT)) atomicMin(&box[1], y0);
+    if (x1 > __hip_atomic_load(&box[2], __ATOMIC_RELAXED, __HIP_MEMORY_SCOPE_AGENT)) atomicMax(&box[2], x1);
+    if (y1 > __hip_atomic_load(&box[3], __ATOMIC_RELAXED, __HIP_MEMORY_SCOPE_AGENT)) atomicMax(&box[3], y1);
 }
 __global__ void __launch_bounds__(kB) index_splat_kernel(const Batch<IndexArgs> B, const FrameGeom g) { index_splat_body(B, g, (int)blockIdx.x); }
 
@@ -292,17 +317,31 @@
 {
     const VBlock vb = batch_decode(B.h);
     const IndexArgs& a = B.m[vb.model];
-    const float4* __restrict__ surfels = a.surfels; unsigned long long* __restrict__ keys = a.keys; unsigned* __restrict__ index = a.index;
-    float4* __restrict__ vertConf = a.vertConf; float4* __restrict__ colorTime = a.colorTime; float4* __restrict__ normRad = a.normRad;
+    const float4* __restrict__ surfels = a.surfels; unsigned long long* __restrict__ keys = a.keys;
+    float4* __restrict__ const rec = a.clean_rec;
+    const int flags = a.flags, n = g.cols * g.rows;
     const int q = vb.bid * kB + threadIdx.x;
-    if (q >= g.cols * g.rows) return;
+    if (flags & kIxBox) {
+        int* const boxes = texel_boxes(reinterpret_cast<const float*>(rec), (size_t)n);
+        const int slot = (flags & kIxSlot1) ? 1 : 0;
+        if (vb.bid == 0 && threadIdx.x < 4) boxes[4 * (1 - slot) + threadIdx.x] = threadIdx.x < 2 ? 0x7fffffff : -1;
+        const TexelBox b = load_texel_box(rec, n, slot, g.cols, g.rows);
+        const int q0 = vb.bid * kB, q1 = min(q0 + kB, n) - 1;
+        if (q0 >= n || b.x1 < b.x0) return;
+        const int r0 = q0 / g.cols, r1 = q1 / g.cols;
+        if (r1 < b.y0 || r0 > b.y1) return;
+        if (r0 == r1 && (q1 - r0 * g.cols < b.x0 || q0 - r0 * g.cols > b.x1)) return;
+        if (q >= n) return;
+        const int y = q / g.cols, x = q - y * g.cols;
+        if (!box_has(b, x, y)) return;
+    }
+    if (q >= n) return;
     const unsigned long long k = keys[q];
     keys[q] = kEmptyKey;
-    float4* __restrict__ const rec = a.clean_rec;
-    const float dflt = rec ? a.clean_depth[q] : 0.f;
+    const bool planes = flags & kIxPlanes, assoc = flags & kIxAssocRec;
+    const float dflt = (rec && !assoc) ? a.clean_depth[q] : 0.f;
     if (k == kEmptyKey) {
-        index[q] = 0;
-        vertConf[q] = colorTime[q] = normRad[q] = make_float4(0, 0, 0, 0);
+        if (planes) { a.index[q] = 0; a.vertConf[q] = a.colorTime[q] = a.normRad[q] = make_float4(0, 0, 0, 0); }
         if (rec) { rec[2 * q] = make_float4(0, 0, 0, 0); rec[2 * q + 1] = make_float4(0, 0, __uint_as_float(0u), dflt); }
         return;
     }
@@ -310,12 +349,15 @@
     const float4 pc = surfels[id * 3], ct = surfels[id * 3 + 1], nr = surfels[id * 3 + 2];
     const Mat4 T = index_matrix(a);
     const f3 ph = xform_point(T, f3{pc.x, pc.y, pc.z});
-    const f3 n = normalized(xform_dir(T, f3{nr.x, nr.y, nr.z}));
-    index[q] = id;
-    vertConf[q] = make_float4(ph.x, ph.y, ph.z, pc.w);
-    colorTime[q] = ct;
-    normRad[q] = make_float4(n.x, n.y, n.z, nr.w);
-    if (rec) { rec[2 * q] = make_float4(ph.x, ph.y, ph.z, pc.w); rec[2 * q + 1] = make_float4(ct.z, ct.w, __uint_as_float(id), dflt); }
+    const f3 nn = normalized(xform_dir(T, f3{nr.x, nr.y, nr.z}));
+    if (planes) {
+        a.index[q] = id;
+        a.vertConf[q] = make_float4(ph.x, ph.y, ph.z, pc.w);
+        a.colorTime[q] = ct;
+        a.normRad[q] = make_float4(nn.x, nn.y, nn.z, nr.w);
+    }
+    if (rec && assoc) { rec[2 * q] = make_float4(ph.x, ph.y, ph.z, __uint_as_float(id)); rec[2 * q + 1] = make_float4(nn.x, nn.y, nn.z, 0.f); }
+    else if (rec) { rec[2 * q] = make_float4(ph.x, ph.y, ph.z, pc.w); rec[2 * q + 1] = make_float4(ct.z, ct.w, __uint_as_float(id), dflt); }
 }
 
 struct SplatSetup { f3 ph, n; float rad, pn; int x_lo, x_hi, y_lo, y_hi; };
@@ -493,6 +535,7 @@
 
 struct FuseArgs {
     const unsigned* index; const float4* vertConf; const float4* normRad;
+    const float4* rec; int box_slot;
     const uchar4* rgba; const float* depth_raw; const float* depth_filt; const unsigned char* mask;
     const float* tcx; const float* tcy;
     Mat4 pose; cf_cam cam; float inv_fx, inv_fy;
@@ -547,6 +590,22 @@
     const float windowMultiplier = 2;
     const float iBeg = tcx - (scale * indexXStep * windowMultiplier), jBeg = tcy - (scale * indexYStep * windowMultiplier);
     const int X0 = (int)floorf(iBeg * (float)cols - 0.5f), Y0 = (int)floorf(jBeg * (float)rows - 0.5f);
+    const float4* __restrict__ const rec = a.rec;
+    const TexelBox bx = load_texel_box(rec, cols * rows, rec ? a.box_slot : -1, cols, rows);
+    const auto rec_half = [rec, bx, cols](int tx, int ty, int half) {
+        const float4 v = rec[2 * (ty * cols + tx) + half];
+        return box_has(bx, tx, ty) ? v : make_float4(0, 0, 0, 0);
+    };
+    if (alive && rec) {
+        const int half = sub & 1;
+#pragma unroll
+        for (int p8 = 0; p8 < 8; p8++) {
+            const int row = p8 >> 1, tex = (sub >> 1) + 2 * (p8 & 1), k = row * 4 + tex;
+            const float4 v = rec_half(iclamp(X0 + tex, 0, cols - 1), iclamp(Y0 + row, 0, rows - 1), half);
+            if (half == 0) { P[0 * 16 + k] = v.x; P[1 * 16 + k] = v.y; P[2 * 16 + k] = v.z; P[6 * 16 + k] = v.w; }
+            else { P[3 * 16 + k] = v.x; P[4 * 16 + k] = v.y; P[5 * 16 + k] = v.z; }
+        }
+    } else
     if (alive) {
 #pragma unroll
         for (int c = 0; c < 4; c++) {
@@ -580,7 +639,8 @@
             const int nlx = (int)floorf(ii * (float)cols) - X0, nly = (int)floorf(jj * (float)rows) - Y0;
             const unsigned current = ((unsigned)nlx < 4u && (unsigned)nly < 4u)
                                          ? __float_as_uint(P[6 * 16 + nly * 4 + nlx])
-                                         : a.index[nearest_texel(jj, rows) * cols + nearest_texel(ii, cols)];
+                                         : rec ? __float_as_uint(rec_half(nearest_texel(ii, cols), nearest_texel(jj, rows), 0).w)
+                                               : a.index[nearest_texel(jj, rows) * cols + nearest_texel(ii, cols)];
             if (current > 0U) {
                 const float fu = ii * (float)cols - 0.5f, fv = jj * (float)rows - 0.5f;
                 const float x0f = floorf(fu), y0f = floorf(fv);
@@ -593,7 +653,9 @@
                     vertConf.x = bilerp(qd[0 * 16], qd[0 * 16 + 1], qd[0 * 16 + 4], qd[0 * 16 + 5], wx, wy);
                     vertConf.y = bilerp(qd[1 * 16], qd[1 * 16 + 1], qd[1 * 16 + 4], qd[1 * 16 + 5], wx, wy);
                     vertConf.z = bilerp(qd[2 * 16], qd[2 * 16 + 1], qd[2 * 16 + 4], qd[2 * 16 + 5], wx, wy);
-                } else
+                } else if (rec)
+                    vertConf = tex4_linear_with([&](int tx, int ty) { return rec_half(tx, ty, 0); }, cols, rows, ii, jj);
+                else
                     vertConf = tex4_linear(a.vertConf, cols, rows, ii, jj);
                 const float zdiff = (vertConf.z - vPosLocal.z);
                 if (fabsf(zdiff * lambda) < 0.05f) {
@@ -603,7 +665,9 @@
                         normRad.x = bilerp(qd[3 * 16], qd[3 * 16 + 1], qd[3 * 16 + 4], qd[3 * 16 + 5], wx, wy);
                         normRad.y = bilerp(qd[4 * 16], qd[4 * 16 + 1], qd[4 * 16 + 4], qd[4 * 16 + 5], wx, wy);
                         normRad.z = bilerp(qd[5 * 16], qd[5 * 16 + 1], qd[5 * 16 + 4], qd[5 * 16 + 5], wx, wy);
-                    } else
+                    } else if (rec)
+                        normRad = tex4_linear_with([&](int tx, int ty) { return rec_half(tx, ty, 1); }, cols, rows, ii, jj);
+                    else
                         normRad = tex4_linear(a.normRad, cols, rows, ii, jj);
                     if (dist < bestDist && (fabsf(normRad.z) < 0.75f || fabsf(angle_between(f3{normRad.x, normRad.y, normRad.z}, vNormLocal)) < 0.5f)) {
                         operation = 1; bestDist = dist; best = current; bestSeq = outer * 64 + inner;
@@ -691,6 +755,7 @@
     const float* depth_filt; const unsigned char* mask;
     Mat4 t_inv; cf_cam cam; int cols, rows, time; float confThreshold, outlierCoeff; int timeDelta, maskID;
     const float4* rec;
+    int box_slot;
     const float4* surfels; const unsigned* count; const float4* fresh; const unsigned* n_fresh; unsigned total_bound; float4* staged; unsigned* flags;
     int xcd;
 #ifdef CF_ABLATE
@@ -746,13 +811,20 @@
 #else
     constexpr int abl = 0;
 #endif
+    const TexelBox bx = load_texel_box(rec, cols * rows, rec ? a.box_slot : -1, cols, rows);
+    const float* __restrict__ const depth_filt = a.depth_filt;
+    const auto rec_half = [rec, bx, cols, depth_filt](int tx, int ty, int half) {
+        const int g = ty * cols + tx;
+        float4 v = rec[2 * g + half];
+        if (!box_has(bx, tx, ty)) v = make_float4(0, 0, 0, half ? depth_filt[g] : 0.f);
+        return v;
+    };
     if (window && rec && !(abl & 1)) {
         const int half = sub & 1;
 #pragma unroll
         for (int q = 0; q < 8; q++) {
             const int row = q >> 1, tex = (sub >> 1) + 2 * (q & 1), t = row * 4 + tex;
-            const int g = iclamp(Y0 + row, 0, rows - 1) * cols + iclamp(X0 + tex, 0, cols - 1);
-            const float4 v = rec[2 * g + half];
+            const float4 v = rec_half(iclamp(X0 + tex, 0, cols - 1), iclamp(Y0 + row, 0, rows - 1), half);
             float* const o = P + half * 64 + t;
             o[0] = v.x; o[16] = v.y; o[32] = v.z; o[48] = v.w;
         }
@@ -783,7 +855,8 @@
                 const int nlx = (int)floorf(i * (float)cols) - X0, nly = (int)floorf(j * (float)rows) - Y0;
                 const unsigned current = ((unsigned)nlx < 4u && (unsigned)nly < 4u)
                                              ? __float_as_uint(P[6 * 16 + nly * 4 + nlx])
-                                             : a.index[nearest_texel(j, rows) * cols + nearest_texel(i, cols)];
+                                             : rec ? __float_as_uint(rec_half(nearest_texel(i, cols), nearest_texel(j, rows), 1).z)
+                                                   : a.index[nearest_texel(j, rows) * cols + nearest_texel(i, cols)];
                 if (current > 0U) {
                     float4 vertConf, colorTime;
                     const float fu = i * (float)cols - 0.5f, fv = j * (float)rows - 0.5f;
@@ -798,6 +871,10 @@
                         vertConf.w = bilerp(q[3 * 16], q[3 * 16 + 1], q[3 * 16 + 4], q[3 * 16 + 5], wx, wy);
                         colorTime.z = bilerp(q[4 * 16], q[4 * 16 + 1], q[4 * 16 + 4], q[4 * 16 + 5], wx, wy);
                         colorTime.w = bilerp(q[5 * 16], q[5 * 16 + 1], q[5 * 16 + 4], q[5 * 16 + 5], wx, wy);
+                    } else if (rec) {
+                        vertConf = tex4_linear_with([&](int tx, int ty) { return rec_half(tx, ty, 0); }, cols, rows, i, j);
+                        const float4 zw = tex4_linear_with([&](int tx, int ty) { return rec_half(tx, ty, 1); }, cols, rows, i, j);
+                        colorTime = make_float4(0, 0, zw.x, zw.y);
                     } else {
                         vertConf = tex4_linear(a.vertConf, cols, rows, i, j);
                         colorTime = tex4_linear(a.colorTime, cols, rows, i, j);
@@ -877,7 +954,7 @@
 static IndexArgs index_args(const IndexPassArgs& h)
 {
     return IndexArgs{reinterpret_cast<const float4*>(h.surfels), h.count, mat4_from(h.t_inv), h.maxDepth, h.time, h.timeDelta, h.id_begin, h.id_end,
-                     h.keys, h.index, reinterpret_cast<float4*>(h.vertConf), reinterpret_cast<float4*>(h.colorTime), reinterpret_cast<float4*>(h.normRad),
+                     h.flags, h.keys, h.index, reinterpret_cast<float4*>(h.vertConf), reinterpret_cast<float4*>(h.colorTime), reinterpret_cast<float4*>(h.normRad),
                      h.t_inv_dev, reinterpret_cast<float4*>(h.clean_rec), h.clean_depth};
 }
 void launch_index_keys_batch(hipStream_t s, const IndexPassArgs* items, int n_items, cf_cam cam, int cols, int rows)
@@ -919,7 +996,7 @@
 {
     IndexPassArgs a{};
     a.surfels = surfels; for (int q = 0; q < 16; q++) a.t_inv[q] = t_inv[q]; a.keys = keys; a.index = index; a.vertConf = vertConf; a.colorTime = colorTime;
-    a.normRad = normRad;
+    a.normRad = normRad; a.flags = kIxPlanes;
     launch_index_resolve_batch(s, &a, 1, cf_cam{}, cols, rows);
 }
 void launch_predict_indices(hipStream_t s, const float* surfels, const unsigned* count, unsigned count_bound, const float t_inv[16], cf_cam cam,
@@ -988,6 +1065,7 @@
             const SurfelFuseArgs& h = items[base + k];
             FuseArgs& a = B.m[k];
             a.index = h.index; a.vertConf = reinterpret_cast<const float4*>(h.vertConf); a.normRad = reinterpret_cast<const float4*>(h.normRad);
+            a.rec = reinterpret_cast<const float4*>(h.rec); a.box_slot = h.box_slot;
             a.rgba = reinterpret_cast<const uchar4*>(h.rgba); a.depth_raw = h.depth_raw; a.depth_filt = h.depth_filt; a.mask = h.mask;
             a.tcx = h.tcx; a.tcy = h.tcy; a.pose = mat4_from(h.pose); a.cam = h.cam; a.inv_fx = h.inv_fx; a.inv_fy = h.inv_fy;
             a.cols = h.cols; a.rows = h.rows; a.time = h.time; a.weighting = h.weighting; a.maskID = h.maskID; a.maxDepth = h.maxDepth;
@@ -1062,7 +1140,7 @@
             const SurfelCleanArgs& h = p.h;
             CleanArgs& a = B.m[k];
             a.index = h.index; a.vertConf = reinterpret_cast<const float4*>(h.vertConf); a.colorTime = reinterpret_cast<const float4*>(h.colorTime);
-            a.rec = reinterpret_cast<const float4*>(h.rec);
+            a.rec = reinterpret_cast<const float4*>(h.rec); a.box_slot = h.box_slot;
             a.depth_filt = h.depth_filt; a.mask = h.mask; a.t_inv = mat4_from(h.t_inv); a.cam = h.cam; a.cols = h.cols; a.rows = h.rows; a.time = h.time;
             a.confThreshold = h.confThreshold; a.outlierCoeff = h.outlierCoeff; a.timeDelta = h.timeDelta; a.maskID = h.maskID;
             a.surfels = reinterpret_cast<const float4*>(p.surfels); a.count = p.count; a.fresh = reinterpret_cast<const float4*>(p.fresh);
diff --git a/co_fusion_amd/lib.py b/co_fusion_amd/lib.py
--- a/co_fusion_amd/lib.py
+++ b/co_fusion_amd/lib.py
@@ -18,7 +18,7 @@
     "cf_odom_track_batch_async", "cf_odom_fetch_result", "cf_odom_get_covariance", "cf_odom_bind_frame_maps", "cf_odom_share_frame_maps", "cf_odom_set_culling", "cf_odom_set_band", "cf_set_collective", "cf_model_predict_indices_sharded", "cf_odom_buffer",
     "cf_bilateral", "cf_model_create", "cf_model_destroy", "cf_model_initialise", "cf_model_count",
     "cf_model_predict_indices", "cf_model_index_keys", "cf_model_index_resolve", "cf_model_combined_predict", "cf_model_prefetch_fill_ratio", "cf_model_perform_fill_in", "cf_model_requires_fill_in",
-    "cf_model_fuse", "cf_model_clean", "cf_models_frame_passes", "cf_models_preindex", "cf_model_download_map", "cf_model_upload_map", "cf_model_buffer",
+    "cf_model_fuse", "cf_model_clean", "cf_models_frame_passes", "cf_models_preindex", "cf_model_index_box", "cf_model_download_map", "cf_model_upload_map", "cf_model_buffer",
     "cf_fusion_weight", "cf_seg_create", "cf_seg_destroy", "cf_seg_slic", "cf_seg_accumulate", "cf_seg_crf", "cf_seg_upsample", "cf_seg_sums", "cf_seg_infer", "cf_seg_run_batch", "cf_seg_fetch", "cf_seg_publish_poses", "cf_seg_fetch_poses",
     "cf_seg_labels",
     "cf_depth_pyramid", "cf_set_icp_launch", "cf_set_icp_arith", "cf_get_icp_arith", "cf_set_gn_mode", "cf_profile_enable", "cf_profile_read", "cf_odom_bench_icp", "cf_odom_level0_visited", "cf_odom_last_launch_shape",
diff --git a/co_fusion_amd/model.py b/co_fusion_amd/model.py
--- a/co_fusion_amd/model.py
+++ b/co_fusion_amd/model.py
@@ -89,6 +89,11 @@
                                                     time_delta, _p(depth_filt), _p(mask), mask_id, C.byref(c)))
         return c.value
 
+    def index_box(self):
+        box = (C.c_int * 4)(); culled = C.c_int(); passes = C.c_uint32()
+        self.ctx._check(self.ctx.lib.cf_model_index_box(self.h, box, C.byref(culled), C.byref(passes)))
+        return tuple(box), bool(culled.value), passes.value
+
     def download_map(self):
         n = self.count()
         out = np.zeros((max(n, 1), SURFEL), np.float32)
diff --git a/include/cofusion_hip.h b/include/cofusion_hip.h
--- a/include/cofusion_hip.h
+++ b/include/cofusion_hip.h
@@ -216,6 +216,7 @@
     int time;
 } cf_model_preindex;
 int cf_models_preindex(cf_ctx *ctx, const cf_model_preindex *items, int n, float depth_cutoff, int time_delta);
+int cf_model_index_box(cf_model *m, int box[4], int *culled, uint32_t *passes);
 int cf_model_download_map(cf_model *m, float *host_surfels, uint32_t capacity, uint32_t *count);
 int cf_model_upload_map(cf_model *m, const float *host_surfels, uint32_t count);
 int cf_model_buffer(cf_model *m, int which, void **dptr, uint64_t *bytes);
```
